# cisco/thor

Hardware: AMD Instinct MI355X
Metric: encoder Mpixels/s at fixed qp, bit-exact recon vs ref (higher is better)
Workload: dtype u8

## Files before the change

### include/thor_hip.h

```cpp
#ifndef THOR_HIP_H
#define THOR_HIP_H
#include <stddef.h>
#include <stdint.h>
#ifdef __cplusplus
extern "C" {
#endif

struct thor_encoder_info;
void encode_frame_lbd(struct thor_encoder_info* encoder_info);
void encode_frame_hbd(struct thor_encoder_info* encoder_info);

typedef struct thor_hip_params {
  int width, height, qp;
  int bitdepth, input_bitdepth;
  float frame_rate;
  float lambda_coeffI, lambda_coeffP;
  float early_skip_thr;
  int enable_tb_split, enable_pb_split, max_num_ref, HQperiod;
  int num_reorder_pics, interp_ref;
  int dqpP, dqpI;
  float mqpP;
  int intra_period, intra_rdo, encoder_speed;
  int deblocking, cdef, clpf, use_block_contexts, enable_bipred;
  int cfl_intra, cfl_inter;
  int dyadic_coding;
  float lambda_coeffB, lambda_coeffB0, lambda_coeffB1, lambda_coeffB2, lambda_coeffB3;
  int dqpB, dqpB0, dqpB1, dqpB2, dqpB3;
  float mqpB, mqpB0, mqpB1, mqpB2, mqpB3;
  int max_clpf_strength;
  int log2_sb_size;
} thor_hip_params;

typedef struct thor_hip_encoder thor_hip_encoder;

int thor_hip_params_from_config(thor_hip_params* p, const char* cfg_path);

int thor_hip_params_set(thor_hip_params* p, const char* name, const char* value);

int thor_hip_params_set_sb_size(thor_hip_params* p, int log2_sb_size);

int thor_hip_device_count(void);
thor_hip_encoder* thor_hip_open(const thor_hip_params* p, int num_streams, int device);
void thor_hip_close(thor_hip_encoder* e);

int thor_hip_begin_sequence(thor_hip_encoder* e, int stream, int skip, int num_frames, int file_frames);
int thor_hip_next_frame(thor_hip_encoder* e, int stream, int* display_index);

size_t thor_hip_frame_bytes(const thor_hip_encoder* e);
int thor_hip_stage_frame(thor_hip_encoder* e, int stream, int slot, const void* yuv);
int thor_hip_stage_frame_device(thor_hip_encoder* e, int stream, int slot, const void* dev_yuv);
int thor_hip_encode_staged(thor_hip_encoder* e, const int* slots);
typedef void (*thor_hip_frames_done_fn)(void* user, int first_stream, int num_streams);
int thor_hip_encode_staged_run(thor_hip_encoder* e, int nframes, thor_hip_frames_done_fn done, void* user);
int thor_hip_last_display_index(const thor_hip_encoder* e, int stream);
int thor_hip_encode_frame(thor_hip_encoder* e, const void* const* yuv_per_stream);

size_t thor_hip_stream_bytes(const thor_hip_encoder* e, int stream);
const uint8_t* thor_hip_stream_data(const thor_hip_encoder* e, int stream);
int thor_hip_get_recon(thor_hip_encoder* e, int stream, void* yuv_out);

void thor_hip_kernel_time(thor_hip_encoder* e, double* sb_ms, long* sb_launches, double* filter_ms);
void thor_hip_kernel_time_reset(thor_hip_encoder* e);
void thor_hip_read_stats(thor_hip_encoder* e, unsigned long long out[4], int reset);
void thor_hip_set_frame_distortion(thor_hip_encoder* e, int on);
typedef struct thor_hip_frame_stats {
  int display_index;
  int frame_type;
  int qp;
  int num_bits;
  int num_ref;
  int ref_array[4];
  int ref_frame_num[4];
  int has_sse;
  unsigned long long sse[3];
  double psnr[3];
} thor_hip_frame_stats;
int thor_hip_frame_stats_count(const thor_hip_encoder* e, int stream);
int thor_hip_get_frame_stats(const thor_hip_encoder* e, int stream, int i, thor_hip_frame_stats* out);
int thor_hip_report(const thor_hip_encoder* e, int stream, char* buf, size_t n);
int thor_hip_stat_line(const thor_hip_encoder* e, int stream, int num_frames, char* buf, size_t n);

void thor_hip_read_prof(thor_hip_encoder* e, long long out[32]);

int thor_hip_sad_batch(const uint8_t* org, int w, int h, const uint8_t* ref_plane, int plane_w, int plane_h,
                       int rstride, int bx, int by, const int* cand, int n, uint32_t* out);
int thor_hip_interp_luma(const uint8_t* ref_plane, int plane_w, int plane_h, int rstride, int pad, int bx, int by,
                         int w, int h, const int16_t* mv, int n, int bipred, uint8_t* out);
int thor_hip_code_tu_batch(const uint8_t* org, const uint8_t* pred, int size, int qp, int coeff_type, int fast, int n,
                           int16_t* coefq, uint8_t* rec, int* cbp);
typedef struct thor_hip_cell {
  int16_t mv0x, mv0y, mv1x, mv1y;
  uint8_t mode, size, tbpb, cbp;
  int8_t ref0, ref1, dir;
  uint8_t pad;
} thor_hip_cell;
int thor_hip_deblock_frame(uint8_t* yuv, int width, int height, int qp, const thor_hip_cell* cells);

int thor_hip_sad_batch_hbd(const uint16_t* org, int w, int h, const uint16_t* ref_plane, int plane_w, int plane_h,
                           int rstride, int bx, int by, const int* cand, int n, uint32_t* out);
int thor_hip_interp_luma_hbd(const uint16_t* ref_plane, int plane_w, int plane_h, int rstride, int pad, int bx, int by,
                             int w, int h, const int16_t* mv, int n, int bipred, int bitdepth, uint16_t* out);
int thor_hip_code_tu_batch_hbd(const uint16_t* org, const uint16_t* pred, int size, int qp, int coeff_type, int fast, int n,
                               int bitdepth, int16_t* coefq, uint16_t* rec, int* cbp);
int thor_hip_deblock_frame_hbd(uint16_t* yuv, int width, int height, int qp, int bitdepth, const thor_hip_cell* cells);

int thor_hip_kat_intra(const void* plane, int width, int height, int stride, int bitdepth, int size, int tb_split, int n, const int* par,
                       const void* rblocks, void* out);
int thor_hip_kat_inter_yuv(const void* yuv, int width, int height, int bitdepth, int size, int n, const int* par, const int16_t* mv, void* out);
int thor_hip_kat_average(const void* a, const void* b, int size, int bitdepth, int n, void* out);
int thor_hip_kat_cfl(const void* y, void* uv, const void* ry, int n_luma, int bitdepth, int n);
int thor_hip_kat_cdef_dir(const void* blocks, int bitdepth, int n, int* dir, int* var);
int thor_hip_kat_cdef_filter(const void* plane, int width, int height, int stride, int bitdepth, int bsize, int n, const int* par, void* out);
int thor_hip_kat_clpf(const void* rec_yuv, const void* org_yuv, int width, int height, int bitdepth, int qp, const thor_hip_cell* cells,
                      const int* strength, int fb_log2, const uint8_t* fb_on, uint32_t* stats, void* out_yuv);
int thor_hip_kat_interpolate(const void* yuv0, const void* yuv1, int width, int height, int bitdepth, void* out_yuv);

int thor_hip_kat_motion_estimate(const void* cur, const void* ref, int width, int height, int bitdepth, int n, const int* par, const double* lambda,
                                 const int16_t* cand, int ncand_total, int* out);
int thor_hip_kat_motion_estimate_bi(const void* cur, const void* ref0, const void* ref1, int width, int height, int bitdepth, int n, const int* par,
                                    const double* lambda, const int16_t* cand, int* out, int16_t* list_out);
int thor_hip_kat_early_skip(const int* chroma, const void* org, const void* pred, const int* size, const int* qp, const float* thr, int bitdepth, int n, int* out);
int thor_hip_kat_coeff_syntax(int n, const int* par, const int16_t* coef, int words, uint32_t* buf_single, uint32_t* buf_team, int* out);
int thor_hip_kat_block_syntax(int n, const int* par, const int16_t* pool, int npool, int words, uint32_t* buf_coop, uint32_t* buf_single, int* out);
int thor_hip_kat_gather_bits(int n, const uint32_t* src, int src_words, const int* src_off, const int* nbits, const long long* dst_bit, uint32_t* dst, int dst_words);

int thor_hip_frame_sse(const void* a, const void* b, int w, int h, int bitdepth, unsigned long long out[3]);
int thor_hip_kat_depth_up(const void* in, int w, int h, int bitdepth, int input_bitdepth, uint16_t* out);
int thor_hip_kat_depth_down(const uint16_t* in, int w, int h, int bitdepth, int input_bitdepth, void* out);
int thor_hip_frame_sse_depth(const void* a, const void* b, int w, int h, int bitdepth, int input_bitdepth, unsigned long long out[3]);

int thor_hip_superblock_kernel_info(int sample_bytes, int* num_regs, int* lds_bytes, int* private_bytes, int* workgroups_per_cu);
int thor_hip_superblock_kernel_in_use(void);

#ifdef __cplusplus
}
#endif
#endif
```

### thor_amd/binding.py

```python
import ctypes as C
import os
import subprocess
import numpy as np

REPO_ROOT = os.path.dirname(os.path.dirname(os.path.abspath(__file__)))
_LIB = None


def lib_path():
    return os.environ.get('THOR_HIP_LIB') or os.path.join(REPO_ROOT, 'thor_amd', 'libthor_hip.so')


HIPCC_FLAGS = ['--offload-arch=gfx950', '-O3', '-std=c++17', '-ffp-contract=off', '-fno-strict-aliasing', '-fPIC', '-pthread']
NATIVE_SOURCES = ['thor_hip.cpp', 'thor_hip_lat.cpp', 'thor_hip_wide.cpp', 'thor_hip_katbits.cpp']


def build_native(force=False):
    csrc = os.path.join(REPO_ROOT, 'thor_amd', 'csrc')
    out = os.path.join(REPO_ROOT, 'thor_amd', 'libthor_hip.so')
    hdrs = [os.path.join(csrc, f) for f in os.listdir(csrc)]
    hdrs += [os.path.join(REPO_ROOT, 'include', f) for f in os.listdir(os.path.join(REPO_ROOT, 'include'))]
    newest = max(os.path.getmtime(h) for h in hdrs)
    if force or not os.path.exists(out) or os.path.getmtime(out) < newest:
        hipcc = '/opt/rocm/bin/hipcc' if os.path.exists('/opt/rocm/bin/hipcc') else 'hipcc'
# ... 250 lines not shown
    return a.ctypes.data_as(C.c_void_p)


def _pix(bitdepth):
    return np.uint16 if bitdepth > 8 else np.uint8


def sad_batch(org, ref_plane, bx, by, cand, bitdepth=8):
    T = _pix(bitdepth)
    org = np.ascontiguousarray(org, dtype=T); ref_plane = np.ascontiguousarray(ref_plane, dtype=T)
    cand = np.ascontiguousarray(cand, dtype=np.int32)
    out = np.zeros(len(cand), dtype=np.uint32)
    fn = lib().thor_hip_sad_batch_hbd if bitdepth > 8 else lib().thor_hip_sad_batch
    rc = fn(_vp(org), org.shape[1], org.shape[0], _vp(ref_plane), ref_plane.shape[1], ref_plane.shape[0], ref_plane.shape[1], bx, by,
            _vp(cand), len(cand), _vp(out))
    if rc:
        raise RuntimeError(f'thor_hip_sad_batch rc={rc}')
    return out


def interp_luma(ref_padded, pad, pic_w, pic_h, bx, by, w, h, mvs, bipred, bitdepth=8):
    T = _pix(bitdepth)
    ref_padded = np.ascontiguousarray(ref_padded, dtype=T); mvs = np.ascontiguousarray(mvs, dtype=np.int16)
    out = np.zeros((len(mvs), h, w), dtype=T)
    if bitdepth > 8:
        rc = lib().thor_hip_interp_luma_hbd(_vp(ref_padded), pic_w, pic_h, ref_padded.shape[1], pad, bx, by, w, h, _vp(mvs), len(mvs),
                                            bipred, bitdepth, _vp(out))
    else:
        rc = lib().thor_hip_interp_luma(_vp(ref_padded), pic_w, pic_h, ref_padded.shape[1], pad, bx, by, w, h, _vp(mvs), len(mvs),
                                        bipred, _vp(out))
    if rc:
        raise RuntimeError(f'thor_hip_interp_luma rc={rc}')
    return out


def code_tu_batch(org, pred, qp, coeff_type, fast, bitdepth=8):
    T = _pix(bitdepth)
    org = np.ascontiguousarray(org, dtype=T); pred = np.ascontiguousarray(pred, dtype=T)
    n, size = org.shape[0], org.shape[1]
    q = min(size, 16)
    coefq = np.zeros((n, q, q), dtype=np.int16); rec = np.zeros_like(org); cbp = np.zeros(n, dtype=np.int32)
    if bitdepth > 8:
        rc = lib().thor_hip_code_tu_batch_hbd(_vp(org), _vp(pred), size, qp, coeff_type, fast, n, bitdepth, _vp(coefq), _vp(rec), _vp(cbp))
    else:
        rc = lib().thor_hip_code_tu_batch(_vp(org), _vp(pred), size, qp, coeff_type, fast, n, _vp(coefq), _vp(rec), _vp(cbp))
    if rc:
        raise RuntimeError(f'thor_hip_code_tu_batch rc={rc}')
    return coefq, rec, cbp


def deblock_frame(yuv, width, height, qp, cells, bitdepth=8):
    yuv = np.ascontiguousarray(yuv, dtype=_pix(bitdepth)).copy()
    cells = np.ascontiguousarray(cells, dtype=np.uint8)
    assert yuv.size == width * height * 3 // 2 and cells.size == (width // 4) * (height // 4) * 16
    if bitdepth > 8:
        rc = lib().thor_hip_deblock_frame_hbd(_vp(yuv), width, height, qp, bitdepth, _vp(cells))
    else:
        rc = lib().thor_hip_deblock_frame(_vp(yuv), width, height, qp, _vp(cells))
    if rc:
        raise RuntimeError(f'thor_hip_deblock_frame rc={rc}')
    return yuv


def _kat(name, *args):
    fn = getattr(lib(), name)
    fn.restype = C.c_int
    rc = fn(*args)
    if rc:
        raise RuntimeError(f'{name} rc={rc}')


def kat_intra(plane, size, par, bitdepth=8, rblocks=None):
    T = _pix(bitdepth)
    plane = np.ascontiguousarray(plane, dtype=T); par = np.ascontiguousarray(par, dtype=np.int32)
    n = len(par)
    out = np.zeros((n, size, size), dtype=T)
    rb = np.ascontiguousarray(rblocks, dtype=T) if rblocks is not None else None
    _kat('thor_hip_kat_intra', _vp(plane), plane.shape[1], plane.shape[0], plane.shape[1], bitdepth, size, 1 if rb is not None else 0, n, _vp(par),
         _vp(rb) if rb is not None else None, _vp(out))
    return out


def kat_inter_yuv(yuv, width, height, size, par, mvs, bitdepth=8):
    T = _pix(bitdepth)
    yuv = np.ascontiguousarray(yuv, dtype=T); par = np.ascontiguousarray(par, dtype=np.int32); mvs = np.ascontiguousarray(mvs, dtype=np.int16)
    n = len(par)
    out = np.zeros((n, size * size * 3 // 2), dtype=T)
    _kat('thor_hip_kat_inter_yuv', _vp(yuv), width, height, bitdepth, size, n, _vp(par), _vp(mvs), _vp(out))
    return out


def kat_average(a, b, size, bitdepth=8):
    T = _pix(bitdepth)
    a = np.ascontiguousarray(a, dtype=T); b = np.ascontiguousarray(b, dtype=T)
    out = np.zeros_like(a)
    _kat('thor_hip_kat_average', _vp(a), _vp(b), size, bitdepth, len(a), _vp(out))
    return out


def kat_cfl(y, uv, ry, n_luma, bitdepth=8):
    T = _pix(bitdepth)
    y = np.ascontiguousarray(y, dtype=T); ry = np.ascontiguousarray(ry, dtype=T); uv = np.array(uv, dtype=T, order='C')
    _kat('thor_hip_kat_cfl', _vp(y), _vp(uv), _vp(ry), n_luma, bitdepth, len(y))
    return uv


def kat_cdef_dir(blocks, bitdepth=8):
    T = _pix(bitdepth)
    blocks = np.ascontiguousarray(blocks, dtype=T)
    n = len(blocks)
    d = np.zeros(n, dtype=np.int32); v = np.zeros(n, dtype=np.int32)
    _kat('thor_hip_kat_cdef_dir', _vp(blocks), bitdepth, n, _vp(d), _vp(v))
    return d, v


def kat_cdef_filter(plane, bsize, par, bitdepth=8):
    T = _pix(bitdepth)
    plane = np.ascontiguousarray(plane, dtype=T); par = np.ascontiguousarray(par, dtype=np.int32)
    out = np.zeros((len(par), bsize, bsize), dtype=T)
    _kat('thor_hip_kat_cdef_filter', _vp(plane), plane.shape[1], plane.shape[0], plane.shape[1], bitdepth, bsize, len(par), _vp(par), _vp(out))
    return out


def kat_clpf(rec, org, width, height, qp, cells, strength, fb_log2, fb_on, bitdepth=8):
    T = _pix(bitdepth)
    rec = np.ascontiguousarray(rec, dtype=T); org = np.ascontiguousarray(org, dtype=T)
    cells = np.ascontiguousarray(cells, dtype=np.uint8); fb_on = np.ascontiguousarray(fb_on, dtype=np.uint8)
    st = np.ascontiguousarray(strength, dtype=np.int32)
    nblk = (width // 8) * (height // 8) + 2 * (width // 16) * (height // 16)
    stats = np.zeros((nblk, 4), dtype=np.uint32)
    out = np.zeros_like(rec)
    _kat('thor_hip_kat_clpf', _vp(rec), _vp(org), width, height, bitdepth, qp, _vp(cells), _vp(st), fb_log2, _vp(fb_on), _vp(stats), _vp(out))
    return stats, out


def kat_interpolate(yuv0, yuv1, width, height, bitdepth=8):
    T = _pix(bitdepth)
    a = np.ascontiguousarray(yuv0, dtype=T); b = np.ascontiguousarray(yuv1, dtype=T)
    out = np.zeros_like(a)
    _kat('thor_hip_kat_interpolate', _vp(a), _vp(b), width, height, bitdepth, _vp(out))
    return out


def kat_motion_estimate(cur, ref, par, lam, cand, bitdepth=8):
    T = _pix(bitdepth)
    cur = np.ascontiguousarray(cur, dtype=T); ref = np.ascontiguousarray(ref, dtype=T)
    par = np.ascontiguousarray(par, dtype=np.int32); lam = np.ascontiguousarray(lam, dtype=np.float64); cand = np.ascontiguousarray(cand, dtype=np.int16).reshape(-1, 2)
    assert cur.shape == ref.shape and par.shape[1] == 17 and len(lam) == len(par)
    out = np.full((len(par), 3), -1, dtype=np.int32)
    _kat('thor_hip_kat_motion_estimate', _vp(cur), _vp(ref), cur.shape[1], cur.shape[0], bitdepth, len(par), _vp(par), _vp(lam), _vp(cand), len(cand), _vp(out))
    return out


def kat_motion_estimate_bi(cur, ref0, ref1, par, lam, cand, bitdepth=8):
    T = _pix(bitdepth)
    cur, ref0, ref1 = (np.ascontiguousarray(a, dtype=T) for a in (cur, ref0, ref1))
    par = np.ascontiguousarray(par, dtype=np.int32); lam = np.ascontiguousarray(lam, dtype=np.float64); cand = np.ascontiguousarray(cand, dtype=np.int16)
    assert cur.shape == ref0.shape == ref1.shape and par.shape[1] == 17 and len(lam) == len(par) and cand.size == 12 * len(par)
    out = np.full((len(par), 3), -1, dtype=np.int32)
    lists = np.zeros((len(par), 6, 2), dtype=np.int16)
    _kat('thor_hip_kat_motion_estimate_bi', _vp(cur), _vp(ref0), _vp(ref1), cur.shape[1], cur.shape[0], bitdepth, len(par), _vp(par), _vp(lam), _vp(cand), _vp(out), _vp(lists))
    return out, lists


def kat_early_skip(chroma, org, pred, size, qp, thr, bitdepth=8):
    T = _pix(bitdepth)
    org = np.ascontiguousarray(org, dtype=T); pred = np.ascontiguousarray(pred, dtype=T)
    chroma, size, qp = (np.ascontiguousarray(a, dtype=np.int32) for a in (chroma, size, qp))
    thr = np.ascontiguousarray(thr, dtype=np.float32)
    n = len(org)
    assert org.shape == pred.shape == (n, 32, 32) and len(chroma) == len(size) == len(qp) == len(thr) == n
    out = np.full(n, -1, dtype=np.int32)
    _kat('thor_hip_kat_early_skip', _vp(chroma), _vp(org), _vp(pred), _vp(size), _vp(qp), _vp(thr), bitdepth, n, _vp(out))
    return out


def kat_coeff_syntax(par, coef, words, buf_single, buf_team):
    par = np.ascontiguousarray(par, dtype=np.int32); coef = np.ascontiguousarray(coef, dtype=np.int16)
    n = len(par)
    b1 = np.ascontiguousarray(buf_single, dtype=np.uint32).copy(); bt = np.ascontiguousarray(buf_team, dtype=np.uint32).copy()
    assert par.shape == (n, 4) and coef.shape == (n, 256) and b1.shape == (n, words) and bt.shape == (n, words)
    out = np.zeros((n, 6), dtype=np.int32)
    _kat('thor_hip_kat_coeff_syntax', n, _vp(par), _vp(coef), words, _vp(b1), _vp(bt), _vp(out))
    return out, b1, bt


def kat_block_syntax(par, pool, words, fill=0):
    par = np.ascontiguousarray(par, dtype=np.int32); pool = np.ascontiguousarray(pool, dtype=np.int16)
    n = len(par)
    assert par.shape == (n, 57) and pool.ndim == 2 and pool.shape[1] == 256
    bc = np.full((n, words), fill, dtype=np.uint32); b1 = np.full((n, words), fill, dtype=np.uint32)
    out = np.zeros((n, 10), dtype=np.int32)
    _kat('thor_hip_kat_block_syntax', n, _vp(par), _vp(pool), len(pool), words, _vp(bc), _vp(b1), _vp(out))
    return out, bc, b1


def kat_gather_bits(src, src_off, nbits, dst_bit, dst_words):
    src = np.ascontiguousarray(src, dtype=np.uint32); src_off = np.ascontiguousarray(src_off, dtype=np.int32)
    nbits = np.ascontiguousarray(nbits, dtype=np.int32); dst_bit = np.ascontiguousarray(dst_bit, dtype=np.int64)
    dst = np.zeros(dst_words, dtype=np.uint32)
    _kat('thor_hip_kat_gather_bits', len(nbits), _vp(src), len(src), _vp(src_off), _vp(nbits), _vp(dst_bit), _vp(dst), dst_words)
    return dst


def frame_sse(a, b, width, height, bitdepth=8):
    T = _pix(bitdepth)
    a = np.ascontiguousarray(a, dtype=T).reshape(-1); b = np.ascontiguousarray(b, dtype=T).reshape(-1)
    if a.size != width * height * 3 // 2 or b.size != a.size:
        raise ValueError('frame size does not match width x height 4:2:0')
    out = (C.c_ulonglong * 3)()
    rc = lib().thor_hip_frame_sse(_vp(a), _vp(b), width, height, bitdepth, out)
    if rc:
        raise RuntimeError(f'thor_hip_frame_sse returned {rc}')
    return [int(v) for v in out]


def _depth_frame(a, depth, width, height):
    a = np.ascontiguousarray(a, dtype=_pix(depth)).reshape(-1)
    if a.size != width * height * 3 // 2:
        raise ValueError('frame size does not match width x height 4:2:0')
    return a


def kat_depth_up(frame, width, height, bitdepth, input_bitdepth):
    a = _depth_frame(frame, input_bitdepth, width, height)
    out = np.zeros(a.size, dtype=np.uint16)
    _kat('thor_hip_kat_depth_up', _vp(a), width, height, bitdepth, input_bitdepth, _vp(out))
    return out


def kat_depth_down(frame, width, height, bitdepth, input_bitdepth):
    a = _depth_frame(frame, 16, width, height)
    out = np.zeros(a.size, dtype=_pix(input_bitdepth))
    _kat('thor_hip_kat_depth_down', _vp(a), width, height, bitdepth, input_bitdepth, _vp(out))
    return out


def frame_sse_depth(a, b, width, height, bitdepth, input_bitdepth):
    T = 16 if bitdepth > input_bitdepth else bitdepth
    a = _depth_frame(a, T, width, height); b = _depth_frame(b, T, width, height)
    out = (C.c_ulonglong * 3)()
    _kat('thor_hip_frame_sse_depth', _vp(a), _vp(b), width, height, bitdepth, input_bitdepth, out)
    return [int(v) for v in out]
```

### thor_amd/csrc/hip_kat.h

```cpp
#pragma once
#include "tk_kat_bits.h"
namespace tk {
template <typename PIX>
__global__ __launch_bounds__(64) void k_kat_sad(const PIX* org, int w, int h, const PIX* refp, int rstride, int bx, int by, const int* cand, int n,
                                               uint32_t* out) {
  const Team t = mk_team((int)threadIdx.x, 64);
  struct KC { const PIX* p; int dx, dy; };
  MeWin win;
  win.on = 0; win.w32 = nullptr; win.ox = win.oy = win.Ww = win.Wh = win.pitch = 0;
  auto cnd = [&](int c) -> KC {
    KC x;
    x.dx = cand[2 * c]; x.dy = cand[2 * c + 1];
    x.p = refp + (size_t)(by + x.dy) * rstride + bx + x.dx;
    return x;
  };
  seg_sads<SP_GLOBAL>(t, n, org, w, rstride, w, h, win, cnd, [&](int c, const KC&, int sad, int mine) { if (mine) out[c] = (uint32_t)sad; });
}
template <typename PIX>
__global__ __launch_bounds__(64) void k_kat_interp(const PIX* ref0, int rstride, int pic_w, int pic_h, int bx, int by, int w, int h,
                                                  const int16_t* mv, int bipred, int bitdepth, PIX* out) {
  const Team t = mk_team((int)threadIdx.x, 64);
  const int i = blockIdx.x;
  pred_luma<SP_GLOBAL>(t, out + (size_t)i * w * h, w, ref0 + (size_t)by * rstride + bx, rstride, w, h, mk_mv(mv[2 * i], mv[2 * i + 1]), 0,
            bipred, pic_w, pic_h, bx, by, bitdepth);
}
template <typename PIX>
__global__ __launch_bounds__(64) void k_kat_tu(const PIX* org, const PIX* pred, int size, int qp, int coeff_type, int fast, int bitdepth,
                                              int16_t* coefq, PIX* rec, int* cbp) {
  __shared__ XformWs xf;
  __shared__ XformTabs tabs;
  __shared__ int16_t cq[256];
  const Team t = mk_team((int)threadIdx.x, 64, tabs.izz);
  xf.prof = nullptr;
  xf.tabs = &tabs;
  xform_tables_fill(&tabs, (int)threadIdx.x, 64);
  t.sync();
  const int i = blockIdx.x, qs = size < 16 ? size : 16;
  const size_t o = (size_t)i * size * size;
  int c = code_tu(t, &xf, org + o, size, pred + o, size, rec + o, size, size, qp, coeff_type, fast, cq, bitdepth);
  for (int k = threadIdx.x; k < qs * qs; k += 64) coefq[(size_t)i * qs * qs + k] = cq[k];
  if (threadIdx.x == 0) cbp[i] = c;
}

template <typename PIX>
__global__ __launch_bounds__(64) void k_kat_intra(const PIX* plane, int stride, int bitdepth, int size, int tb_split, const int* par, const PIX* rblocks,
                                                 PIX* out) {
  __shared__ IntraEdge<PIX> edge;
  const Team t = mk_team((int)threadIdx.x, 64);
  const int it = blockIdx.x;
  const int* q = par + 7 * it;
  const int cbs = tb_split ? 2 * size : size;
  const PIX* rblock = tb_split ? rblocks + (size_t)it * cbs * cbs + q[5] * cbs + q[6] : nullptr;
  make_edges<SP_GLOBAL>(t, &edge, plane + (size_t)q[0] * stride + q[1], stride, rblock, cbs, q[5], q[6], q[0], q[1], size, q[2], q[3], tb_split, bitdepth);
  pred_intra<SP_GLOBAL>(t, &edge, q[0] + q[5], q[1] + q[6], size, out + (size_t)it * size * size, size, q[4], bitdepth);
}
template <typename PIX>
__global__ __launch_bounds__(kWgThreads, (sizeof(PIX) == 1 ? (int)kOcc : 2)) void k_kat_inter_yuv(Plane3<PIX> ref, int width, int height, int bitdepth, int size, const int* par, const int16_t* mv, PIX* out) {
  const Team t = mk_team((int)threadIdx.x, 64);
  const int it = blockIdx.x;
  const int* q = par + 5 * it;
  mv_t m[4];
  for (int k = 0; k < 4; k++) m[k] = mk_mv(mv[(it * 4 + k) * 2], mv[(it * 4 + k) * 2 + 1]);
  PIX* o = out + (size_t)it * (size * size * 3 / 2);
  pred_inter_yuv<SP_GLOBAL>(t, ref, o, o + size * size, o + size * size * 5 / 4, q[0], q[1], size, size, size, m, q[2], width, height, q[3], q[4], bitdepth);
}
template <typename PIX> __global__ __launch_bounds__(64) void k_kat_average(const PIX* a, const PIX* b, int size, PIX* out) {
  const Team t = mk_team((int)threadIdx.x, 64);
  const size_t o = (size_t)blockIdx.x * (size * size * 3 / 2);
  const int n = size * size, c = n / 4;
  average_yuv<SP_GLOBAL>(t, out + o, out + o + n, out + o + n + c, a + o, a + o + n, a + o + n + c, b + o, b + o + n, b + o + n + c, size, size, size);
}
template <typename PIX>
__global__ __launch_bounds__(kWgThreads, (sizeof(PIX) == 1 ? (int)kOcc : 2)) void k_kat_cfl(const PIX* y, PIX* uv, const PIX* ry, int n, int bitdepth) {
  const Team t = mk_team((int)threadIdx.x, 64);
  const int it = blockIdx.x, c = (n / 2) * (n / 2);
  improve_uv<PIX, SP_GLOBAL>(t, nullptr, y + (size_t)it * n * n, uv + (size_t)it * 2 * c, uv + (size_t)it * 2 * c + c, ry + (size_t)it * n * n, n, n, n, bitdepth);
}
template <typename PIX> __global__ void k_kat_cdef_dir(const PIX* blocks, int n, int cs, int* dir, int* var) {
  const int i = (int)(blockIdx.x * blockDim.x + threadIdx.x);
  if (i >= n) return;
  int v = 0;
  dir[i] = cdef_find_dir(blocks + (size_t)i * 64, 8, &v, cs);
  var[i] = v;
}
template <typename PIX>
__global__ __launch_bounds__(64) void k_kat_cdef_filter(const PIX* plane, int w, int h, int stride, int bsize, int cs, const int* par, PIX* out) {
  const int it = blockIdx.x, k = threadIdx.x;
  if (k >= bsize * bsize) return;
  const int* q = par + 7 * it;
  const int x = q[0] + k % bsize, y = q[1] + k / bsize;
  out[(size_t)it * bsize * bsize + k] = (PIX)cdef_filter_px(plane, stride, x, y, w, h, q[2], q[3], q[4], q[5], q[6], cs);
}
enum { kKatMePar = 17 };
template <typename PIX>
__global__ __launch_bounds__(kWgThreads, (sizeof(PIX) == 1 ? (int)kOcc : 2)) void k_kat_me(int bi, Plane3<PIX> cur, Plane3<PIX> ref0, Plane3<PIX> ref1, int fw, int fh, int bitdepth,
                                                                                           const int* par, const double* lam, const int16_t* cand, unsigned char* big, int* out,
                                                                                           int16_t* list_out) {
  __shared__ WgShared sh;
  __shared__ SmallWs<PIX> sws;
  const int lane = (int)threadIdx.x, it = (int)blockIdx.x;
  TeamWs<PIX> ws = make_ws(&sws, &sh, (BigWs<PIX>*)big);
  const Team t = mk_team(lane, 64, sh.tabs.izz);
  xform_tables_fill(&sh.tabs, lane, 64);
  const int* q = par + kKatMePar * it;
  const int cbx = q[0], cby = q[1], cb = q[2], pux = cbx + q[3], puy = cby + q[4];
  MeLists* lists = &sh.lists;
  const int nl = bi ? 6 : q[14];
  for (int c = lane; c < nl; c += 64) { lists->mvcand[0][c].x = cand[2 * (q[15] + c)]; lists->mvcand[0][c].y = cand[2 * (q[15] + c) + 1]; }
  if (lane == 0) { lists->mvcand_num[0] = q[14]; lists->mvcand_mask[0] = 0; lists->best_ref = 0; }
  const int lds_blk = __builtin_amdgcn_readfirstlane(cb <= kLdsBlk);
  PIX* orgc = (PIX*)sh.org_raw;
  if (lds_blk)
    for (int k = lane; k < cb * cb; k += 64) orgc[k] = cur.y[(size_t)(cby + k / cb) * cur.sy + cbx + k % cb];
  __syncthreads();
  MeArgs a;
  a.cb_size = cb; a.ostride = lds_blk ? cb : cur.sy; a.width = q[5]; a.height = q[6]; a.rstride = ref0.sy; a.sign = q[11]; a.fwidth = fw; a.fheight = fh;
  a.xpos = cbx; a.ypos = cby; a.pu_x = pux; a.pu_y = puy; a.enable_bipred = q[12]; a.bitdepth = bitdepth; a.speed = q[13]; a.lam = lam[it];
  const mv_t mvc = mk_mv(q[7], q[8]), mvp = mk_mv(q[9], q[10]);
  const PIX* org = lds_blk ? orgc + q[4] * cb + q[3] : cur.y + (size_t)puy * cur.sy + pux;
  mv_t mv = mk_mv(0, 0);
  unsigned cost;
  if (bi) {
    const PIX* r0 = ref0.y + (size_t)cby * ref0.sy + cbx;
    const PIX* r1 = ref1.y + (size_t)cby * ref1.sy + cbx;
    cost = lds_blk ? motion_estimate_bi<PIX, SP_LDS>(t, ws.mep, org, r0, r1, a, mvc, mvp, 0, &mv) : motion_estimate_bi<PIX, SP_GLOBAL>(t, ws.mep, org, r0, r1, a, mvc, mvp, 0, &mv);
  } else {
    if (q[16]) me_stage_cb_window<PIX>(t, ws.mep, ref0.y + (size_t)cby * ref0.sy + cbx, ref0.sy, cbx, cby, cb, mvc, a.sign, fw, fh, 0);
    const PIX* rp = ref0.y + (size_t)puy * ref0.sy + pux;
    cost = lds_blk ? motion_estimate<PIX, SP_LDS>(t, ws.mep, org, rp, a, mvc, mvp, 0, &mv) : motion_estimate<PIX, SP_GLOBAL>(t, ws.mep, org, rp, a, mvc, mvp, 0, &mv);
  }
  __syncthreads();
  if (lane == 0) { out[3 * it] = mv.x; out[3 * it + 1] = mv.y; out[3 * it + 2] = (int)cost; }
  if (bi && lane < 6) { list_out[12 * it + 2 * lane] = lists->mvcand[0][lane].x; list_out[12 * it + 2 * lane + 1] = lists->mvcand[0][lane].y; }
}
template <typename PIX>
__global__ __launch_bounds__(kWgThreads, (sizeof(PIX) == 1 ? (int)kOcc : 2)) void k_kat_early_skip(const int* chroma, const PIX* org, const PIX* pred, const int* size, const int* qp,
                                                                                                   const float* thr, int bitdepth, unsigned char* big, int* out) {
  __shared__ FrameJob<PIX> sJ;
  __shared__ WgShared sh;
  __shared__ SmallWs<PIX> sws;
  __shared__ TeamWs<PIX> s_view;
  const int lane = (int)threadIdx.x, it = (int)blockIdx.x;
  lds_st(&s_view, make_ws(&sws, &sh, (BigWs<PIX>*)big));
  WsP<PIX> ws = ldsc(&s_view);
  JobR<PIX> J = *ldsc(&sJ);
  const Team t = mk_team(lane, 64, sh.tabs.izz);
  xform_tables_fill(&sh.tabs, lane, 64);
  if (lane == 0) sJ.cfg.bitdepth = bitdepth;
  const int ch = __builtin_amdgcn_readfirstlane(chroma[it]), n = __builtin_amdgcn_readfirstlane(size[it]), qpi = __builtin_amdgcn_readfirstlane(qp[it]);
  const float th = thr[it];
  const PIX* o = org + (size_t)it * 1024;
  const PIX* p = pred + (size_t)it * 1024;
  const int lds_blk = n <= (ch ? kLdsBlk / 2 : kLdsBlk);
  PIX* lo = sws.lbuf;
  PIX* lp = sws.lbuf + kLdsBlk * kLdsBlk;
  if (lds_blk)
    for (int k = lane; k < n * n; k += 64) { lo[k] = o[(k / n) * 32 + k % n]; lp[k] = p[(k / n) * 32 + k % n]; }
  __syncthreads();
  int r;
  if (ch) r = lds_blk ? early_skip_subC<PIX, SP_LDS>(t, J, ws, lo, n, lp, n, n, qpi, th) : early_skip_subC<PIX, SP_GLOBAL>(t, J, ws, o, 32, p, 32, n, qpi, th);
  else r = lds_blk ? early_skip_sub<PIX, SP_LDS>(t, J, ws, lo, n, lp, n, n, qpi, th) : early_skip_sub<PIX, SP_GLOBAL>(t, J, ws, o, 32, p, 32, n, qpi, th);
  if (lane == 0) out[it] = r;
}
}

template <typename PIX>
static int kat_sad_batch(const PIX* org, int w, int h, const PIX* ref_plane, int plane_w, int plane_h, int rstride, int bx, int by, const int* cand,
                         int n, uint32_t* out) {
  if (!org || !ref_plane || !cand || !out || n <= 0 || w < 4 || h < 4 || (w & (w - 1)) || (h & (h - 1))) return 1;
  for (int i = 0; i < n; i++) {
    int x = bx + cand[2 * i], y = by + cand[2 * i + 1];
    if (x < 0 || y < 0 || x + w > plane_w || y + h > plane_h) return 2;
  }
  if (!ensure_init_any()) return 3;
  DevBuf<PIX> d_org((size_t)w * h, org);
  DevBuf<PIX> d_ref((size_t)rstride * plane_h + 16);
  backend::h2d(d_ref, ref_plane, (size_t)rstride * plane_h * sizeof(PIX));
  DevBuf<int> d_c((size_t)2 * n, cand);
  DevBuf<uint32_t> d_o(n);
  hipLaunchKernelGGL(k_kat_sad<PIX>, dim3(1), dim3(64), 0, g_stream, d_org, w, h, d_ref, rstride, bx, by, d_c, n, d_o);
  HIPCHECK(hipGetLastError());
  backend::d2h(out, d_o, (size_t)n * 4);
  return 0;
}
extern "C" int thor_hip_sad_batch(const uint8_t* org, int w, int h, const uint8_t* ref_plane, int plane_w, int plane_h, int rstride,
                                  int bx, int by, const int* cand, int n, uint32_t* out) {
  return kat_sad_batch<uint8_t>(org, w, h, ref_plane, plane_w, plane_h, rstride, bx, by, cand, n, out);
}
extern "C" int thor_hip_sad_batch_hbd(const uint16_t* org, int w, int h, const uint16_t* ref_plane, int plane_w, int plane_h, int rstride,
                                      int bx, int by, const int* cand, int n, uint32_t* out) {
  return kat_sad_batch<uint16_t>(org, w, h, ref_plane, plane_w, plane_h, rstride, bx, by, cand, n, out);
}

template <typename PIX>
static int kat_interp_luma(const PIX* ref_plane, int plane_w, int plane_h, int rstride, int pad, int bx, int by, int w, int h, const int16_t* mv,
                           int n, int bipred, int bitdepth, PIX* out) {
  if (!ref_plane || !mv || !out || n <= 0) return 1;
  if (!ensure_init_any()) return 3;
  DevBuf<PIX> d_ref((size_t)rstride * (plane_h + 2 * pad), ref_plane);
  DevBuf<int16_t> d_mv((size_t)2 * n, mv);
  DevBuf<PIX> d_o((size_t)n * w * h);
  hipLaunchKernelGGL(k_kat_interp<PIX>, dim3(n), dim3(64), 0, g_stream, d_ref.get() + (size_t)pad * rstride + pad, rstride, plane_w, plane_h, bx,
                     by, w, h, d_mv, bipred, bitdepth, d_o);
  HIPCHECK(hipGetLastError());
  backend::d2h(out, d_o, (size_t)n * w * h * sizeof(PIX));
  return 0;
}
extern "C" int thor_hip_interp_luma(const uint8_t* ref_plane, int plane_w, int plane_h, int rstride, int pad, int bx, int by, int w,
                                    int h, const int16_t* mv, int n, int bipred, uint8_t* out) {
  return kat_interp_luma<uint8_t>(ref_plane, plane_w, plane_h, rstride, pad, bx, by, w, h, mv, n, bipred, 8, out);
}
extern "C" int thor_hip_interp_luma_hbd(const uint16_t* ref_plane, int plane_w, int plane_h, int rstride, int pad, int bx, int by, int w,
                                        int h, const int16_t* mv, int n, int bipred, int bitdepth, uint16_t* out) {
  if (bitdepth < 9 || bitdepth > 12) return 1;
  return kat_interp_luma<uint16_t>(ref_plane, plane_w, plane_h, rstride, pad, bx, by, w, h, mv, n, bipred, bitdepth, out);
}

template <typename PIX>
static int kat_code_tu_batch(const PIX* org, const PIX* pred, int size, int qp, int coeff_type, int fast, int n, int bitdepth, int16_t* coefq,
                             PIX* rec, int* cbp) {
  if (!org || !pred || !coefq || !rec || !cbp || n <= 0) return 1;
  if (size != 4 && size != 8 && size != 16 && size != 32 && size != 64 && size != 128) return 2;
  if (!ensure_init_any()) return 3;
  const size_t px = (size_t)n * size * size;
  const int qs = size < 16 ? size : 16;
  DevBuf<PIX> d_org(px, org), d_pred(px, pred), d_rec(px);
  DevBuf<int16_t> d_cq((size_t)n * qs * qs);
  DevBuf<int> d_cbp(n);
  hipLaunchKernelGGL(k_kat_tu<PIX>, dim3(n), dim3(64), 0, g_stream, d_org, d_pred, size, qp, coeff_type, fast, bitdepth, d_cq, d_rec,
                     d_cbp);
  HIPCHECK(hipGetLastError());
  backend::d2h(coefq, d_cq, (size_t)n * qs * qs * 2);
  backend::d2h(rec, d_rec, px * sizeof(PIX));
  backend::d2h(cbp, d_cbp, (size_t)n * 4);
  return 0;
}
extern "C" int thor_hip_code_tu_batch(const uint8_t* org, const uint8_t* pred, int size, int qp, int coeff_type, int fast, int n,
                                      int16_t* coefq, uint8_t* rec, int* cbp) {
  return kat_code_tu_batch<uint8_t>(org, pred, size, qp, coeff_type, fast, n, 8, coefq, rec, cbp);
}
extern "C" int thor_hip_code_tu_batch_hbd(const uint16_t* org, const uint16_t* pred, int size, int qp, int coeff_type, int fast, int n,
                                          int bitdepth, int16_t* coefq, uint16_t* rec, int* cbp) {
  if (bitdepth < 9 || bitdepth > 12) return 1;
  return kat_code_tu_batch<uint16_t>(org, pred, size, qp, coeff_type, fast, n, bitdepth, coefq, rec, cbp);
}

template <typename PIX> static int kat_deblock_frame(PIX* yuv, int width, int height, int qp, int bitdepth, const thor_hip_cell* cells) {
  static_assert(sizeof(thor_hip_cell) == sizeof(DbCell), "thor_hip_cell must mirror tk::DbCell");
  if (!yuv || !cells || width % 8 || height % 8 || width < 16 || height < 16 || qp < 0 || qp > 51) return 1;
  if (!ensure_init_any()) return 3;
  DevFrame<PIX> f;
  f.alloc(width, height, 0);
  DevBuf<DbCell> d_cells((size_t)(width / 4) * (height / 4), (const DbCell*)cells);
  upload_yuv(f, yuv, width, height);
  FrameJob<PIX> J;
  memset(&J, 0, sizeof(J));
  J.cfg.width = width; J.cfg.height = height; J.cfg.bitdepth = bitdepth;
  J.qp = qp; J.rec = f.p; J.cells = d_cells; J.cell_stride = width / 4;
  DevBuf<FrameJob<PIX>> d_job(1, &J);
  backend::run_deblock<PIX>(d_job, &J, 1);
  backend::dev_sync();
  download_yuv(f, yuv, width, height);
  f.release();
  return 0;
}
extern "C" int thor_hip_deblock_frame(uint8_t* yuv, int width, int height, int qp, const thor_hip_cell* cells) {
  return kat_deblock_frame<uint8_t>(yuv, width, height, qp, 8, cells);
}
extern "C" int thor_hip_deblock_frame_hbd(uint16_t* yuv, int width, int height, int qp, int bitdepth, const thor_hip_cell* cells) {
  if (bitdepth < 9 || bitdepth > 12) return 1;
  return kat_deblock_frame<uint16_t>(yuv, width, height, qp, bitdepth, cells);
}

namespace {
template <typename PIX>
int kat_intra(const PIX* plane, int width, int height, int stride, int bitdepth, int size, int tb_split, int n, const int* par, const PIX* rblocks, PIX* out) {
  if (!plane || !par || !out || n <= 0 || size < 4 || size > 64 || (size & (size - 1)) || (tb_split && !rblocks) || stride < width) return 1;
  const int cbs = tb_split ? 2 * size : size;
  for (int i = 0; i < n; i++) {
    const int* q = par + 7 * i;
    if (q[0] < 0 || q[1] < 0 || q[0] + cbs > height || q[1] + cbs > width || q[4] < 0 || q[5] < 0 || q[6] < 0 || q[5] + size > cbs || q[6] + size > cbs) return 2;
    if ((q[2] && q[1] + 2 * cbs > width) || (q[3] && q[0] + 2 * cbs > height)) return 2;
  }
  if (!ensure_init_any()) return 3;
  DevBuf<PIX> d_p((size_t)stride * height, plane);
  DevBuf<int> d_par((size_t)7 * n, par);
  DevBuf<PIX> d_rb(tb_split ? (size_t)n * cbs * cbs : 0, tb_split ? rblocks : nullptr);
  DevBuf<PIX> d_o((size_t)n * size * size);
// ... 29 lines not shown
  const size_t per = (size_t)size * size * 3 / 2;
  DevBuf<PIX> d_o(per * n);
  hipLaunchKernelGGL(k_kat_inter_yuv<PIX>, dim3(n), dim3(64), 0, g_stream, ref.p, width, height, bitdepth, size, d_par, d_mv, d_o);
  HIPCHECK(hipGetLastError());
  backend::d2h(out, d_o, per * n * sizeof(PIX));
  ref.release();
  return 0;
}
template <typename PIX> int kat_average(const PIX* a, const PIX* b, int size, int n, PIX* out) {
  if (!a || !b || !out || n <= 0 || size < 8 || size > 128 || (size & (size - 1))) return 1;
  if (!ensure_init_any()) return 3;
  const size_t tot = (size_t)n * size * size * 3 / 2;
  DevBuf<PIX> d_a(tot, a), d_b(tot, b), d_o(tot);
  hipLaunchKernelGGL(k_kat_average<PIX>, dim3(n), dim3(64), 0, g_stream, d_a, d_b, size, d_o);
  HIPCHECK(hipGetLastError());
  backend::d2h(out, d_o, tot * sizeof(PIX));
  return 0;
}
template <typename PIX> int kat_cfl(const PIX* y, PIX* uv, const PIX* ry, int nl, int bitdepth, int n) {
  if (!y || !uv || !ry || n <= 0 || nl < 8 || nl > 128 || (nl & (nl - 1))) return 1;
  if (!ensure_init_any()) return 3;
  const size_t ny = (size_t)n * nl * nl, nc = (size_t)n * 2 * (nl / 2) * (nl / 2);
  DevBuf<PIX> d_y(ny, y), d_r(ny, ry), d_uv(nc, uv);
  hipLaunchKernelGGL(k_kat_cfl<PIX>, dim3(n), dim3(64), 0, g_stream, d_y, d_uv, d_r, nl, bitdepth);
  HIPCHECK(hipGetLastError());
  backend::d2h(uv, d_uv, nc * sizeof(PIX));
  return 0;
}
template <typename PIX> int kat_cdef_dir(const PIX* blocks, int bitdepth, int n, int* dir, int* var) {
  if (!blocks || !dir || !var || n <= 0) return 1;
  if (!ensure_init_any()) return 3;
  DevBuf<PIX> d_b((size_t)n * 64, blocks);
  DevBuf<int> d_d(n), d_v(n);
  hipLaunchKernelGGL(k_kat_cdef_dir<PIX>, dim3((n + 63) / 64), dim3(64), 0, g_stream, d_b, n, bitdepth - 8, d_d, d_v);
  HIPCHECK(hipGetLastError());
  backend::d2h(dir, d_d, (size_t)n * 4); backend::d2h(var, d_v, (size_t)n * 4);
  return 0;
}
template <typename PIX> int kat_cdef_filter(const PIX* plane, int w, int h, int stride, int bitdepth, int bsize, int n, const int* par, PIX* out) {
  if (!plane || !par || !out || n <= 0 || (bsize != 4 && bsize != 8) || stride < w) return 1;
  for (int i = 0; i < n; i++) {
    const int* q = par + 7 * i;
    if (q[0] < 0 || q[1] < 0 || q[0] + bsize > w || q[1] + bsize > h || q[4] < 0 || q[4] > 7) return 2;
  }
  if (!ensure_init_any()) return 3;
  DevBuf<PIX> d_p((size_t)stride * h, plane);
  DevBuf<int> d_par((size_t)7 * n, par);
  DevBuf<PIX> d_o((size_t)n * bsize * bsize);
  hipLaunchKernelGGL(k_kat_cdef_filter<PIX>, dim3(n), dim3(64), 0, g_stream, d_p, w, h, stride, bsize, bitdepth - 8, d_par, d_o);
  HIPCHECK(hipGetLastError());
  backend::d2h(out, d_o, (size_t)n * bsize * bsize * sizeof(PIX));
  return 0;
}
template <typename PIX>
int kat_clpf(const PIX* rec_yuv, const PIX* org_yuv, int width, int height, int bitdepth, int qp, const thor_hip_cell* cells, const int* strength, int fb_log2,
             const uint8_t* fb_on, uint32_t* stats, PIX* out_yuv) {
  if (!rec_yuv || !org_yuv || !cells || !strength || !fb_on || !stats || !out_yuv || width % 16 || height % 16 || fb_log2 < 5 || fb_log2 > 7) return 1;
  if (!ensure_init_any()) return 3;
  DevFrame<PIX> rec, src, org;
  rec.alloc(width, height, 0); src.alloc(width, height, 0); org.alloc(width, height, 0);
  upload_yuv(rec, rec_yuv, width, height); upload_yuv(src, rec_yuv, width, height); upload_yuv(org, org_yuv, width, height);
  DevBuf<DbCell> d_cells((size_t)(width / 4) * (height / 4), (const DbCell*)cells);
  const int nblk = (width / 8) * (height / 8) + 2 * (width / 16) * (height / 16);
  const int nfb = ((width + (1 << fb_log2) - 1) >> fb_log2) * ((height + (1 << fb_log2) - 1) >> fb_log2);
  DevBuf<uint32_t> d_stats((size_t)4 * nblk);
  DevBuf<uint8_t> d_on((size_t)nfb, fb_on);
  ClpfJob<PIX> J;
  memset(&J, 0, sizeof(J));
  J.rec = rec.p; J.src = src.p; J.org = org.p; J.width = width; J.height = height; J.bitdepth = bitdepth; J.qp = qp;
  J.cells = d_cells; J.cs = width / 4; J.stats = d_stats;
  for (int k = 0; k < 3; k++) J.strength[k] = strength[k];
  J.fb_log2 = fb_log2; J.fb_on = d_on;
  DevBuf<ClpfJob<PIX>> d_job(1, &J);
  backend::run_clpf_stats<PIX>(d_job, &J, 1);
  backend::run_clpf_apply<PIX>(d_job, &J, 1);
  backend::dev_sync();
  backend::d2h(stats, d_stats, (size_t)4 * nblk * 4);
  download_yuv(rec, out_yuv, width, height);
  rec.release(); src.release(); org.release();
  return 0;
}
template <typename PIX> int kat_interpolate(const PIX* yuv0, const PIX* yuv1, int width, int height, int bitdepth, PIX* out_yuv) {
  if (!yuv0 || !yuv1 || !out_yuv || width % 8 || height % 8 || width < 64 || height < 64) return 1;
  if (!ensure_init_any()) return 3;
  SeqParams sp;
  sp.width = width; sp.height = height; sp.bitdepth = bitdepth; sp.input_bitdepth = bitdepth;
  sp.num_reorder_pics = 7; sp.interp_ref = 1; sp.max_num_ref = 2; sp.HQperiod = 8; sp.cdef = 0; sp.clpf = 0;
  Engine<PIX>* eng = new Engine<PIX>();
  eng->open(sp, 1);
  Stream<PIX>& q = eng->st[0];
  for (int k = 0; k < 2; k++) {
    upload_yuv(q.rec, k ? yuv1 : yuv0, width, height);
    FrameJob<PIX> J;
    memset(&J, 0, sizeof(J));
    J.cfg.width = width; J.cfg.height = height; J.rec = q.rec.p;
    backend::run_make_ref<PIX>(&J, &q.ring[k].p, 1);
    backend::dev_sync();
  }
  std::vector<FrameParams> fp(1);
  fp[0].interp_ref = 1; fp[0].interp_src[0] = 0; fp[0].interp_src[1] = 1; fp[0].frame_num = 1;
  eng->make_interp_frames(fp, 0, 1);
  backend::dev_sync();
  download_yuv(q.interp, out_yuv, width, height);
  eng->close();
  delete eng;
  return 0;
}
template <typename PIX> DevFrame<PIX> kat_luma_frame(const PIX* luma, int width, int height, int pad_ref) {
  std::vector<PIX> yuv((size_t)width * height * 3 / 2, (PIX)0);
  memcpy(yuv.data(), luma, (size_t)width * height * sizeof(PIX));
  if (pad_ref) return kat_padded_ref(yuv.data(), width, height);
  DevFrame<PIX> f;
  f.alloc(width, height, 0);
  upload_yuv(f, yuv.data(), width, height);
  return f;
}
template <typename PIX>
int kat_me(int bi, const PIX* cur, const PIX* ref0, const PIX* ref1, int width, int height, int bitdepth, int n, const int* par, const double* lam, const int16_t* cand,
           int ncand_total, int* out, int16_t* list_out) {
  if (!cur || !ref0 || (bi && (!ref1 || !list_out)) || !par || !lam || !out || n <= 0 || ncand_total < 0 || (ncand_total && !cand) || width % 8 || height % 8 || width < 16 ||
      height < 16 || width > 8192 || height > 8192)
    return 1;
  auto pow2 = [](int v, int lo, int hi) { return v >= lo && v <= hi && !(v & (v - 1)); };
  for (int i = 0; i < n; i++) {
    const int* q = par + kKatMePar * i;
    if (!pow2(q[2], 8, kMaxSb) || !pow2(q[5], 4, q[2]) || !pow2(q[6], 4, q[2]) || (q[11] & ~1) || (q[12] & ~1) || q[13] < 0 || q[13] > 2 || !(lam[i] >= 0.0 && lam[i] <= 1e6)) return 1;
    if (q[0] < 0 || q[1] < 0 || q[0] + q[2] > width || q[1] + q[2] > height || q[3] < 0 || q[4] < 0 || q[3] + q[5] > q[2] || q[4] + q[6] > q[2] || q[3] % 4 || q[4] % 4) return 2;
    for (int k = 7; k <= 10; k++) if (q[k] < -8192 || q[k] > 8192) return 1;
    const int slots = bi ? 6 : q[14];
    if (q[14] < 0 || q[14] > (bi ? 6 : 64) || q[15] < 0 || q[15] + slots > ncand_total) return 2;
    if (bi && (q[3] || q[4] || q[5] != q[2] || q[6] != q[2])) return 1;
    for (int c = 0; c < slots; c++) if (cand[2 * (q[15] + c)] < -2047 || cand[2 * (q[15] + c)] > 2047 || cand[2 * (q[15] + c) + 1] < -2047 || cand[2 * (q[15] + c) + 1] > 2047) return 1;
  }
  if (!ensure_init_any()) return 3;
  DevFrame<PIX> fc = kat_luma_frame(cur, width, height, 0), f0 = kat_luma_frame(ref0, width, height, 1), f1 = bi ? kat_luma_frame(ref1, width, height, 1) : DevFrame<PIX>();
  {
    DevBuf<int> d_par((size_t)kKatMePar * n, par);
    DevBuf<double> d_lam(n, lam);
    DevBuf<int16_t> d_cand((size_t)2 * (ncand_total ? ncand_total : 1));
    if (ncand_total) backend::h2d(d_cand, cand, (size_t)4 * ncand_total);
    DevBuf<unsigned char> d_big(sizeof(BigWs<PIX>));
    DevBuf<int> d_o((size_t)3 * n);
    DevBuf<int16_t> d_l((size_t)12 * n);
    hipLaunchKernelGGL(k_kat_me<PIX>, dim3(n), dim3(64), 0, g_stream, bi, fc.p, f0.p, bi ? f1.p : f0.p, width, height, bitdepth, d_par, d_lam, d_cand, d_big, d_o, d_l);
    HIPCHECK(hipGetLastError());
    backend::d2h(out, d_o, (size_t)3 * n * 4);
    if (bi) backend::d2h(list_out, d_l, (size_t)12 * n * 2);
  }
  fc.release(); f0.release();
  if (bi) f1.release();
  return 0;
}
template <typename PIX>
int kat_early_skip(const int* chroma, const PIX* org, const PIX* pred, const int* size, const int* qp, const float* thr, int bitdepth, int n, int* out) {
  if (!chroma || !org || !pred || !size || !qp || !thr || !out || n <= 0) return 1;
  for (int i = 0; i < n; i++) {
    const int s = size[i];
    if ((chroma[i] & ~1) || qp[i] < 0 || qp[i] > 51 || !(thr[i] >= 0.0f && thr[i] <= 1e3f)) return 1;
    if (chroma[i] ? (s != 4 && s != 8 && s != 16) : (s != 8 && s != 16 && s != 32)) return 2;
  }
  if (!ensure_init_any()) return 3;
  DevBuf<PIX> d_org((size_t)n * 1024, org), d_pred((size_t)n * 1024, pred);
  DevBuf<int> d_ch(n, chroma), d_size(n, size), d_qp(n, qp), d_o(n);
  DevBuf<float> d_thr(n, thr);
  DevBuf<unsigned char> d_big(sizeof(BigWs<PIX>));
  hipLaunchKernelGGL(k_kat_early_skip<PIX>, dim3(n), dim3(64), 0, g_stream, d_ch, d_org, d_pred, d_size, d_qp, d_thr, bitdepth, d_big, d_o);
  HIPCHECK(hipGetLastError());
  backend::d2h(out, d_o, (size_t)n * 4);
  return 0;
}
}
#define KAT_BD(call8, call16) do { if (bitdepth == 8) return call8; if (bitdepth >= 9 && bitdepth <= 12) return call16; return 1; } while (0)
extern "C" int thor_hip_kat_intra(const void* plane, int width, int height, int stride, int bitdepth, int size, int tb_split, int n, const int* par,
                                  const void* rblocks, void* out) {
  KAT_BD(kat_intra<uint8_t>((const uint8_t*)plane, width, height, stride, 8, size, tb_split, n, par, (const uint8_t*)rblocks, (uint8_t*)out),
         kat_intra<uint16_t>((const uint16_t*)plane, width, height, stride, bitdepth, size, tb_split, n, par, (const uint16_t*)rblocks, (uint16_t*)out));
}
extern "C" int thor_hip_kat_inter_yuv(const void* yuv, int width, int height, int bitdepth, int size, int n, const int* par, const int16_t* mv, void* out) {
  KAT_BD(kat_inter_yuv<uint8_t>((const uint8_t*)yuv, width, height, 8, size, n, par, mv, (uint8_t*)out),
         kat_inter_yuv<uint16_t>((const uint16_t*)yuv, width, height, bitdepth, size, n, par, mv, (uint16_t*)out));
}
extern "C" int thor_hip_kat_average(const void* a, const void* b, int size, int bitdepth, int n, void* out) {
  KAT_BD(kat_average<uint8_t>((const uint8_t*)a, (const uint8_t*)b, size, n, (uint8_t*)out),
         kat_average<uint16_t>((const uint16_t*)a, (const uint16_t*)b, size, n, (uint16_t*)out));
}
extern "C" int thor_hip_kat_cfl(const void* y, void* uv, const void* ry, int n_luma, int bitdepth, int n) {
  KAT_BD(kat_cfl<uint8_t>((const uint8_t*)y, (uint8_t*)uv, (const uint8_t*)ry, n_luma, 8, n),
         kat_cfl<uint16_t>((const uint16_t*)y, (uint16_t*)uv, (const uint16_t*)ry, n_luma, bitdepth, n));
}
extern "C" int thor_hip_kat_cdef_dir(const void* blocks, int bitdepth, int n, int* dir, int* var) {
  KAT_BD(kat_cdef_dir<uint8_t>((const uint8_t*)blocks, 8, n, dir, var), kat_cdef_dir<uint16_t>((const uint16_t*)blocks, bitdepth, n, dir, var));
}
extern "C" int thor_hip_kat_cdef_filter(const void* plane, int width, int height, int stride, int bitdepth, int bsize, int n, const int* par, void* out) {
  KAT_BD(kat_cdef_filter<uint8_t>((const uint8_t*)plane, width, height, stride, 8, bsize, n, par, (uint8_t*)out),
         kat_cdef_filter<uint16_t>((const uint16_t*)plane, width, height, stride, bitdepth, bsize, n, par, (uint16_t*)out));
}
extern "C" int thor_hip_kat_clpf(const void* rec_yuv, const void* org_yuv, int width, int height, int bitdepth, int qp, const thor_hip_cell* cells,
                                 const int* strength, int fb_log2, const uint8_t* fb_on, uint32_t* stats, void* out_yuv) {
  KAT_BD(kat_clpf<uint8_t>((const uint8_t*)rec_yuv, (const uint8_t*)org_yuv, width, height, 8, qp, cells, strength, fb_log2, fb_on, stats, (uint8_t*)out_yuv),
         kat_clpf<uint16_t>((const uint16_t*)rec_yuv, (const uint16_t*)org_yuv, width, height, bitdepth, qp, cells, strength, fb_log2, fb_on, stats, (uint16_t*)out_yuv));
}
extern "C" int thor_hip_kat_motion_estimate(const void* cur, const void* ref, int width, int height, int bitdepth, int n, const int* par, const double* lambda,
                                            const int16_t* cand, int ncand_total, int* out) {
  KAT_BD(kat_me<uint8_t>(0, (const uint8_t*)cur, (const uint8_t*)ref, nullptr, width, height, 8, n, par, lambda, cand, ncand_total, out, nullptr),
         kat_me<uint16_t>(0, (const uint16_t*)cur, (const uint16_t*)ref, nullptr, width, height, bitdepth, n, par, lambda, cand, ncand_total, out, nullptr));
}
extern "C" int thor_hip_kat_motion_estimate_bi(const void* cur, const void* ref0, const void* ref1, int width, int height, int bitdepth, int n, const int* par,
                                               const double* lambda, const int16_t* cand, int* out, int16_t* list_out) {
  KAT_BD(kat_me<uint8_t>(1, (const uint8_t*)cur, (const uint8_t*)ref0, (const uint8_t*)ref1, width, height, 8, n, par, lambda, cand, 6 * n, out, list_out),
         kat_me<uint16_t>(1, (const uint16_t*)cur, (const uint16_t*)ref0, (const uint16_t*)ref1, width, height, bitdepth, n, par, lambda, cand, 6 * n, out, list_out));
}
extern "C" int thor_hip_kat_early_skip(const int* chroma, const void* org, const void* pred, const int* size, const int* qp, const float* thr, int bitdepth, int n, int* out) {
  KAT_BD(kat_early_skip<uint8_t>(chroma, (const uint8_t*)org, (const uint8_t*)pred, size, qp, thr, 8, n, out),
         kat_early_skip<uint16_t>(chroma, (const uint16_t*)org, (const uint16_t*)pred, size, qp, thr, bitdepth, n, out));
}
extern "C" int thor_hip_kat_coeff_syntax(int n, const int* par, const int16_t* coef, int words, uint32_t* buf_single, uint32_t* buf_team, int* out) {
  if (n <= 0 || !par || !coef || words <= 0 || words > (1 << 16) || !buf_single || !buf_team || !out) return 1;
  for (int i = 0; i < n; i++) if (kat_coeff_check(par + kKatCoPar * i, words)) return 1;
  if (!ensure_init_any()) return 3;
  DevBuf<int> d_par((size_t)kKatCoPar * n, par), d_o((size_t)kKatCoOut * n);
  DevBuf<int16_t> d_c((size_t)256 * n, coef);
  DevBuf<uint32_t> d_1((size_t)words * n, buf_single), d_t((size_t)words * n, buf_team);
  if (thor_katbits_launch_coeff(g_stream, n, d_par, d_c, words, d_1, d_t, d_o)) return 3;
  backend::d2h(buf_single, d_1, (size_t)words * n * 4); backend::d2h(buf_team, d_t, (size_t)words * n * 4);
  backend::d2h(out, d_o, (size_t)kKatCoOut * n * 4);
  return 0;
}
extern "C" int thor_hip_kat_block_syntax(int n, const int* par, const int16_t* pool, int npool, int words, uint32_t* buf_coop, uint32_t* buf_single, int* out) {
  if (n <= 0 || !par || npool < 0 || (npool && !pool) || words <= 0 || words > (1 << 16) || !buf_coop || !buf_single || !out) return 1;
  std::vector<int16_t> coef((size_t)n * 3072);
  for (int i = 0; i < n; i++) if (kat_block_resolve(par + kKatBlPar * i, pool, npool, coef.data() + (size_t)i * 3072)) return 1;
  if (!ensure_init_any()) return 3;
  DevBuf<int> d_par((size_t)kKatBlPar * n, par), d_o((size_t)kKatBlOut * n);
  DevBuf<int16_t> d_c(coef.size(), coef.data());
  DevBuf<uint32_t> d_w((size_t)words * n, buf_coop), d_1((size_t)words * n, buf_single);
  if (thor_katbits_launch_block(g_stream, n, d_par, d_c, words, d_w, d_1, d_o)) return 3;
  backend::d2h(buf_coop, d_w, (size_t)words * n * 4); backend::d2h(buf_single, d_1, (size_t)words * n * 4);
  backend::d2h(out, d_o, (size_t)kKatBlOut * n * 4);
  return 0;
}
extern "C" int thor_hip_kat_gather_bits(int n, const uint32_t* src, int src_words, const int* src_off, const int* nbits, const long long* dst_bit, uint32_t* dst, int dst_words) {
  if (n <= 0 || !src || src_words <= 0 || !src_off || !nbits || !dst_bit || !dst || dst_words <= 0) return 1;
  for (int i = 0; i < n; i++) {
    if (nbits[i] < 0 || src_off[i] < 0 || dst_bit[i] < 0) return 1;
    if ((long long)src_off[i] + (nbits[i] + 31) / 32 > src_words || dst_bit[i] + nbits[i] > (long long)dst_words * 32) return 2;
  }
  if (!ensure_init_any()) return 3;
  std::vector<backend::GatherItem> items(n);
  DevBuf<uint32_t> d_src((size_t)src_words, src), d_dst((size_t)dst_words);
  for (int i = 0; i < n; i++) {
    items[i].src = d_src.get() + src_off[i]; items[i].nbits = nbits[i]; items[i].dst_bit = dst_bit[i];
  }
  DevBuf<backend::GatherItem> d_items((size_t)n, items.data());
  backend::run_gather(d_items, n, d_dst);
  backend::d2h(dst, d_dst, (size_t)dst_words * 4);
  return 0;
}
template <typename PIX> int frame_sse_host(const PIX* a, const PIX* b, int width, int height, unsigned long long out[3]) {
  if (!a || !b || !out || width % 8 || height % 8 || width < 8 || height < 8) return 1;
  if (!ensure_init_any()) return 3;
  DevFrame<PIX> fa, fb;
  fa.alloc(width, height, 0); fb.alloc(width, height, 0);
  upload_yuv(fa, a, width, height); upload_yuv(fb, b, width, height);
  FrameJob<PIX> J;
  memset(&J, 0, sizeof(J));
  J.cfg.width = width; J.cfg.height = height; J.orig = fa.p; J.rec = fb.p;
  DevBuf<FrameJob<PIX>> dj(1, &J);
  DevBuf<unsigned long long> dout(4);
  launch_frame_sse<PIX>(dj, &J, 1, dout);
  backend::dev_sync();
  backend::d2h(out, dout, 3 * sizeof(unsigned long long));
  fa.release(); fb.release();
  return 0;
}
extern "C" int thor_hip_frame_sse(const void* a, const void* b, int w, int h, int bitdepth, unsigned long long out[3]) {
  KAT_BD(frame_sse_host<uint8_t>((const uint8_t*)a, (const uint8_t*)b, w, h, out),
         frame_sse_host<uint16_t>((const uint16_t*)a, (const uint16_t*)b, w, h, out));
}
static int kat_depth_args(const void* a, const void* b, int w, int h, int bitdepth, int input_bitdepth) {
  auto ok = [](int d) { return d == 8 || d == 10 || d == 12; };
  return !a || !b || w % 8 || h % 8 || w < 8 || h < 8 || !ok(bitdepth) || !ok(input_bitdepth) || input_bitdepth >= bitdepth;
}
extern "C" int thor_hip_kat_depth_up(const void* in, int w, int h, int bitdepth, int input_bitdepth, uint16_t* out) {
  if (kat_depth_args(in, out, w, h, bitdepth, input_bitdepth)) return 1;
  if (!ensure_init_any()) return 3;
  const size_t bytes = (size_t)w * h * 3 / 2 * (input_bitdepth > 8 ? 2 : 1);
  DevBuf<uint8_t> packed(bytes, (const uint8_t*)in);
  DevFrame<uint16_t> f;
  f.alloc(w, h, 0);
  launch_depth_up(packed, f.p, w, h, bitdepth, input_bitdepth);
  backend::dev_sync();
  download_yuv(f, out, w, h);
  f.release();
  return 0;
}
extern "C" int thor_hip_kat_depth_down(const uint16_t* in, int w, int h, int bitdepth, int input_bitdepth, void* out) {
  if (kat_depth_args(in, out, w, h, bitdepth, input_bitdepth)) return 1;
  if (!ensure_init_any()) return 3;
  const size_t bytes = (size_t)w * h * 3 / 2 * (input_bitdepth > 8 ? 2 : 1);
  DevBuf<uint8_t> packed(bytes);
  DevFrame<uint16_t> f;
  f.alloc(w, h, 0);
  upload_yuv(f, in, w, h);
  launch_depth_down(f.p, packed, w, h, bitdepth, input_bitdepth);
  backend::d2h(out, packed, bytes);
  f.release();
  return 0;
}
extern "C" int thor_hip_frame_sse_depth(const void* a, const void* b, int w, int h, int bitdepth, int input_bitdepth, unsigned long long out[3]) {
  if (bitdepth == input_bitdepth) return thor_hip_frame_sse(a, b, w, h, bitdepth, out);
  if (!out || kat_depth_args(a, b, w, h, bitdepth, input_bitdepth)) return 1;
  if (!ensure_init_any()) return 3;
  DevFrame<uint16_t> fa, fb;
  fa.alloc(w, h, 0); fb.alloc(w, h, 0);
  upload_yuv(fa, (const uint16_t*)a, w, h); upload_yuv(fb, (const uint16_t*)b, w, h);
  FrameJob<uint16_t> J;
  memset(&J, 0, sizeof(J));
  J.cfg.width = w; J.cfg.height = h; J.orig = fa.p; J.rec = fb.p;
  DevBuf<FrameJob<uint16_t>> dj(1, &J);
  DevBuf<unsigned long long> dout(4);
  launch_frame_sse_depth(dj, &J, 1, bitdepth, input_bitdepth, dout);
  backend::dev_sync();
  backend::d2h(out, dout, 3 * sizeof(unsigned long long));
  fa.release(); fb.release();
  return 0;
}
extern "C" int thor_hip_kat_interpolate(const void* yuv0, const void* yuv1, int width, int height, int bitdepth, void* out_yuv) {
  KAT_BD(kat_interpolate<uint8_t>((const uint8_t*)yuv0, (const uint8_t*)yuv1, width, height, 8, (uint8_t*)out_yuv),
         kat_interpolate<uint16_t>((const uint16_t*)yuv0, (const uint16_t*)yuv1, width, height, bitdepth, (uint16_t*)out_yuv));
}

extern "C" int thor_hip_superblock_kernel_info(int sample_bytes, int* num_regs, int* lds_bytes, int* private_bytes, int* workgroups_per_cu) {
  if (!ensure_init_any()) return 3;
  hipFuncAttributes a;
  int per_cu = 0;
  if (sample_bytes == 1) {
    HIPCHECK(hipFuncGetAttributes(&a, reinterpret_cast<const void*>(&k_superblocks<uint8_t>)));
    HIPCHECK(hipOccupancyMaxActiveBlocksPerMultiprocessor(&per_cu, k_superblocks<uint8_t>, kWgThreads, 0));
  } else if (sample_bytes == 2) {
    HIPCHECK(hipFuncGetAttributes(&a, reinterpret_cast<const void*>(&k_superblocks<uint16_t>)));
    HIPCHECK(hipOccupancyMaxActiveBlocksPerMultiprocessor(&per_cu, k_superblocks<uint16_t>, kWgThreads, 0));
  } else if (sample_bytes == 0) {
    if (thor_lat_kernel_info(num_regs, lds_bytes, private_bytes)) return 2;
    if (workgroups_per_cu) *workgroups_per_cu = thor_lat_workgroups_per_cu();
    return 0;
  } else if (sample_bytes == 3) {
    if (thor_wide_kernel_info(num_regs, lds_bytes, private_bytes)) return 2;
    if (workgroups_per_cu) *workgroups_per_cu = thor_wide_workgroups_per_cu();
    return 0;
  } else return 1;
  if (num_regs) *num_regs = a.numRegs;
  if (lds_bytes) *lds_bytes = (int)a.sharedSizeBytes;
  if (private_bytes) *private_bytes = (int)a.localSizeBytes;
  if (workgroups_per_cu) *workgroups_per_cu = per_cu;
  return 0;
}
extern "C" int thor_hip_superblock_kernel_in_use(void) { return tk::backend::g_last_kern; }
```

### thor_amd/csrc/tk_block_md.h

```cpp
#pragma once
#include "tk_block_search.h"

namespace tk {
template <typename PIX, int SP>
TK_DEVNI unsigned mode_decision(const Team t, JobR<PIX> J, WsP<PIX> ws, Node& nd) {
  const auto& c = J.cfg;
  const int size = nd.size;
  const double lambda = J.lambda;
  const int rect = nd.bw != size || nd.bh != size;
  const int max_tb = c.enable_tb_split == 1 ? 2 : 1;
  const int max_pb = c.enable_pb_split ? 4 : 1;
  unsigned min_cost = kCostInit;
  int do_inter = 1, do_intra = 1;
  BlkParam p;
  p.mode = M_SKIP; p.intra_mode = 0; p.skip_idx = 0; p.pb_part = P_NONE; p.ref0 = p.ref1 = 0; p.dir = 0;
  p.tb_param = 0; p.tb_split = 0; p.cbp_y = p.cbp_u = p.cbp_v = 0;
  for (int i = 0; i < 4; i++) { p.mv0[i] = mk_mv(0, 0); p.mv1[i] = mk_mv(0, 0); }

  if (J.frame_type != F_I) {
    p.tb_param = 0;
    p.pb_part = P_NONE;
    for (int k = 0; k < nd.syn.num_skip; k++) {
      set_cand(p, nd.skip[k], k, M_SKIP);
      unsigned cost = rdo_trial<PIX, SP>(t, J, ws, nd, p, lambda);
      if (cost < min_cost) { min_cost = cost; if (t.rank == 0) keep_best(nd, p); }
    }
  }
  if ((size < 128 || c.encoder_speed == 0) && !rect) {
    if (J.frame_type != F_I) {
      for (int k = 0; k < nd.syn.num_merge; k++) {
        set_cand(p, nd.merge[k], k, M_MERGE);
        for (int tb = 0; tb <= max_tb - 1; tb++) {
          p.tb_param = (int8_t)tb;
          unsigned cost = rdo_trial<PIX, SP>(t, J, ws, nd, p, lambda, tb > 0, min_cost);
          if (cost < min_cost) { min_cost = cost; if (t.rank == 0) keep_best(nd, p); }
        }
      }
      const int intra_inter_sad = c.encoder_speed > 0;
      unsigned sad_intra = 0xffffffffu;
      if (intra_inter_sad) {
        int im;
        sad_intra = intra_sad_search<PIX, SP>(t, J, ws, nd, J.num_intra_modes, &im);
        sad_intra += (unsigned)(int)mul_add_nofma(J.sqrt_lambda, 2.0, 0.5);
      }
      mv_t mv_center[kMaxRefs];
      mv_t mv_all[4][4];
      mv_t mvp = mk_mv(0, 0);
      const PIX* oy = ws->org_y;
      int min_idx = 0, max_idx = J.num_ref - 1;
      {
        const int br = ws->mep->lists->best_ref;
        if (!(br < 0 || c.encoder_speed < 2 || c.enable_bipred)) min_idx = max_idx = br;
      }
      if (J.frame_type == F_B && J.interp_ref > 2) min_idx = 1;
      unsigned worst_cost = 0, best_cost = 0xffffffffu;
      for (int r = min_idx; r <= max_idx; r++) {
        mvp = get_mv_pred(J.cells, J.cell_stride, nd.ypos, nd.xpos, c.width, c.height, size, sb_size_of(c));
        if (t.rank == 0) add_mvcand(ws->mep, r, mvp);
        t.sync();
        nd.syn.mvp = mvp;
        mv_center[r] = mvp;
        unsigned sad_inter = 0xffffffffu;
        for (int part = 0; part < max_pb; part++) {
          unsigned sad = search_inter<PIX, SP>(t, J, ws, nd.ypos, nd.xpos, size, oy, ws->org_sy, r, mv_center[r], mvp, mv_all[part], part, J.sign[r]);
          add_cands4(t, ws, r, mv_all[part]);
          mv_center[r] = mv_all[0][0];
          sad_inter = sad < sad_inter ? sad : sad_inter;
        }
        if (intra_inter_sad) {
          do_inter = sad_inter < sad_intra;
          if (sad_inter < sad_intra) do_intra = 0;
        }
        if (!do_inter) continue;
        p.mode = M_INTER;
        p.ref0 = p.ref1 = (int8_t)r;
        for (int part = 0; part < max_pb; part++) {
          p.pb_part = (int8_t)part;
          for (int i = 0; i < 4; i++) { p.mv0[i] = mv_all[part][i]; p.mv1[i] = mv_all[part][i]; }
          const int min_tb = c.encoder_speed < 1 ? -1 : 0;
          for (int tb = min_tb; tb <= max_tb - 1; tb++) {
            p.tb_param = (int8_t)tb;
            unsigned cost = rdo_trial<PIX, SP>(t, J, ws, nd, p, lambda, tb > min_tb, (c.encoder_speed < 2 || c.enable_bipred) ? min_cost : 0xffffffffu);
            worst_cost = cost > worst_cost ? cost : worst_cost;
            best_cost = cost < best_cost ? cost : best_cost;
            if (cost < min_cost) { min_cost = cost; if (t.rank == 0) keep_best(nd, p); }
          }
        }
      }
      if (worst_cost && worst_cost * 3u > best_cost * 4u) {
        t.sync();
        if (t.rank == 0) ws->mep->lists->best_ref = 0;
        t.sync();
      }
      if (J.num_ref > 1 && c.enable_bipred && do_inter) {
        int r0, r1;
        mv_t a0[4], a1[4];
        search_bipred<PIX, SP>(t, J, ws, nd, 0, mv_center, mvp, &r0, &r1, a0, a1);
        p.mode = M_BIPRED;
        p.pb_part = P_NONE;
        p.ref0 = (int8_t)r0; p.ref1 = (int8_t)r1;
        for (int i = 0; i < 4; i++) { p.mv0[i] = a0[i]; p.mv1[i] = a1[i]; }
        for (int tb = 0; tb <= max_tb - 1; tb++) {
          p.tb_param = (int8_t)tb;
          unsigned cost = rdo_trial<PIX, SP>(t, J, ws, nd, p, lambda, tb > 0, min_cost);
          if (cost < min_cost) { min_cost = cost; if (t.rank == 0) keep_best(nd, p); }
        }
        if (J.frame_type == F_B && c.encoder_speed == 0) {
          const int ri0 = J.interp_ref ? 1 : 0, ri1 = J.interp_ref ? 2 : 1;
          const Plane3<PIX> f0 = lds_ld(&J.ref[ri0]);
          const Plane3<PIX> f1 = lds_ld(&J.ref[ri1]);
          MeArgs a;
          a.cb_size = size; a.ostride = ws->org_sy; a.width = size; a.height = size; a.rstride = f0.sy; a.sign = 0;
          a.fwidth = c.width; a.fheight = c.height; a.xpos = nd.xpos; a.ypos = nd.ypos; a.enable_bipred = 1;
          a.bitdepth = c.bitdepth; a.lam = J.sqrt_lambda; a.speed = c.encoder_speed; a.pu_x = nd.xpos; a.pu_y = nd.ypos;
          mv_t mvb;
          motion_estimate_bi<PIX, SP>(t, ws->mep, oy, f0.y + nd.ypos * f0.sy + nd.xpos, f1.y + nd.ypos * f1.sy + nd.xpos, a, mv_center[ri0],
                             mvp, ri0, &mvb);
          p.mode = M_BIPRED;
          p.pb_part = P_NONE;
          p.ref0 = (int8_t)ri0; p.ref1 = (int8_t)ri1;
          for (int i = 0; i < 4; i++) { p.mv0[i] = mvb; p.mv1[i] = mvb; }
          p.tb_param = 0;
          unsigned cost = rdo_trial<PIX, SP>(t, J, ws, nd, p, lambda);
          if (cost < min_cost) { min_cost = cost; if (t.rank == 0) keep_best(nd, p); }
        }
      }
    }
    p.mode = M_INTRA;
    int intra_mode = 0;
    unsigned best_tb_cost[2] = {kCostInit, kCostInit};
    if (!do_intra) {
    } else if (c.intra_rdo) {
      unsigned min_intra = kCostInit;
      for (int m = 0; m < J.num_intra_modes; m++) {
        p.intra_mode = (int8_t)m;
        unsigned tbc[2] = {kCostInit, kCostInit};
        int improved = 0;
        for (int tb = 0; tb <= max_tb - 1; tb++) {
          p.tb_param = (int8_t)tb;
          unsigned cost = rdo_trial<PIX, SP>(t, J, ws, nd, p, lambda, 0, min_intra < min_cost ? min_intra : min_cost);
          tbc[tb] = cost;
          if (cost < min_intra) { min_intra = cost; intra_mode = m; improved = 1; }
        }
        if (improved) { best_tb_cost[0] = tbc[0]; best_tb_cost[1] = tbc[1]; }
      }
      p.intra_mode = (int8_t)intra_mode;
      for (int tb = 0; tb <= max_tb - 1; tb++) {
        p.tb_param = (int8_t)tb;
        unsigned cost = best_tb_cost[tb];
        if (cost < min_cost) { min_cost = cost; p.cbp_y = p.cbp_u = p.cbp_v = 0; if (t.rank == 0) keep_best(nd, p); }
      }
    } else {
      intra_sad_search<PIX, SP>(t, J, ws, nd, J.num_intra_modes, &intra_mode);
      p.intra_mode = (int8_t)intra_mode;
      for (int tb = 0; tb <= max_tb - 1; tb++) {
        p.tb_param = (int8_t)tb;
        unsigned cost = rdo_trial<PIX, SP>(t, J, ws, nd, p, lambda);
        if (cost < min_cost) { min_cost = cost; if (t.rank == 0) keep_best(nd, p); }
      }
    }
  }
  return min_cost;
}
}
```

### thor_amd/csrc/tk_block_queue.h

```cpp
#pragma once
#include "tk_block_md.h"

namespace tk {
TK_DEV BlkParam blank_param() {
  BlkParam p;
  p.mode = M_SKIP; p.intra_mode = 0; p.skip_idx = 0; p.pb_part = P_NONE; p.ref0 = p.ref1 = 0; p.dir = 0;
  p.tb_param = 0; p.tb_split = 0; p.cbp_y = p.cbp_u = p.cbp_v = 0;
  for (int i = 0; i < 4; i++) { p.mv0[i] = mk_mv(0, 0); p.mv1[i] = mk_mv(0, 0); }
  return p;
}

template <typename PIX, int SP>
TK_DEV void snapshot_trial(const Team t, WsP<PIX> ws, int size, const BlkParam& p) {
  BigWs<PIX>* g = ws->big;
  const int sc = size >> 1;
  copy_block<SP_GLOBAL, SP>(t, g->best_y, size, ws->rec_y, size, size, size);
  copy_block<SP_GLOBAL, SP>(t, g->best_u, sc, ws->rec_u, sc, sc, sc);
  copy_block<SP_GLOBAL, SP>(t, g->best_v, sc, ws->rec_v, sc, sc, sc);
  if (TKU(p.cbp_y) | TKU(p.cbp_u) | TKU(p.cbp_v)) {
    const int tbs = TKU(p.tb_split);
    const int qy = tbs ? tmin(size >> 1, (int)kMaxQuant) : tmin(size, (int)kMaxQuant);
    const int ny = (tbs ? 4 : 1) * qy * qy;
    const int csplit = tbs && sc > 4;
    const int qc = csplit ? tmin(sc >> 1, (int)kMaxQuant) : tmin(sc, (int)kMaxQuant);
    const int nc = (csplit ? 4 : 1) * qc * qc;
    const int16_t *cy = ws->coef_y, *cu = ws->coef_u, *cv = ws->coef_v;
    TK_GLOBAL int16_t* dy = gptr(g->best_cy);
    TK_GLOBAL int16_t* du = gptr(g->best_cu);
    TK_GLOBAL int16_t* dv = gptr(g->best_cv);
    for (int k = t.rank; k < ny; k += t.size) dy[k] = cy[k];
    for (int k = t.rank; k < nc; k += t.size) { du[k] = cu[k]; dv[k] = cv[k]; }
  }
}

template <typename PIX> struct MdCtx {
  Wg wg;
  WgShared* sh;
  Node* nd;
  unsigned long long mykey;
};

template <typename PIX, int SP>
TK_DEV int par_trial(const Team t, JobR<PIX> J, WsP<PIX> ws, MdCtx<PIX>& M, BlkParam& p, unsigned order, int reuse_pred) {
  int untouched = 0;
  const unsigned cost = rdo_trial<PIX, SP>(t, J, ws, *M.nd, p, J.lambda, reuse_pred, 0xffffffffu, &M.sh->bestkey, order, nullptr, &untouched);
  if (cost == (unsigned)kCostInit) return !untouched;
  const unsigned long long key = ((unsigned long long)cost << 32) | order;
  if (key < M.mykey) {
    M.mykey = key;
    if (t.rank == 0) {
      lds_st(&M.sh->wbest[M.wg.wave], normalize_best(*M.nd, p));
      *ldsc(&M.sh->wkey[M.wg.wave]) = key;
      wg_min64(&M.sh->bestkey, key);
    }
    snapshot_trial<PIX, SP>(t, ws, tk_uniform(ldsc(M.nd)->size), p);
    t.sync();
  }
  return 1;
}

TK_DEV void wg_wait_at_least(const Team t, int* p, int at_least) {
  const unsigned long long w0 = wg_clock();
  for (unsigned spins = 1;; spins++) {
    const int d = wg_load_acquire(p);
    if (team_bcast0(t, d) >= at_least) break;
    if ((spins & 1023u) == 0 && tk_uniform64(wg_clock() - w0) > (unsigned long long)kWgWaitLimit) wg_wait_failed();
    wg_pause();
  }
}
template <typename PIX, int SP>
TK_DEVNI int md_bijoint_telescope(const Team t, JobR<PIX> J, WsP<PIX> ws, MdCtx<PIX>& M) {
  const auto& c = J.cfg;
  WgShared* const sh_ = tk_uniform_ptr(M.sh);
  int mine = 0;
  if (t.rank == 0) mine = wg_cas(&sh_->bj_state, 0, 1);
  if (!team_bcast0(t, mine)) return 0;
  const NodePos nd = node_pos(M.nd);
  const int ri0 = J.interp_ref ? 1 : 0, ri1 = J.interp_ref ? 2 : 1;
  const Plane3<PIX> f0 = lds_ld(&J.ref[ri0]);
  const Plane3<PIX> f1 = lds_ld(&J.ref[ri1]);
  MeArgs a;
  a.cb_size = nd.size; a.ostride = ws->org_sy; a.width = nd.size; a.height = nd.size; a.rstride = f0.sy; a.sign = 0;
  a.fwidth = c.width; a.fheight = c.height; a.xpos = nd.xpos; a.ypos = nd.ypos; a.enable_bipred = 1;
  a.bitdepth = c.bitdepth; a.lam = J.sqrt_lambda; a.speed = c.encoder_speed; a.pu_x = nd.xpos; a.pu_y = nd.ypos;
  mv_t mvb = mk_mv(0, 0);
  const mv_t ctr = lds_ld(&sh_->ref_mv[ri0][0][0]);
  const unsigned sad = motion_estimate_bi<PIX, SP>(t, ws->mep, ws->org_y, f0.y + nd.ypos * f0.sy + nd.xpos, f1.y + nd.ypos * f1.sy + nd.xpos, a, ctr,
                                                   lds_ld(&sh_->mvp), ri0, &mvb, 1);
  t.sync();
  if (t.rank == 0) {
    *ldsc(&sh_->bj_sad) = sad;
    lds_st(&sh_->bj_mv, mvb);
    wg_store_release(&sh_->bj_state, 2);
  }
  t.sync();
  return 1;
}

template <typename PIX, int SP>
TK_DEVNI void md_item_bipred(const Team t, JobR<PIX> J, WsP<PIX> ws, MdCtx<PIX>& M) {
  const auto& c = J.cfg;
  Node& nd_ = *M.nd;
  const NodePos nd = node_pos(&nd_);
  const int size = nd.size;
  const int max_tb = c.enable_tb_split == 1 ? 2 : 1;
  const mv_t mvp = lds_ld(&M.sh->mvp);
  mv_t mv_center[kMaxRefs];
  for (int r = 0; r < kMaxRefs; r++) mv_center[r] = lds_ld(&M.sh->mv_center[r]);
  int r0, r1;
  mv_t a0[4], a1[4];
  search_bipred<PIX, SP>(t, J, ws, nd_, 0, mv_center, mvp, &r0, &r1, a0, a1);
  BlkParam p = blank_param();
  p.mode = M_BIPRED; p.pb_part = P_NONE;
  p.ref0 = (int8_t)r0; p.ref1 = (int8_t)r1;
  for (int i = 0; i < 4; i++) { p.mv0[i] = a0[i]; p.mv1[i] = a1[i]; }
  for (int tb = 0, have_pred = 0; tb <= max_tb - 1; tb++) {
    p.tb_param = (int8_t)tb;
    have_pred |= par_trial<PIX, SP>(t, J, ws, M, p, 54u + (unsigned)tb, have_pred);
  }
  if (J.frame_type == F_B) {
    const int ri0 = J.interp_ref ? 1 : 0, ri1 = J.interp_ref ? 2 : 1;
    const Plane3<PIX> f0 = lds_ld(&J.ref[ri0]);
    const Plane3<PIX> f1 = lds_ld(&J.ref[ri1]);
    const PIX* oy = ws->org_y;
    MeArgs a;
    a.cb_size = size; a.ostride = ws->org_sy; a.width = size; a.height = size; a.rstride = f0.sy; a.sign = 0;
    a.fwidth = c.width; a.fheight = c.height; a.xpos = nd.xpos; a.ypos = nd.ypos; a.enable_bipred = 1;
    a.bitdepth = c.bitdepth; a.lam = J.sqrt_lambda; a.speed = c.encoder_speed; a.pu_x = nd.xpos; a.pu_y = nd.ypos;
    WgShared* const sh_ = tk_uniform_ptr(M.sh);
    if (!md_bijoint_telescope<PIX, SP>(t, J, ws, M)) wg_wait_at_least(t, &sh_->bj_state, 2);
    mv_t mvb = lds_ld(&sh_->bj_mv);
    const unsigned sad0 = (unsigned)tk_uniform((int)*ldsc(&sh_->bj_sad));
    motion_estimate_bi<PIX, SP>(t, ws->mep, oy, f0.y + nd.ypos * f0.sy + nd.xpos, f1.y + nd.ypos * f1.sy + nd.xpos, a, mv_center[ri0], mvp, ri0, &mvb, 2, sad0);
    p.mode = M_BIPRED; p.pb_part = P_NONE;
    p.ref0 = (int8_t)ri0; p.ref1 = (int8_t)ri1;
    for (int i = 0; i < 4; i++) { p.mv0[i] = mvb; p.mv1[i] = mvb; }
    p.tb_param = 0;
    par_trial<PIX, SP>(t, J, ws, M, p, 56u, 0);
  }
}

template <typename PIX, int SP>
TK_DEVNI void md_item_ref(const Team t, JobR<PIX> J, WsP<PIX> ws, MdCtx<PIX>& M, int r) {
  const auto& c = J.cfg;
  const NodePos nd = node_pos(M.nd);
  const int size = nd.size;
  const int max_pb = c.enable_pb_split ? 4 : 1;
  const mv_t mvp = lds_ld(&M.sh->mvp);
  const PIX* oy = ws->org_y;
  if (t.rank == 0) add_mvcand(ws->mep, r, mvp);
  t.sync();
  mv_t mv_center = mvp;
  if (t.rank == 0) ldsc(ws->mep)->cwin_valid = 0;
  t.sync();
  for (int part = 0; part < max_pb; part++) {
    mv_t mv_all[4];
    search_inter<PIX, SP>(t, J, ws, nd.ypos, nd.xpos, size, oy, ws->org_sy, r, mv_center, mvp, mv_all, part, J.sign[r]);
    add_cands4(t, ws, r, mv_all);
    if (part == 0) {
      mv_center = mv_all[0];
      if (max_pb > 1) {
        const Plane3<PIX> rp = lds_ld(&J.ref[r]);
        me_stage_cb_window<PIX>(t, ws->mep, rp.y + nd.ypos * rp.sy + nd.xpos, rp.sy, nd.xpos, nd.ypos, size, mv_center, J.sign[r], c.width, c.height, r);
      }
    }
    if (t.rank == 0) {
      for (int i = 0; i < 4; i++) lds_st(&M.sh->ref_mv[r][part][i], mv_all[i]);
      if (part == max_pb - 1) lds_st(&M.sh->mv_center[r], mv_center);
      wg_fetch_add(&M.sh->parts_done[r], 1);
    }
    t.sync();
  }
  if (t.rank == 0) ldsc(ws->mep)->cwin_valid = 0;
  t.sync();
}

template <typename PIX, int SP>
TK_DEVNI void md_item_trial(const Team t, JobR<PIX> J, WsP<PIX> ws, MdCtx<PIX>& M, int r, int part) {
  const auto& c = J.cfg;
  const int max_tb = c.enable_tb_split == 1 ? 2 : 1;
  r = tk_uniform(r); part = tk_uniform(part);
  WgShared* const sh_ = tk_uniform_ptr(M.sh);
  TK_PROFMD_MARK(pwt_);
  wg_wait_at_least(t, &sh_->parts_done[r], part + 1);
  if (TK_PROFMD_ON(2)) TK_PROFMD_ACC(ws, 20, pwt_);
  mv_t mv_all[4][4];
  for (int q = 0; q <= part; q++)
    for (int i = 0; i < 4; i++) mv_all[q][i] = lds_ld(&sh_->ref_mv[r][q][i]);
  int dup = 0;
  for (int q = 0; q < part && c.enable_pb_split; q++) {
    int eq = 1;
    for (int i = 0; i < 4; i++) eq = eq && mv_all[q][i].x == mv_all[part][i].x && mv_all[q][i].y == mv_all[part][i].y;
    dup = dup || eq;
  }
  if (tk_uniform(dup)) return;
  BlkParam p = blank_param();
  p.mode = M_INTER;
  p.ref0 = p.ref1 = (int8_t)r;
  p.pb_part = (int8_t)part;
  for (int i = 0; i < 4; i++) { p.mv0[i] = mv_all[part][i]; p.mv1[i] = mv_all[part][i]; }
  for (int tb = -1, have_pred = 0; tb <= max_tb - 1; tb++) {
    p.tb_param = (int8_t)tb;
    have_pred |= par_trial<PIX, SP>(t, J, ws, M, p, 6u + 12u * (unsigned)r + 3u * (unsigned)part + (unsigned)(tb + 1), have_pred);
  }
}

template <typename PIX, int SP>
TK_DEVNI void bipred_par(const Wg wg, const Team t, JobR<PIX> J, WsP<PIX> ws, MdCtx<PIX>& M) {
  const auto& c = J.cfg;
  WgShared* sh_ = M.sh;
  const auto sh = ldsc(sh_);
  const NodePos nd = node_pos(M.nd);
  const auto lists = ldsc(lds_ld(&ws->mep->lists));
  const int size = nd.size;
  const int num_iter = c.encoder_speed == 0 ? 2 : 1;
  const int max_tb = c.enable_tb_split == 1 ? 2 : 1;
  const mv_t mvp = lds_ld(&sh_->mvp);
  int prev_ref[2] = {-1, -1}, prev_cnt[2][kMaxRefs];
  mv_t prev_mv[2][4];
  mv_t min0[4], min1[4];
  for (int i = 0; i < 4; i++) { min0[i] = mvp; min1[i] = mvp; }
  int ref0 = 0, ref1 = 0;
  unsigned min_sad = 1u << 30;
  if (wg.wave == 0 && t.rank == 0) sh->bp_org8 = ws->org8;
  t.sync();
  wg.barrier();
  PIX* const org8 = (PIX*)sh->bp_org8;
  const int whole = nd.bw == size && nd.bh == size;
  for (int n = 0; n < num_iter; n++)
    for (int list = 1; list >= 0; list--) {
      const int buf = (2 * n + (1 - list)) & 1;
      const mv_t* mo = list ? min0 : min1;
      const int ref_o = list ? ref0 : ref1;
      int same = n > 0 && prev_ref[list] == ref_o;
      for (int i = 0; i < 4; i++) same = same && prev_mv[list][i].x == mo[i].x && prev_mv[list][i].y == mo[i].y;
      for (int r = 0; r < J.num_ref; r++) {
        const int cnt = lists->mvcand_num[r];
        same = same && prev_cnt[list][r] == cnt;
        prev_cnt[list][r] = cnt;
      }
      prev_ref[list] = ref_o;
      for (int i = 0; i < 4; i++) prev_mv[list][i] = mo[i];
      if (tk_uniform(same)) continue;
      if (whole) {
        const Plane3<PIX> rp = lds_ld(&J.ref[ref_o]);
        const int sgn = J.sign[ref_o];
        const mv_t mvc_ = clip_mv(mo[0], nd.ypos, nd.xpos, c.width, c.height, size, size, sgn);
        const SubPel sp = luma_setup(mvc_, sgn, size, size, c.width, c.height, nd.xpos, nd.ypos, c.enable_bipred);
        const PIX* ry = rp.y + nd.ypos * rp.sy + nd.xpos;
        const int rows = (size + wg.nwaves - 1) / wg.nwaves, r0 = tmin(size, wg.wave * rows), r1 = tmin(size, r0 + rows);
        const auto o8 = spc<SP>(org8);
        const auto oys = spc<SP>(ws->org_y);
        const int osy = ws->org_sy;
        const Pow2 pw = mk_pow2(size);
        for (int k = r0 * size + t.rank; k < r1 * size; k += t.size) {
          int i, j;
          split2(pw, k, i, j);
          o8[k] = (PIX)sat_pix(2 * (int)oys[i * osy + j] - luma_sample(ry, rp.sy, i, j, sp, c.enable_bipred, c.bitdepth), c.bitdepth);
        }
      } else if (wg.wave == 0) {
        pred_inter_yuv<SP>(t, lds_ld(&J.ref[ref_o]), ws->pred_y, ws->pred_u, ws->pred_v, nd.ypos, nd.xpos, size, nd.bw, nd.bh, mo, J.sign[ref_o], c.width,
                           c.height, c.enable_bipred, 0, c.bitdepth, 1);
        t.sync();
        build_org8<PIX, SP>(t, org8, ws->org_y, ws->org_sy, ws->pred_y, size, c.bitdepth);
      }
      t.sync();
      wg.barrier();
      for (int r = wg.wave; r < J.num_ref; r += wg.nwaves) {
        mv_t mv_all[4];
        const unsigned sad = search_inter<PIX, SP>(t, J, ws, nd.ypos, nd.xpos, size, org8, size, r, lds_ld(&sh_->mv_center[r]), mvp, mv_all, 0, J.sign[r]);
        add_cands4(t, ws, r, mv_all);
        if (t.rank == 0) { sh->bp_sad2[buf][r] = sad; for (int i = 0; i < 4; i++) lds_st(&sh_->bp_mv2[buf][r][i], mv_all[i]); }
      }
      t.sync();
      wg.barrier();
      for (int r = 0; r < J.num_ref; r++) {
        const unsigned sd = (unsigned)tk_uniform((int)sh->bp_sad2[buf][r]);
        if (sd < min_sad) {
          min_sad = sd;
          if (list) { ref1 = r; for (int i = 0; i < 4; i++) min1[i] = lds_ld(&sh_->bp_mv2[buf][r][i]); }
          else { ref0 = r; for (int i = 0; i < 4; i++) min0[i] = lds_ld(&sh_->bp_mv2[buf][r][i]); }
        }
      }
    }
  for (int tb = 0; tb <= max_tb - 1; tb++)
    if (wg.wave == tb % wg.nwaves) {
      BlkParam p = blank_param();
      p.mode = M_BIPRED; p.pb_part = P_NONE;
      p.ref0 = (int8_t)ref0; p.ref1 = (int8_t)ref1;
      for (int i = 0; i < 4; i++) { p.mv0[i] = min0[i]; p.mv1[i] = min1[i]; }
      p.tb_param = (int8_t)tb;
      par_trial<PIX, SP>(t, J, ws, M, p, 54u + (unsigned)tb, 0);
    }
}

template <typename PIX, int SP>
TK_MDW void md_worker_sp(const Wg wg, const Team t, JobR<PIX> J, WsP<PIX> ws) {
  WgShared* sh_ = ws->sh;
  const auto sh = ldsc(sh_);
  MdCtx<PIX> M;
  M.wg = wg; M.sh = sh_; M.nd = &sh_->stack[sh->node]; M.mykey = ~0ull;
  if (t.rank == 0) sh->wsnap[wg.wave] = (void*)ws->big;
  const auto ndl = ldsc(M.nd);
  ws_select(ws, tk_uniform(ndl->size));
  org_select(t, J, ws, tk_uniform(ndl->size), ndl->ypos, ndl->xpos, ndl->bw, ndl->bh, 0);
  const auto& c = J.cfg;
  const int max_tb = c.enable_tb_split == 1 ? 2 : 1;
  const int n_items = sh->n_items;
#if TK_PROF_MD
  long long pmd_acc_[4] = {0, 0, 0, 0};
#endif
  for (;;) {
    int i = 0;
    if (t.rank == 0) i = wg_fetch_add(&sh_->next_item, 1);
    i = team_bcast0(t, i);
    if (i >= n_items) break;
    const int kind = team_bcast0(t, sh->items[i].kind), ia = team_bcast0(t, sh->items[i].a), ib = team_bcast0(t, sh->items[i].b);
    TK_PROFMD_MARK(pk_);
    if (kind == MD_SKIP) {
      BlkParam p = blank_param();
      set_cand(p, lds_ld(&M.nd->skip[ia]), ia, M_SKIP);
      par_trial<PIX, SP>(t, J, ws, M, p, (unsigned)ia, 0);
    } else if (kind == MD_MERGE) {
      BlkParam p = blank_param();
      set_cand(p, lds_ld(&M.nd->merge[ia]), ia, M_MERGE);
      for (int tb = 0, have_pred = 0; tb <= max_tb - 1; tb++) {
        p.tb_param = (int8_t)tb;
        have_pred |= par_trial<PIX, SP>(t, J, ws, M, p, 2u + 2u * (unsigned)ia + (unsigned)tb, have_pred);
      }
    } else if (kind == MD_INTRA) {
      BlkParam p = blank_param();
      p.mode = M_INTRA; p.intra_mode = (int8_t)ia; p.tb_param = (int8_t)ib;
      par_trial<PIX, SP>(t, J, ws, M, p, 57u + 2u * (unsigned)ia + (unsigned)ib, 0);
    } else if (kind == MD_REF) {
      md_item_ref<PIX, SP>(t, J, ws, M, ia);
      t.sync();
      int done = 0;
      if (t.rank == 0) done = wg_fetch_add(&sh_->refs_done, 1) + 1;
      done = team_bcast0(t, done);
      if (done == sh->n_ref_items && sh->do_bipred == 1) {
        md_item_bipred<PIX, SP>(t, J, ws, M);
      }
    } else if (kind == MD_TRIAL) {
      md_item_trial<PIX, SP>(t, J, ws, M, ia, ib);
    } else if (kind == MD_BIJOINT) {
      wg_wait_at_least(t, &sh_->parts_done[J.interp_ref ? 1 : 0], 1);
      md_bijoint_telescope<PIX, SP>(t, J, ws, M);
    }
#if TK_PROF_MD
    if (TK_PROFMD_ON(1)) {
      const int slot_ = (kind == MD_SKIP || kind == MD_MERGE) ? 0 : kind == MD_INTRA ? 1 : (kind == MD_REF || kind == MD_BIJOINT) ? 2 : 3;
      if (TK_PROFMD_ON(8)) { const long long d_ = TK_CYC() - pk_; pmd_acc_[0] += slot_ == 0 ? d_ : 0; pmd_acc_[1] += slot_ == 1 ? d_ : 0; pmd_acc_[2] += slot_ == 2 ? d_ : 0; pmd_acc_[3] += slot_ == 3 ? d_ : 0; }
      else TK_PROF_ACC(ws, 16 + slot_, pk_);
    }
#endif
  }
#if TK_PROF_MD
  if (TK_PROFMD_ON(8) && t.rank == 0) for (int q_ = 0; q_ < 4; q_++) ws->prof[16 + q_] += pmd_acc_[q_];
#endif
  if (tk_uniform(sh->do_bipred) == 2) {
    t.sync();
    TK_PROF_MARK(pb_);
    wg.barrier();
    bipred_par<PIX, SP>(wg, t, J, ws, M);
    TK_PROF_ACC(ws, 27, pb_);
  }
}
template <typename PIX>
TK_DEV void md_worker(const Wg wg, const Team t, JobR<PIX> J, WsP<PIX> ws) {
  const auto sh = ldsc(ws->sh);
  const int size = tk_uniform(ldsc(&ws->sh->stack[sh->node])->size);
  if (size <= kLdsBlk) md_worker_sp<PIX, SP_LDS>(wg, t, J, ws);
  else md_worker_sp<PIX, SP_GLOBAL>(wg, t, J, ws);
}

template <typename PIX>
TK_DEV void wg_helper_loop(const Wg wg, const Team t, JobR<PIX> J, WsP<PIX> ws) {
  for (;;) {
    TK_PROF_MARK(ph_);
    wg.barrier();
    TK_PROF_ACC(ws, 28, ph_);
    const int cmd = team_bcast0(t, ws->sh->cmd);
    if (cmd == WG_CMD_EXIT) { wg.barrier(); break; }
#ifdef THOR_PROF
    { TK_PROF_MARK(pw_); md_worker(wg, t, J, ws); TK_PROF_ACC(ws, 5, pw_); }
#else
    md_worker(wg, t, J, ws);
#endif
    t.sync();
    wg.barrier();
  }
}

template <typename PIX>
TK_MDW unsigned mode_decision_par(const Wg wg, const Team t, JobR<PIX> J, WsP<PIX> ws, int node, int* win_wave) {
  const auto& c = J.cfg;
  WgShared* sh_ = ws->sh;
  const auto sh = ldsc(sh_);
  const auto nd = ldsc(&sh_->stack[node]);
  const int max_tb = c.enable_tb_split == 1 ? 2 : 1;
  const int inter = J.frame_type != F_I;
  TK_PROFMD_MARK(pqs_);
  mv_t mvp = mk_mv(0, 0);
  if (inter) mvp = get_mv_pred(J.cells, J.cell_stride, nd->ypos, nd->xpos, c.width, c.height, nd->size, sb_size_of(c));
  t.sync();
  if (t.rank == 0) {
    int n = 0;
    auto push = [&](int kind, int a, int b) { sh->items[n].kind = (int8_t)kind; sh->items[n].a = (int8_t)a; sh->items[n].b = (int8_t)b; sh->items[n].pad = 0; n++; };
    static_assert(2 + 2 + kMaxRefs + 1 + 2 * kNumIntraModes + 4 * kMaxRefs <= kMdMaxItems, "work queue too small");
    static_assert(6 + 12 * kMaxRefs <= 54, "evaluation-order layout: the reference trials must end before the bi-prediction trials");
    if (inter) {
      for (int k = 0; k < nd->syn.num_skip; k++) push(MD_SKIP, k, 0);
      for (int k = 0; k < nd->syn.num_merge; k++) push(MD_MERGE, k, 0);
      for (int r = 0; r < J.num_ref; r++) push(MD_REF, r, 0);
      if (J.num_ref > 1 && c.enable_bipred && J.frame_type == F_B) push(MD_BIJOINT, 0, 0);
      nd->syn.mvp.x = mvp.x; nd->syn.mvp.y = mvp.y;
    }
    for (int m = 0; m < J.num_intra_modes; m++)
      for (int tb = 0; tb <= max_tb - 1; tb++) push(MD_INTRA, m, tb);
    if (inter)
      for (int part = 0; part < (c.enable_pb_split ? 4 : 1); part++)
        for (int r = 0; r < J.num_ref; r++) { push(MD_TRIAL, r, part); sh->parts_done[r] = 0; }
    sh->n_items = n; sh->next_item = 0;
    sh->refs_done = 0; sh->n_ref_items = inter ? J.num_ref : 0;
    sh->do_bipred = (inter && J.num_ref > 1 && c.enable_bipred) ? (J.frame_type == F_P ? 2 : 1) : 0;
    sh->bj_state = 0;
    sh->node = node; lds_st(&sh_->mvp, mvp);
    sh->bestkey = ~0ull;
    for (int w = 0; w < kWaves; w++) sh->wkey[w] = ~0ull;
    sh->cmd = WG_CMD_MD;
  }
  t.sync();
  if (TK_PROFMD_ON(4)) TK_PROFMD_ACC(ws, 21, pqs_);
  wg.barrier();
#ifdef THOR_PROF
  { TK_PROF_MARK(pw_); md_worker(wg, t, J, ws); TK_PROF_ACC(ws, 5, pw_); t.sync(); wg.barrier(); TK_PROF_ACC(ws, 29, pw_); }
#else
// ... 18 lines not shown
```

### thor_amd/csrc/tk_block_search.h

```cpp
#pragma once
#include "tk_block_rd.h"

namespace tk {
template <typename PIX, int SP>
TK_DEV unsigned search_inter(const Team t, JobR<PIX> J, WsP<PIX> ws, int ypos, int xpos, int size,
                             const PIX* org, int ostride, int ref_idx, mv_t mvc, mv_t mvp, mv_t* mv_arr, int part,
                             int sign) {
  const Plane3<PIX> ref = lds_ld(&J.ref[ref_idx]);
  const PIX* ref_y = ref.y + ypos * ref.sy + xpos;
  MeArgs a;
  a.cb_size = size; a.rstride = ref.sy; a.sign = sign; a.fwidth = J.cfg.width; a.fheight = J.cfg.height;
  a.xpos = xpos; a.ypos = ypos; a.enable_bipred = J.cfg.enable_bipred; a.bitdepth = J.cfg.bitdepth;
  a.lam = J.sqrt_lambda; a.ostride = ostride; a.speed = J.cfg.encoder_speed;
  unsigned sad = 0;
  mv_t mv, mvp2 = mvp;
  if (part == P_NONE) {
    a.width = size; a.height = size; a.pu_x = xpos; a.pu_y = ypos;
    sad += motion_estimate<PIX, SP>(t, ws->mep, org, ref_y, a, mvc, mvp2, ref_idx, &mv);
    mv_arr[0] = mv_arr[1] = mv_arr[2] = mv_arr[3] = mv;
  } else if (part == P_HOR) {
    a.width = size; a.height = size / 2;
    for (int index = 0; index < 4; index += 2) {
      int py = index >> 1;
      a.pu_x = xpos; a.pu_y = ypos + py * (size / 2);
      sad += motion_estimate<PIX, SP>(t, ws->mep, org + py * (size / 2) * ostride, ref_y + py * (size / 2) * ref.sy, a, mvc, mvp2, ref_idx, &mv);
      mv_arr[index] = mv; mv_arr[index + 1] = mv;
      mvp2 = mv_arr[0];
    }
  } else if (part == P_VER) {
    a.width = size / 2; a.height = size;
    for (int index = 0; index < 2; index++) {
      a.pu_x = xpos + index * (size / 2); a.pu_y = ypos;
      sad += motion_estimate<PIX, SP>(t, ws->mep, org + index * (size / 2), ref_y + index * (size / 2), a, mvc, mvp2, ref_idx, &mv);
      mv_arr[index] = mv; mv_arr[index + 2] = mv;
      mvp2 = mv_arr[0];
    }
  } else {
    a.width = size / 2; a.height = size / 2;
    for (int index = 0; index < 4; index++) {
      int px = index & 1, py = index >> 1;
      a.pu_x = xpos + px * (size / 2); a.pu_y = ypos + py * (size / 2);
      sad += motion_estimate<PIX, SP>(t, ws->mep, org + py * (size / 2) * ostride + px * (size / 2),
                             ref_y + py * (size / 2) * ref.sy + px * (size / 2), a, mvc, mvp2, ref_idx, &mv);
      mv_arr[index] = mv;
      mvp2 = mv_arr[0];
    }
  }
  return sad;
}

template <typename PIX> TK_DEV void add_cands4(const Team t, WsP<PIX> ws, int ref_idx, const mv_t* mv4) {
  if (t.rank == 0)
    for (int i = 0; i < 4; i++) add_mvcand(ws->mep, ref_idx, mv4[i]);
  t.sync();
}

template <typename PIX, int SP>
TK_DEV void build_org8(const Team t, PIX* o8_, const PIX* oy_, int osy, const PIX* py_, int size, int bitdepth) {
#ifndef TK_NOVEC
  const int S = (int)sizeof(PIX);
  const unsigned al = (unsigned)(uintptr_t)o8_ | (unsigned)(uintptr_t)oy_ | (unsigned)(uintptr_t)py_ | (unsigned)(osy * S);
  if (tk_uniform(!(al & (unsigned)(4 * S - 1)))) {
    const int ppr = size >> 2, lg = ilog2((unsigned)ppr);
    for (int k = t.rank; k < ppr * size; k += t.size) {
      const int i = k >> lg, j = (k & (ppr - 1)) << 2;
      int o[4], p[4];
      load_samples<SP, PIX, 4>(oy_ + i * osy + j, o);
      load_samples<SP, PIX, 4>(py_ + i * size + j, p);
      for (int q = 0; q < 4; q++) o[q] = sat_pix(2 * o[q] - p[q], bitdepth);
      store_samples<SP, PIX, 4>(o8_ + i * size + j, o);
    }
    return;
  }
#endif
  const auto o8 = spc<SP>(o8_);
  const auto oys = spc<SP>(oy_);
  const auto pys = spc<SP>(py_);
  for (int k = t.rank; k < size * size; k += t.size) {
    int i, j;
    split2(mk_pow2(size), k, i, j);
    o8[k] = (PIX)sat_pix(2 * (int)oys[i * osy + j] - (int)pys[k], bitdepth);
  }
}

template <typename PIX, int SP>
TK_DEVNI void search_bipred(const Team t, JobR<PIX> J, WsP<PIX> ws, const Node& nd_, int part,
                          const mv_t* mv_center, mv_t mvp, int* ref_idx0, int* ref_idx1, mv_t* mv_arr0, mv_t* mv_arr1) {
  const auto& c = J.cfg;
  const NodePos nd = node_pos(&nd_);
  const auto lists = ldsc(lds_ld(&ws->mep->lists));
  const int size = nd.size;
  const int num_iter = c.encoder_speed == 0 ? 2 : 1;
  int min_ref0 = (J.frame_type == F_B && J.interp_ref > 0) ? 1 : 0, min_ref1 = 0;
  mv_t min0[4], min1[4];
  for (int i = 0; i < 4; i++) { min0[i] = mvp; min1[i] = mvp; }
  unsigned min_sad = 1u << 30;
  const PIX* oy = ws->org_y;
  const int osy = ws->org_sy;
  int prev_ref[2] = {-1, -1}, prev_cnt[2][kMaxRefs];
  mv_t prev_mv[2][4];
  for (int n = 0; n < num_iter; n++) {
    const int stop = part == 0 ? 0 : 1;
    for (int list = 1; list >= stop; list--) {
      mv_t mvo = list ? min0[0] : min1[0];
      int ref_o = list ? min_ref0 : min_ref1;
      {
        const mv_t* mo = list ? min0 : min1;
        int same = n > 0 && prev_ref[list] == ref_o;
        for (int i = 0; i < 4; i++) same = same && prev_mv[list][i].x == mo[i].x && prev_mv[list][i].y == mo[i].y;
        for (int r = 0; r < J.num_ref; r++) {
          const int cnt = lists->mvcand_num[r];
          same = same && prev_cnt[list][r] == cnt;
          prev_cnt[list][r] = cnt;
        }
        prev_ref[list] = ref_o;
        for (int i = 0; i < 4; i++) prev_mv[list][i] = mo[i];
        if (tk_uniform(same)) continue;
      }
      pred_inter_yuv<SP>(t, lds_ld(&J.ref[ref_o]), ws->pred_y, ws->pred_u, ws->pred_v, nd.ypos, nd.xpos, size, nd.bw, nd.bh,
                     list ? min0 : min1, J.sign[ref_o], c.width, c.height, c.enable_bipred, part > 0, c.bitdepth, 1);
      t.sync();
      build_org8<PIX, SP>(t, ws->org8, oy, osy, ws->pred_y, size, c.bitdepth);
      t.sync();
      int ref_start, ref_end;
      if (J.frame_type == F_P) { ref_start = 0; ref_end = J.num_ref - 1; }
      else {
        ref_start = ref_end = list ? 1 : 0;
        if (J.interp_ref) { ref_start++; ref_end++; }
      }
      for (int r = ref_start; r <= ref_end; r++) {
        mv_t mvp2 = (J.frame_type == F_B && list == 1) ? mvo : mvp;
        mv_t mv_all[4];
        unsigned sad = search_inter<PIX, SP>(t, J, ws, nd.ypos, nd.xpos, size, ws->org8, size, r, mv_center[r], mvp2, mv_all, part, J.sign[r]);
        add_cands4(t, ws, r, mv_all);
        if (sad < min_sad) {
          min_sad = sad;
          if (list) { min_ref1 = r; for (int i = 0; i < 4; i++) min1[i] = mv_all[i]; }
          else { min_ref0 = r; for (int i = 0; i < 4; i++) min0[i] = mv_all[i]; }
        }
      }
    }
  }
  *ref_idx0 = min_ref0;
  *ref_idx1 = min_ref1;
  for (int i = 0; i < 4; i++) { mv_arr0[i] = min0[i]; mv_arr1[i] = min1[i]; }
}

template <typename PIX, int SP>
TK_DEVNI unsigned intra_sad_search(const Team t, JobR<PIX> J, WsP<PIX> ws, const Node& nd, int num_modes, int* mode_out) {
  const auto& c = J.cfg;
  const int size = nd.size, bd = c.bitdepth;
  const int ur = upright_avail(nd.ypos, nd.xpos, size, size, c.width, sb_size_of(c));
  const int dl = downleft_avail(nd.ypos, nd.xpos, size, size, c.height, sb_size_of(c));
  const PIX* fy = J.rec.y + nd.ypos * J.rec.sy + nd.xpos;
  const PIX* oy = ws->org_y;
  const int osy = ws->org_sy;
  make_edges<SP>(t, ws->edgep, fy, J.rec.sy, (const PIX*)nullptr, 0, 0, 0, nd.ypos, nd.xpos, size, ur, dl, 0, bd);
  t.sync();
  unsigned min_sad = 1u << 30;
  int best = 0;
  const int n = num_modes == 4 ? 4 : 10;
  for (int e = 0; e < n; e++) {
    const int m = e == 0 ? 0 : e == 1 ? 2 : e == 2 ? 3 : e == 3 ? 1 : e;
    pred_intra<SP>(t, ws->edgep, 1, 1, size, ws->pred_y, size, m, bd);
    t.sync();
    int local = 0;
    for (int k = t.rank; k < size * size; k += t.size) {
      int i, j;
      split2(mk_pow2(size), k, i, j);
      local += iabs((int)spc<SP>(oy)[i * osy + j] - (int)spc<SP>(ws->pred_y)[k]);
    }
    const unsigned sad = (unsigned)team_sum(t, local) >> (bd - 8);
    t.sync();
    if (sad < min_sad) { min_sad = sad; best = m; }
  }
  *mode_out = best;
  return min_sad;
}
}
```

### thor_amd/csrc/tk_common.h

```cpp
#pragma once
#include <stdint.h>
#include <stddef.h>
#if defined(THOR_HOSTSIM)
#include <string.h>
#include <stdlib.h>
#include <stdio.h>
#include <sched.h>
#define TK_DEV static inline
#define TK_HD static inline
#define TK_CONST static const
#define TK_HOST 1
#else
#include <hip/hip_runtime.h>
#define TK_DEV __device__ __forceinline__
#define TK_HD __host__ __device__ __forceinline__
#define TK_DEVNI __device__ __noinline__
#define TK_CONST __device__ const
#define TK_HOST 0
#endif
#if TK_HOST
#define TK_DEVNI static
#endif
#if TK_HOST
#define TK_UNROLL
#else
#define TK_UNROLL _Pragma("unroll")
#endif
#if defined(THOR_PROF) && !TK_HOST
#define TK_PROF_DEV 1
#else
#define TK_PROF_DEV 0
#endif
#if TK_PROF_DEV && !defined(THOR_PROF_NOMACROS)
#define TK_PROF_MACROS 1
#else
#define TK_PROF_MACROS 0
#endif
#if TK_PROF_DEV && defined(THOR_PROF_ME)
#define TK_PROF_ME 1
#else
#define TK_PROF_ME 0
#endif
#if TK_PROF_DEV && defined(THOR_PROF_MD)
#define TK_PROF_MD 1
#else
#define TK_PROF_MD 0
#endif
#if TK_PROF_DEV && defined(THOR_PROF_SUBPEL)
#define TK_PROF_SUBPEL 1
#else
#define TK_PROF_SUBPEL 0
#endif
#if defined(TK_MDW_INLINE)
#define TK_MDW TK_DEV
#else
#define TK_MDW TK_DEVNI
#endif

namespace tk {

#if TK_HOST && defined(THOR_HOSTSIM_LANES)
namespace hostlanes {
void barrier();
const unsigned long long* exchange_begin(unsigned long long v);
void exchange_end();
int lanes();
int rank();
}
#define TK_LANES 1
#else
#define TK_LANES 0
#endif

struct Team {
  int rank;
#if TK_HOST
  int size;
#else
  static constexpr int size = 64;
#endif
  const int16_t* izz = nullptr;
#if TK_LANES
  inline void sync() const { hostlanes::barrier(); }
  inline void block_sync() const { hostlanes::barrier(); }
#elif TK_HOST
  inline void sync() const {}
  inline void block_sync() const {}
#else
  __device__ __forceinline__ void sync() const {
    __builtin_amdgcn_fence(__ATOMIC_RELEASE, "workgroup");
    __builtin_amdgcn_wave_barrier();
    __builtin_amdgcn_fence(__ATOMIC_ACQUIRE, "workgroup");
  }
  __device__ __forceinline__ void block_sync() const { __syncthreads(); }
#endif
};

TK_DEV Team mk_team(int rank, int size, const int16_t* izz = nullptr) {
  Team t;
  t.rank = rank;
#if TK_HOST
  t.size = size;
#else
  (void)size;
#endif
  t.izz = izz;
  return t;
}
#if !TK_HOST
struct BlockTeam {
  int rank;
  int size;
  __device__ __forceinline__ void block_sync() const { __syncthreads(); }
};
#endif

#if !TK_HOST
#ifndef TK_WAVES
#define TK_WAVES 4
#endif
enum { kWaves = TK_WAVES };
#elif defined(THOR_HOSTSIM_WAVES)
enum { kWaves = THOR_HOSTSIM_WAVES };
#else
enum { kWaves = 1 };
#endif
#if TK_HOST && defined(THOR_HOSTSIM_WAVES)
namespace hostwaves { void barrier(); }
#endif
struct Wg {
  int wave, nwaves;
#if TK_PROF_DEV
  long long* prof;
  __device__ __forceinline__ void barrier() const {
    const long long t0 = (long long)__builtin_readcyclecounter();
    __syncthreads();
    if ((threadIdx.x & 63) == 0) prof[26] += (long long)__builtin_readcyclecounter() - t0;
  }
#elif !TK_HOST
  __device__ __forceinline__ void barrier() const { __syncthreads(); }
#elif defined(THOR_HOSTSIM_WAVES)
  inline void barrier() const { hostwaves::barrier(); }
#else
  inline void barrier() const {}
#endif
};
TK_DEV int wg_fetch_add(int* p, int v) {
#if TK_HOST
  return __atomic_fetch_add(p, v, __ATOMIC_ACQ_REL);
#else
  return __hip_atomic_fetch_add((__attribute__((address_space(3))) int*)p, v, __ATOMIC_ACQ_REL, __HIP_MEMORY_SCOPE_WORKGROUP);
#endif
}
TK_DEV void wg_min64(unsigned long long* p, unsigned long long v) {
#if TK_HOST
  unsigned long long cur = __atomic_load_n(p, __ATOMIC_RELAXED);
  while (v < cur && !__atomic_compare_exchange_n(p, &cur, v, true, __ATOMIC_ACQ_REL, __ATOMIC_RELAXED)) {}
#else
  __hip_atomic_fetch_min((__attribute__((address_space(3))) unsigned long long*)p, v, __ATOMIC_RELAXED, __HIP_MEMORY_SCOPE_WORKGROUP);
#endif
}
TK_DEV int wg_load_acquire(const int* p) {
#if TK_HOST
  return __atomic_load_n(p, __ATOMIC_ACQUIRE);
#else
  return __hip_atomic_load((const __attribute__((address_space(3))) int*)p, __ATOMIC_ACQUIRE, __HIP_MEMORY_SCOPE_WORKGROUP);
#endif
}
TK_DEV void wg_store_release(int* p, int v) {
#if TK_HOST
  __atomic_store_n(p, v, __ATOMIC_RELEASE);
#else
  __hip_atomic_store((__attribute__((address_space(3))) int*)p, v, __ATOMIC_RELEASE, __HIP_MEMORY_SCOPE_WORKGROUP);
#endif
}
TK_DEV int wg_cas(int* p, int expected, int desired) {
#if TK_HOST
  return __atomic_compare_exchange_n(p, &expected, desired, false, __ATOMIC_ACQ_REL, __ATOMIC_ACQUIRE) ? 1 : 0;
#else
  return __hip_atomic_compare_exchange_strong((__attribute__((address_space(3))) int*)p, &expected, desired, __ATOMIC_ACQ_REL, __ATOMIC_ACQUIRE,
                                              __HIP_MEMORY_SCOPE_WORKGROUP) ? 1 : 0;
#endif
}
TK_DEV void wg_pause() {
#if TK_HOST
  sched_yield();
#else
  __builtin_amdgcn_s_sleep(8);
#endif
}
#if TK_HOST
}
#include <time.h>
namespace tk {
#endif
#if TK_HOST
static inline unsigned long long wg_wait_limit() {
  static const unsigned long long lim = [] { const char* e = getenv("THOR_HOSTSIM_WAIT_S"); return (unsigned long long)((e && atof(e) > 0 ? atof(e) : 120.0) * 1e8); }();
  return lim;
}
#define kWgWaitLimit wg_wait_limit()
#else
enum { kWgWaitLimit = 800000000 };
#endif
// ... 523 lines not shown
```

### thor_amd/csrc/tk_me.h

```cpp
#pragma once
#include "tk_me_seg.h"
#include "tk_me_lanes.h"
#include "tk_me_fastsub.h"

namespace tk {

template <typename PIX>
TK_DEV void me_stage_cb_window(const Team t, MeWs* w_, const PIX* ref_cb, int rstride, int cb_x, int cb_y, int cb, mv_t mvc, int sign, int fwidth,
                               int fheight, int ref_idx) {
  const auto w = ldsc(w_);
  const int S = (int)sizeof(PIX), s = sign ? -1 : 1;
  const int cap = TKU(w->win_cap);
  int R = kMeWinR;
  while (R >= kMeWinRmin && me_win_bytes(cb, cb, R, S) > cap) R -= 4;
  const mv_t mv_ref = mk_mv(((mvc.x + 2) >> 2) << 2, ((mvc.y + 2) >> 2) << 2);
  const int Ww = cb + 2 * R, Wh = cb + 2 * R, pitch = Ww * S + 4;
  const int ox = s * (mv_ref.x >> 2) - R, oy = s * (mv_ref.y >> 2) - R;
  const int ok = TKU(w->win != nullptr && R >= kMeWinRmin && cb_x + ox >= -kPadY && cb_x + ox + Ww <= fwidth + kPadY && cb_y + oy >= -kPadY &&
                     cb_y + oy + Wh <= fheight + kPadY);
  t.sync();
  if (ok) {
    const uint32_t* w32 = lds_ld(&w_->win);
    const int rowb = Ww * S, spr = (rowb + 15) >> 4, total = spr * Wh;
    for (int k0 = 0; k0 < total; k0 += t.size) {
      const int k = k0 + t.rank;
      if (k < total) {
        const int row = k / spr, sg = k - row * spr;
        const Seg16 v = seg_load<SP_GLOBAL, 16>((const char*)(ref_cb + (oy + row) * rstride + ox) + 16 * sg);
        const int d = (row * pitch + 16 * sg) >> 2;
        const int nd = tmin(4, (rowb - 16 * sg) >> 2);
#if TK_HOST
        for (int q = 0; q < nd; q++) ((uint32_t*)w32)[d + q] = v.d[q];
#else
        TK_LDS uint32_t* l = (TK_LDS uint32_t*)(uint32_t)(uintptr_t)w32 + d;
        l[0] = v.d[0];
        if (nd > 1) l[1] = v.d[1];
        if (nd > 2) l[2] = v.d[2];
        if (nd > 3) l[3] = v.d[3];
#endif
      }
    }
  }
  if (t.rank == 0) {
    w->cwin_valid = ok; w->cwin_ref = ref_idx; w->cwin_ax = cb_x + ox; w->cwin_ay = cb_y + oy; w->cwin_Ww = Ww; w->cwin_Wh = Wh; w->cwin_pitch = pitch;
  }
  t.sync();
}

template <typename PIX, int SP>
TK_DEVNI unsigned motion_estimate(const Team t, MeWs* w_, const PIX* org, const PIX* ref, const MeArgs& a_in, mv_t mvc,
                                mv_t mvp, int ref_idx, mv_t* mv_out) {
  TK_PROF_T0();
#if TK_PROF_ME
  const long long pme0_ = (long long)__builtin_readcyclecounter();
#endif
  const auto w = ldsc(w_);
  const auto lists = ldsc(lds_ld(&w_->lists));
  const auto orgs = spc<SP>(org);
  auto cmv_get = [&](int c) -> mv_t { return mk_mv(w->cmv[c].x, w->cmv[c].y); };
  auto cmv_set = [&](int c, mv_t m) { w->cmv[c].x = m.x; w->cmv[c].y = m.y; };
  const MeArgs a = uniform(a_in);
  mvc = uniform(mvc);
  mvp = uniform(mvp);
  ref_idx = tk_uniform(ref_idx);
  const int s = a.sign ? -1 : 1;
  const int sh = a.bitdepth - 8;
  unsigned min_sad = kCostInit;
  mv_t mv_opt = mk_mv(0, 0);
  mv_t mv_ref = mk_mv(((mvc.x + 2) >> 2) << 2, ((mvc.y + 2) >> 2) << 2);
  struct FP { mv_t mv; const PIX* p; int dx, dy; unsigned rate; };
  auto rate_of = [&](mv_t m) -> unsigned { return mv_cost(a.lam, m.y - mvp.y, m.x - mvp.x); };
  auto fp_cost = [&](const FP& x, int sad) -> unsigned { return ((unsigned)sad >> sh) + x.rate; };
  auto clip_free = [&](mv_t ctr, int R) -> int {
    const int ext = kPadY - 16, cy = s * ctr.y, cx = s * ctr.x;
    return a.ypos + ((cy - R) >> 2) >= -ext && a.ypos + ((cy + R + 3) >> 2) + a.cb_size <= a.fheight + ext &&
           a.xpos + ((cx - R) >> 2) >= -ext && a.xpos + ((cx + R + 3) >> 2) + a.cb_size <= a.fwidth + ext;
  };
  auto mk_fp = [&](mv_t mv, int noclip) -> FP {
    FP x;
    x.mv = noclip ? mv : clip_mv(mv, a.ypos, a.xpos, a.fwidth, a.fheight, a.cb_size, a.cb_size, a.sign);
    x.dx = s * (x.mv.x >> 2);
    x.dy = s * (x.mv.y >> 2);
    x.p = ref + mul24(x.dy, a.rstride) + x.dx;
    x.rate = rate_of(x.mv);
    return x;
  };
#if TK_PROF_MACROS
  long long pq_ = (long long)__builtin_readcyclecounter();
  if (t.rank == 0) w->prof[11] += 1;
#endif
  MeWin win;
  win.on = 0; win.w32 = nullptr; win.ox = win.oy = win.Ww = win.Wh = win.pitch = 0;
  const int use_cb_win = TKU(w->cwin_valid && w->cwin_ref == ref_idx && a.speed == 0);
  if (use_cb_win) {
    win.Ww = TKU(w->cwin_Ww); win.Wh = TKU(w->cwin_Wh); win.pitch = TKU(w->cwin_pitch);
    win.ox = TKU(w->cwin_ax) - a.pu_x; win.oy = TKU(w->cwin_ay) - a.pu_y;
    win.w32 = lds_ld(&w_->win);
    win.on = 1;
  } else {
    const int S = (int)sizeof(PIX);
    const int cap = TKU(w->win_cap);
    int R = kMeWinR;
    while (R >= kMeWinRmin && me_win_bytes(a.width, a.height, R, S) > cap) R -= 4;
    if (w->win && R >= kMeWinRmin && a.speed == 0) {
      win.Ww = a.width + 2 * R; win.Wh = a.height + 2 * R; win.pitch = win.Ww * S + 4;
      win.ox = s * (mv_ref.x >> 2) - R; win.oy = s * (mv_ref.y >> 2) - R;
      win.w32 = lds_ld(&w_->win);
      win.on = TKU(a.pu_x + win.ox >= -kPadY && a.pu_x + win.ox + win.Ww <= a.fwidth + kPadY && a.pu_y + win.oy >= -kPadY &&
                   a.pu_y + win.oy + win.Wh <= a.fheight + kPadY);
    }
    if (win.on) {
      const int rowb = win.Ww * S;
      const int spr = (rowb + 15) >> 4, total = spr * win.Wh;
      t.sync();
      for (int k0 = 0; k0 < total; k0 += t.size) {
        const int k = k0 + t.rank;
        if (k < total) {
          const int row = k / spr, sg = k - row * spr;
          const Seg16 v = seg_load<SP_GLOBAL, 16>((const char*)(ref + (win.oy + row) * a.rstride + win.ox) + 16 * sg);
          const int d = (row * win.pitch + 16 * sg) >> 2;
          const int nd = tmin(4, (rowb - 16 * sg) >> 2);
#if TK_HOST
          for (int q = 0; q < nd; q++) ((uint32_t*)win.w32)[d + q] = v.d[q];
#else
          TK_LDS uint32_t* l = (TK_LDS uint32_t*)(uint32_t)(uintptr_t)win.w32 + d;
          l[0] = v.d[0];
          if (nd > 1) l[1] = v.d[1];
          if (nd > 2) l[2] = v.d[2];
          if (nd > 3) l[3] = v.d[3];
#endif
        }
      }
      t.sync();
    }
  }
  auto eval_wide = [&](int n) -> unsigned long long {
    unsigned long long bestk = ~0ull;
    for (int base = 0; base < n; base += kMeWideChunk) {
      const int m = n - base < kMeWideChunk ? n - base : kMeWideChunk;
      auto widepel = [&](int c5) -> FP {
        int c = mul24(c5, 13) >> 6, o = c5 - c - (c << 2);
        int off = o == 0 ? -3 : o == 1 ? -1 : o == 2 ? 0 : o == 3 ? 1 : 3;
        FP x;
        x.mv = cmv_get(base + c);
        x.dx = s * (x.mv.x >> 2) + off;
        x.dy = s * (x.mv.y >> 2);
        x.p = ref + mul24(x.dy, a.rstride) + x.dx;
        x.rate = 0;
        return x;
      };
      {
        const auto sadl = ldsc(w_->sad);
        seg_sads<SP>(t, m * 5, org, a.ostride, a.rstride, a.width, a.height, win, widepel, [&](int c5, const FP&, int sad, int mine) { if (mine) sadl[c5] = sad; });
      }
      t.sync();
      unsigned long long k = ~0ull;
      for (int lc = t.rank; lc < m; lc += t.size) {
        const int c = base + lc;
        mv_t mm = cmv_get(c);
        int x = 0;
        unsigned best = 1u << 31;
        for (int o = 0; o < 5; o++) {
          unsigned v = (unsigned)w->sad[lc * 5 + o];
          if (v < best) { best = v; x = o == 0 ? -3 : o == 1 ? -1 : o == 2 ? 0 : o == 3 ? 1 : 3; }
        }
        mm.x = (int16_t)(mm.x + ((s * x) << 2));
        cmv_set(c, mm);
        unsigned long long kk = ((unsigned long long)((best >> sh) + mv_cost(a.lam, mm.y - mvp.y, mm.x - mvp.x)) << 32) | (unsigned)c;
        k = kk < k ? kk : k;
      }
      t.sync();
      k = TKU64(team_min64(t, k));
      bestk = k < bestk ? k : bestk;
    }
    return bestk;
  };
  mv_t g_ctr = mk_mv(0, 0);
  int g_step = 0;
  mv_t gc32 = mk_mv(0, 0), gc16 = mk_mv(0, 0), gc8 = mk_mv(0, 0);
  auto on_grid_of = [&](mv_t m, mv_t ctr, int gs) -> int {
    const int dx = m.x - ctr.x, dy = m.y - ctr.y;
    return !((dx | dy) & (gs - 1)) && iabs(dx) <= 2 * gs && iabs(dy) <= 2 * gs;
  };
  auto on_any_grid = [&](mv_t m) -> int {
    return g_step == 4 && (on_grid_of(m, gc32, 32) | on_grid_of(m, gc16, 16) | on_grid_of(m, gc8, 8) | on_grid_of(m, g_ctr, 4));
  };
  auto on_grid = [&](mv_t m) -> int {
    const int dx = m.x - g_ctr.x, dy = m.y - g_ctr.y;
    return g_step && !((dx | dy) & (g_step - 1)) && iabs(dx) <= 2 * g_step && iabs(dy) <= 2 * g_step;
  };
  const int lw_ = (a.width < 16 / (int)sizeof(PIX)) ? a.width : 16 / (int)sizeof(PIX);
  const int dedup = a.speed == 0 && a.height * (a.width / lw_) >= 16;
  int small_done = 0;
  {
    if (TKU(a.speed == 0 && t.size == 64 && a.width <= 32 && a.height <= 32)) {
#ifndef TK_ME_NO_SMALL
      unsigned long long fr;
#define TK_ME_FP_ARGS t, w_, org, ref, a.cb_size, a.ostride, a.width, a.height, a.rstride, a.sign, a.fwidth, a.fheight, a.xpos, a.ypos, a.lam, win.w32, win.ox, win.oy, win.Ww, win.Wh, win.pitch, win.on, mvc, mvp, ref_idx, sh
      const int rowb = a.width * (int)sizeof(PIX);
      if (rowb == 4) { if constexpr (sizeof(PIX) == 1) fr = me_cand_fullpel<PIX, 4, SP>(TK_ME_FP_ARGS); else fr = 0; }
      else if (rowb == 8) fr = me_cand_fullpel<PIX, 8, SP>(TK_ME_FP_ARGS);
      else fr = me_cand_fullpel<PIX, 16, SP>(TK_ME_FP_ARGS);
#undef TK_ME_FP_ARGS
      min_sad = (unsigned)(fr >> 32);
      mv_opt = mk_mv((int16_t)(uint16_t)(fr >> 16), (int16_t)(uint16_t)fr);
      mv_ref = mv_opt;
      small_done = 1;
#endif
    }
  }
#ifdef TK_ME_CROSSCHECK
  const int xs_have = small_done;
  const unsigned xs_min = min_sad;
  const mv_t xs_mv = mv_opt;
  if (small_done) { small_done = 0; min_sad = kCostInit; mv_opt = mk_mv(0, 0); mv_ref = mk_mv(((mvc.x + 2) >> 2) << 2, ((mvc.y + 2) >> 2) << 2); }
#endif
  if (!small_done) {
  if ((a.cb_size == 16 && a.enable_bipred) || a.speed == 0)
  for (int step = 32; step >= 4; step >>= 1) {
    const int n = step < 32 ? 24 : 25;
    const mv_t centre = mv_ref;
    const int noclip = TKU(clip_free(centre, 2 * step));
    auto tele_mv = [&](int c) -> mv_t {
      int idx = (step < 32 && c >= 12) ? c + 1 : c;
      int q = mul24(idx, 13) >> 6;
      return mk_mv(centre.x + mul24(idx - q - (q << 2) - 2, step), centre.y + mul24(q - 2, step));
    };
    auto tele = [&](int c) -> FP { return mk_fp(tele_mv(c), noclip); };
    if (dedup && g_step) {
      t.sync();
      int cnt = 0;
      for (int c0 = 0; c0 < n; c0 += t.size) {
        const int c = c0 + t.rank;
        const mv_t m = tele_mv(c < n ? c : 0);
        const int keep = c < n && !on_grid(m);
        const unsigned long long mask = team_ballot(t, keep);
        if (keep) cmv_set(cnt + __builtin_popcountll(mask & ((1ull << t.rank) - 1ull)), mk_fp(m, noclip).mv);
        cnt += __builtin_popcountll(mask);
      }
      t.sync();
      cnt = TKU(cnt);
      auto cl = [&](int c) -> FP { return mk_fp(cmv_get(c), 1); };
      unsigned long long k = eval_fullpel<SP>(t, cnt, org, a.ostride, a.rstride, a.width, a.height, win, cl, fp_cost);
      if ((unsigned)(k >> 32) < min_sad) { min_sad = (unsigned)(k >> 32); mv_opt = cmv_get((int)(unsigned)k); }
      t.sync();
    } else
    if (step == 32 && a.cb_size == 16 && a.speed == 1) {
      t.sync();
      for (int c = t.rank; c < n; c += t.size) cmv_set(c, tele(c).mv);
      t.sync();
      unsigned long long k = eval_wide(n);
      if ((unsigned)(k >> 32) < min_sad) { min_sad = (unsigned)(k >> 32); mv_opt = cmv_get((int)(unsigned)k); }
      t.sync();
    } else {
      unsigned long long k = eval_fullpel<SP>(t, n, org, a.ostride, a.rstride, a.width, a.height, win, tele, fp_cost);
      if ((unsigned)(k >> 32) < min_sad) { min_sad = (unsigned)(k >> 32); mv_opt = tele((int)(unsigned)k).mv; }
    }
    g_ctr = centre; g_step = a.speed == 0 ? step : 0;
    if (step == 32) gc32 = centre; else if (step == 16) gc16 = centre; else if (step == 8) gc8 = centre;
    mv_ref = mv_opt;
  }

#if TK_PROF_MACROS
  if (t.rank == 0) w->prof[13] += (long long)__builtin_readcyclecounter() - pq_;
  pq_ = (long long)__builtin_readcyclecounter();
#endif
  {
    const int n = TKU(lists->mvcand_num[ref_idx]);
    if (n > 0) {
      const int wide = a.cb_size == 16;
      for (int c = t.rank; c < n; c += t.size) {
        const mv_t m = mk_mv(lists->mvcand[ref_idx][c].x, lists->mvcand[ref_idx][c].y);
        cmv_set(c, clip_mv(mk_mv(m.x << 2, m.y << 2), a.ypos, a.xpos, a.fwidth, a.fheight, a.cb_size, a.cb_size, a.sign));
      }
      t.sync();
      if (wide) {
        unsigned long long bestk = eval_wide(n);
        if ((unsigned)(bestk >> 32) < min_sad) { min_sad = (unsigned)(bestk >> 32); mv_opt = cmv_get((int)(unsigned)bestk); }
        t.sync();
      } else {
        int cnt = n;
        if (a.speed == 0) {
          cnt = 0;
          for (int c0 = 0; c0 < n; c0 += t.size) {
            const int c = c0 + t.rank;
            const mv_t m = cmv_get(c < n ? c : 0);
// ... 408 lines not shown
```

### thor_amd/csrc/tk_me_lanes.h

```cpp
#pragma once
#include "tk_me_seg.h"

namespace tk {
template <typename PIX, int NB, int SP>
TK_DEVNI unsigned long long me_cand_fullpel(const Team t, MeWs* w_, const PIX* org_, const PIX* ref, int a_cb, int a_ostride, int a_width, int a_height,
                                            int a_rstride, int a_sign, int a_fw, int a_fh, int a_xpos, int a_ypos, double a_lam, const uint32_t* win_w32, int win_ox,
                                            int win_oy, int win_Ww, int win_Wh, int win_pitch, int win_on, mv_t mvc, mv_t mvp, int ref_idx, int a_sh) {
  constexpr int S = (int)sizeof(PIX), SPS = 16 / S;
  const int sh = tk_uniform(a_sh);
  MeWin win_in;
  win_in.w32 = win_w32; win_in.ox = win_ox; win_in.oy = win_oy; win_in.Ww = win_Ww; win_in.Wh = win_Wh; win_in.pitch = win_pitch; win_in.on = win_on;
  const auto lists = ldsc(lds_ld(&w_->lists));
  const int cb = tk_uniform(a_cb), ostride = tk_uniform(a_ostride), width = tk_uniform(a_width), height = tk_uniform(a_height);
  const int rstride = tk_uniform(a_rstride), sign = tk_uniform(a_sign), fw = tk_uniform(a_fw), fh = tk_uniform(a_fh);
  const int xpos = tk_uniform(a_xpos), ypos = tk_uniform(a_ypos);
  const double lam = tk_uniform_f64(a_lam);
  const MeWin win = uniform(win_in);
  mvc = uniform(mvc);
  mvp = uniform(mvp);
  ref_idx = tk_uniform(ref_idx);
  org_ = tk_uniform_ptr(org_);
  ref = tk_uniform_ptr(ref);
  const int s = sign ? -1 : 1;
  const int spr = NB == 16 ? ((width * S) >> 4) : 1;
// ... 68 lines not shown
    const int c = t.rank - lo;
    unsigned k = (cost << 8) | (unsigned)(c & 0xff);
    if (c < 0 || c >= n || cost == ~0u) k = ~0u;
    return team_min32(t, k);
  };
  struct NoWide { enum { value = 0 }; };
  struct Wide { enum { value = 1 }; };
  auto grid_mv = [&](mv_t centre, int step, int c) -> mv_t {
    const int idx = (step < 32 && c >= 12) ? c + 1 : c;
    const int q = mul24(idx, 13) >> 6;
    return mk_mv(centre.x + mul24(idx - q - (q << 2) - 2, step), centre.y + mul24(q - 2, step));
  };
  auto take = [&](mv_t m) {
    m = clip_mv(m, ypos, xpos, fw, fh, cb, cb, sign);
    mv_opt = mk_mv(tk_uniform(m.x), tk_uniform(m.y));
  };
  for (int step = 32; step >= 4;) {
#ifdef TK_ME_NOSPEC
    const int n1 = step < 32 ? 24 : 25, n2 = 0;
#else
    const int n1 = step < 32 ? 24 : 25, n2 = step > 4 ? 24 : 0;
#endif
    const mv_t centre = mv_ref;
    const int c1 = t.rank, c2 = t.rank - n1;
    const int v1 = c1 < n1, v2 = c2 >= 0 && c2 < n2;
    const mv_t m = v2 ? grid_mv(centre, step >> 1, c2) : grid_mv(centre, step, v1 ? c1 : 0);
    const unsigned cost = lane_cost(m, v1 || v2, NoWide(), nullptr);
    const unsigned k1 = range_min(cost, 0, n1);
    if (k1 != ~0u && (k1 >> 8) < min_sad) { min_sad = k1 >> 8; take(grid_mv(centre, step, (int)(k1 & 0xffu))); }
    mv_ref = mv_opt;
    step >>= 1;
    if (n2 && mv_ref.x == centre.x && mv_ref.y == centre.y) {
      const unsigned k2 = range_min(cost, n1, n2);
      if (k2 != ~0u && (k2 >> 8) < min_sad) { min_sad = k2 >> 8; take(grid_mv(centre, step, (int)(k2 & 0xffu))); }
      mv_ref = mv_opt;
      step >>= 1;
    }
  }
  {
    const int n = TKU(lists->mvcand_num[ref_idx]);
    if (n > 0) {
      auto list_mv = [&](int c) -> mv_t { return mk_mv((int16_t)(lists->mvcand[ref_idx][c].x << 2), (int16_t)(lists->mvcand[ref_idx][c].y << 2)); };
      const int valid = t.rank < n;
      const mv_t m = list_mv(valid ? t.rank : 0);
      if (cb == 16) {
        unsigned osel = 0;
        const unsigned cost = lane_cost(m, valid, Wide(), &osel);
        const unsigned k = range_min(cost, 0, n);
        if (k != ~0u && (k >> 8) < min_sad) {
          min_sad = k >> 8;
          const int c = (int)(k & 0xffu);
          const int q = team_read_lane(t, (int)osel, c);
          mv_t mm = clip_mv(list_mv(c), ypos, xpos, fw, fh, cb, cb, sign);
          const int bx = q == 0 ? -3 : q == 1 ? -1 : q == 2 ? 0 : q == 3 ? 1 : 3;
          mm.x = (int16_t)(mm.x + ((s * bx) << 2));
          mv_opt = mk_mv(tk_uniform(mm.x), tk_uniform(mm.y));
        }
      } else {
        const unsigned cost = lane_cost(m, valid, NoWide(), nullptr);
        const unsigned k = range_min(cost, 0, n);
        if (k != ~0u && (k >> 8) < min_sad) { min_sad = k >> 8; take(list_mv((int)(k & 0xffu))); }
      }
    }
    mv_ref = mv_opt;
  }
  {
    auto hex_off = [&](int dir, int* ox, int* oy) {
      *ox = dir == 0 ? 1 : dir == 1 ? 2 : dir == 2 ? 1 : dir == 3 ? -1 : dir == 4 ? -2 : -1;
      *oy = dir == 0 ? -1 : dir == 1 ? 0 : dir == 2 ? 1 : dir == 3 ? 1 : dir == 4 ? 0 : -1;
    };
    int start = 0, end = 5;
    for (int round = 1; round < 6;) {
      const int n = (end - start + 6) % 6 + 1;
      const mv_t centre = mv_ref;
      const int L = t.rank;
      int ox, oy, valid = L < n * 4;
      mv_t m;
      {
        const int j = L < n ? L : mul24(L - n, 11) >> 5;
        const int dir1 = (start + (j < n ? j : 0)) % 6;
        hex_off(dir1, &ox, &oy);
        m = mk_mv(centre.x + ox * 4, centre.y + oy * 4);
        if (L >= n) {
          const int st2 = dir1 ? dir1 - 1 : 5;
          const int dir2 = (st2 + (L - n - mul24(j, 3))) % 6;
          hex_off(dir2, &ox, &oy);
          m = mk_mv(m.x + ox * 4, m.y + oy * 4);
        }
      }
#ifdef TK_ME_NOSPEC
      const int speculate = 0;
#else
      const int speculate = round < 5;
#endif
      if (!speculate) valid = L < n;
      const unsigned cost = lane_cost(m, valid, NoWide(), nullptr);
      int which = -1;
      const unsigned k = range_min(cost, 0, n);
      auto hex_mv = [&](mv_t ctr, int st, int c) -> mv_t { int x, y; hex_off((st + c) % 6, &x, &y); return mk_mv(ctr.x + x * 4, ctr.y + y * 4); };
      if (k != ~0u && (k >> 8) < min_sad) { min_sad = k >> 8; which = (int)(k & 0xffu); take(hex_mv(centre, start, which)); }
      int best_dir = which < 0 ? -1 : (start + which) % 6;
      const mv_t raw = which < 0 ? centre : hex_mv(centre, start, which);
      mv_ref = mv_opt;
      const int start0 = start;
      start = best_dir ? best_dir - 1 : 5;
      end = start + 2;
      end -= (end >= 6) * 6;
      round++;
      if (best_dir < 0) break;
      if (speculate && round < 6 && raw.x == mv_ref.x && raw.y == mv_ref.y) {
        (void)start0;
        const mv_t centre2 = mv_ref;
        const unsigned k2 = range_min(cost, n + 3 * which, 3);
        int which2 = -1;
        if (k2 != ~0u && (k2 >> 8) < min_sad) { min_sad = k2 >> 8; which2 = (int)(k2 & 0xffu); take(hex_mv(centre2, start, which2)); }
        best_dir = which2 < 0 ? -1 : (start + which2) % 6;
        mv_ref = mv_opt;
        start = best_dir ? best_dir - 1 : 5;
        end = start + 2;
        end -= (end >= 6) * 6;
        round++;
        if (best_dir < 0) break;
      }
    }
  }
  return ((unsigned long long)min_sad << 32) | ((unsigned long long)(uint16_t)mv_opt.x << 16) | (unsigned long long)(uint16_t)mv_opt.y;
}


template <int SP>
TK_DEVNI unsigned me_cand8_subpel(const Team t, const uint8_t* org_, int a_ostride, int a_width, int a_height, int a_sign, int a_fw, int a_fh, int a_xpos, int a_ypos,
                                  int a_bipred, double a_lam, const uint32_t* win_w32, int win_ox, int win_oy, int win_Ww, int win_Wh, int win_pitch, int win_on, mv_t base,
                                  int d, mv_t mvp) {
  enum : unsigned { kNone = 0xffffffffu };
  struct { int ostride, width, height, sign, fwidth, fheight, xpos, ypos, enable_bipred; double lam; } a_in = {a_ostride, a_width, a_height, a_sign, a_fw, a_fh, a_xpos, a_ypos, a_bipred, a_lam};
  MeWin win_in;
  win_in.w32 = win_w32; win_in.ox = win_ox; win_in.oy = win_oy; win_in.Ww = win_Ww; win_in.Wh = win_Wh; win_in.pitch = win_pitch; win_in.on = win_on;
  const int ostride = tk_uniform(a_in.ostride), width = tk_uniform(a_in.width), height = tk_uniform(a_in.height), sign = tk_uniform(a_in.sign);
  const int fw = tk_uniform(a_in.fwidth), fh = tk_uniform(a_in.fheight), xpos = tk_uniform(a_in.xpos), ypos = tk_uniform(a_in.ypos);
  const int bip = tk_uniform(a_in.enable_bipred);
  const double lam = tk_uniform_f64(a_in.lam);
  const MeWin win = uniform(win_in);
  base = uniform(base);
  mvp = uniform(mvp);
  d = tk_uniform(d);
  org_ = tk_uniform_ptr(org_);
  if (!win.on) return kNone;
  const int c = t.rank >> 3, part = t.rank & 7;
  const int oy = c == 0 ? 0 : c == 1 ? -d : c == 2 ? d : c == 3 ? 0 : c == 4 ? -d : c == 5 ? -d : d;
  const int ox = c == 0 ? -d : c == 1 ? 0 : c == 2 ? 0 : c == 3 ? d : c == 4 ? -d : c == 5 ? d : c == 6 ? -d : d;
  const mv_t mv = mk_mv(base.x + ox, base.y + oy);
  const SubPel sp = luma_setup(mv, sign, width, height, fw, fh, xpos, ypos, bip);
  const int centre = sp.ver_frac == 2 && sp.hor_frac == 2 && bip < 2;
  const int outside = !(sp.hor_int - 2 >= win.ox && sp.hor_int + width + 6 <= win.ox + win.Ww && sp.ver_int - 2 >= win.oy && sp.ver_int + height + 3 <= win.oy + win.Wh);
  if (team_ballot(t, outside) != 0ull) return kNone;
  const int dual = team_ballot(t, centre) != 0ull;
  const unsigned long long thA = centre ? 0x0000000001010000ull : sp.ph, thB = centre ? 0x0000000102020100ull : sp.ph;
  const int biasA = centre ? 128 * 2 : 128 * 64, biasB = centre ? 128 * 6 : 128 * 64;
  int tv[6];
  for (int m = 0; m < 6; m++) tv[m] = centre ? (m >= 1 && m <= 4 ? 1 : 0) : sp.tv[m];
  const int rnd = centre ? 8 : 2048, rsh = centre ? 4 : 12;
  const int lgw = ilog2((unsigned)width);
  const int SH = height == 4 ? 4 : 8;
  const int units = width * (height == 4 ? 1 : (height >> 3));
  unsigned sad = 0;
  auto strip = [&](auto sh_tag, auto dual_tag, int i0, int j) {
    constexpr int SHC = decltype(sh_tag)::value, DUAL = decltype(dual_tag)::value, NR = SHC + 5;
    const int woff = mul24(i0 + sp.ver_int - 2 - win.oy, win.pitch) + (j + sp.hor_int - 2 - win.ox);
    int hA[NR], hB[NR];
    TK_UNROLL
    for (int r = 0; r < NR; r++) {
      const Seg16 sg = win_seg<8>(win.w32, woff + mul24(r, win.pitch));
      const unsigned lo = sg.d[0] ^ 0x80808080u, hi = sg.d[1] ^ 0x80808080u;
      hA[r] = dot4_i8((int)(unsigned)thA, (int)lo, dot4_i8((int)(unsigned)(thA >> 32), (int)hi, biasA));
      if constexpr (DUAL) hB[r] = dot4_i8((int)(unsigned)thB, (int)lo, dot4_i8((int)(unsigned)(thB >> 32), (int)hi, biasB));
      else hB[r] = hA[r];
    }
    TK_UNROLL
    for (int q = 0; q < SHC; q++) {
      int sum = mul24(tv[0], hA[q]) + mul24(tv[1], hA[q + 1]) + mul24(tv[2], hB[q + 2]) + mul24(tv[3], hB[q + 3]) + mul24(tv[4], hA[q + 4]) + mul24(tv[5], hA[q + 5]);
      const int pr = sat_pix((sum + rnd) >> rsh, 8);
      const int o = (int)spc<SP>(org_)[mul24(i0 + q, ostride) + j];
      sad += (unsigned)(o > pr ? o - pr : pr - o);
    }
  };
  struct S4 { enum { value = 4 }; };
  struct S8 { enum { value = 8 }; };
  struct D0 { enum { value = 0 }; };
  struct D1 { enum { value = 1 }; };
  for (int u = part; u < units; u += 8) {
    const int j = u & (width - 1), i0 = (u >> lgw) << 3;
    if (SH == 4) { if (dual) strip(S4(), D1(), 0, j); else strip(S4(), D0(), 0, j); }
    else { if (dual) strip(S8(), D1(), i0, j); else strip(S8(), D0(), i0, j); }
  }
  const unsigned tot = (unsigned)team_group_sum(t, (int)sad, 8);
  const unsigned cost = tot + mv_cost(lam, mv.y - mvp.y, mv.x - mvp.x);
  unsigned k = (cost << 8) | (unsigned)c;
  if (part != 0) k = ~0u;
  return team_min32(t, k);
}


template <int SP>
TK_DEVNI unsigned me_cand16_subpel(const Team t, const uint16_t* org_, int a_ostride, int a_width, int a_height, int a_sign, int a_fw, int a_fh, int a_xpos, int a_ypos,
                                   int a_bipred, double a_lam, const uint32_t* win_w32, int win_ox, int win_oy, int win_Ww, int win_Wh, int win_pitch, int win_on, mv_t base,
                                   int d, mv_t mvp, int a_bitdepth) {
  enum : unsigned { kNone = 0xffffffffu };
  struct { int ostride, width, height, sign, fwidth, fheight, xpos, ypos, enable_bipred, bitdepth; double lam; } a_in = {a_ostride, a_width, a_height, a_sign, a_fw, a_fh, a_xpos, a_ypos, a_bipred, a_bitdepth, a_lam};
  MeWin win_in;
  win_in.w32 = win_w32; win_in.ox = win_ox; win_in.oy = win_oy; win_in.Ww = win_Ww; win_in.Wh = win_Wh; win_in.pitch = win_pitch; win_in.on = win_on;
  const int ostride = tk_uniform(a_in.ostride), width = tk_uniform(a_in.width), height = tk_uniform(a_in.height), sign = tk_uniform(a_in.sign);
  const int fw = tk_uniform(a_in.fwidth), fh = tk_uniform(a_in.fheight), xpos = tk_uniform(a_in.xpos), ypos = tk_uniform(a_in.ypos);
  const int bip = tk_uniform(a_in.enable_bipred), bitdepth = tk_uniform(a_in.bitdepth);
  const double lam = tk_uniform_f64(a_in.lam);
  const MeWin win = uniform(win_in);
  base = uniform(base);
  mvp = uniform(mvp);
  d = tk_uniform(d);
  org_ = tk_uniform_ptr(org_);
  if (!win.on) return kNone;
  const int c = t.rank >> 3, part = t.rank & 7;
  const int oy = c == 0 ? 0 : c == 1 ? -d : c == 2 ? d : c == 3 ? 0 : c == 4 ? -d : c == 5 ? -d : d;
  const int ox = c == 0 ? -d : c == 1 ? 0 : c == 2 ? 0 : c == 3 ? d : c == 4 ? -d : c == 5 ? d : c == 6 ? -d : d;
  const mv_t mv = mk_mv(base.x + ox, base.y + oy);
  const SubPel sp = luma_setup(mv, sign, width, height, fw, fh, xpos, ypos, bip);
  const int centre = sp.ver_frac == 2 && sp.hor_frac == 2 && bip < 2;
  const int outside = !(sp.hor_int - 2 >= win.ox && sp.hor_int + width + 6 <= win.ox + win.Ww && sp.ver_int - 2 >= win.oy && sp.ver_int + height + 3 <= win.oy + win.Wh);
  if (team_ballot(t, outside) != 0ull) return kNone;
  const int dual = team_ballot(t, centre) != 0ull;
  auto pair = [](int a, int b) -> uint32_t { return (uint32_t)(uint16_t)(int16_t)a | ((uint32_t)(uint16_t)(int16_t)b << 16); };
  uint32_t tA[3], tB[3];
  for (int q = 0; q < 3; q++) {
    tA[q] = centre ? (q == 1 ? pair(1, 1) : 0u) : pair(sp.th[2 * q], sp.th[2 * q + 1]);
    tB[q] = centre ? (q == 0 ? pair(0, 1) : q == 1 ? pair(2, 2) : pair(1, 0)) : pair(sp.th[2 * q], sp.th[2 * q + 1]);
  }
  int tv[6];
  for (int m = 0; m < 6; m++) tv[m] = centre ? (m >= 1 && m <= 4 ? 1 : 0) : sp.tv[m];
  const int rnd = centre ? 8 : 2048, rsh = centre ? 4 : 12;
  const int lgw = ilog2((unsigned)width);
  const int SH = height == 4 ? 4 : 8;
  const int units = width * (height == 4 ? 1 : (height >> 3));
  unsigned sad = 0;
  auto strip = [&](auto sh_tag, auto dual_tag, int i0, int j) {
    constexpr int SHC = decltype(sh_tag)::value, DUAL = decltype(dual_tag)::value, NR = SHC + 5;
    const int woff = mul24(i0 + sp.ver_int - 2 - win.oy, win.pitch) + ((j + sp.hor_int - 2 - win.ox) << 1);
    int hA[NR], hB[NR];
    TK_UNROLL
    for (int r = 0; r < NR; r++) {
      const Seg16 sg = win_seg<12>(win.w32, woff + mul24(r, win.pitch));
      hA[r] = dot2_i16(tA[0], sg.d[0], dot2_i16(tA[1], sg.d[1], dot2_i16(tA[2], sg.d[2], 0)));
      if constexpr (DUAL) hB[r] = dot2_i16(tB[0], sg.d[0], dot2_i16(tB[1], sg.d[1], dot2_i16(tB[2], sg.d[2], 0)));
      else hB[r] = hA[r];
    }
    TK_UNROLL
    for (int q = 0; q < SHC; q++) {
      int sum = mul24(tv[0], hA[q]) + mul24(tv[1], hA[q + 1]) + mul24(tv[2], hB[q + 2]) + mul24(tv[3], hB[q + 3]) + mul24(tv[4], hA[q + 4]) + mul24(tv[5], hA[q + 5]);
      const int pr = sat_pix((sum + rnd) >> rsh, bitdepth);
      const int o = (int)spc<SP>(org_)[mul24(i0 + q, ostride) + j];
      sad += (unsigned)(o > pr ? o - pr : pr - o);
    }
  };
  struct S4 { enum { value = 4 }; };
  struct S8 { enum { value = 8 }; };
  struct D0 { enum { value = 0 }; };
  struct D1 { enum { value = 1 }; };
  for (int u = part; u < units; u += 8) {
    const int j = u & (width - 1), i0 = (u >> lgw) << 3;
    if (SH == 4) { if (dual) strip(S4(), D1(), 0, j); else strip(S4(), D0(), 0, j); }
    else { if (dual) strip(S8(), D1(), i0, j); else strip(S8(), D0(), i0, j); }
  }
  const unsigned tot = (unsigned)team_group_sum(t, (int)sad, 8);
  const unsigned cost = (tot >> (bitdepth - 8)) + mv_cost(lam, mv.y - mvp.y, mv.x - mvp.x);
  unsigned k = (cost << 8) | (unsigned)c;
  if (part != 0) k = ~0u;
  return team_min32(t, k);
}
}
```

### thor_amd/csrc/tk_xform.h

```cpp
#pragma once
#include "tk_common.h"

#ifndef TK_PROF_T0
#if TK_PROF_MACROS
#ifdef THOR_PROF_WALL
#define TK_CYC() ((long long)wall_clock64())
#else
#define TK_CYC() ((long long)__builtin_readcyclecounter())
#endif
#define TK_PROF_T0() long long pt0_ = TK_CYC()
#define TK_PROF_ADD(ws, id) do { if (t.rank == 0) (ws)->prof[id] += TK_CYC() - pt0_; } while (0)
#define TK_PROF_MARK(v) long long v = TK_CYC()
#define TK_PROF_ACC(ws, id, v) do { if (t.rank == 0) (ws)->prof[id] += TK_CYC() - (v); } while (0)
#define TK_PROF_CNT(ws, id) do { if (t.rank == 0) (ws)->prof[id] += 1; } while (0)
#else
#define TK_PROF_T0() do {} while (0)
#define TK_PROF_ADD(ws, id) do {} while (0)
#define TK_PROF_MARK(v) do {} while (0)
#define TK_PROF_ACC(ws, id, v) do {} while (0)
#define TK_PROF_CNT(ws, id) do {} while (0)
#endif
#endif

namespace tk {
// ... 274 lines not shown
    if (jj >= 0) carry = (int)((mV >> jj) & 1ull);
  }
  t.sync();
  return cbp;
}

template <int SC>
TK_DEV void dequantize(const Team t, XformWs* ws, const int16_t* coefq_, int qp, int size) {
  const auto coefq = spc<SC>(coefq_);
  const int qsize = size < kMaxQuant ? size : kMaxQuant;
  const int lshift = qp / 6, rshift = ilog2(size) - 1;
  const int64_t scale = dequant_scale(qp % 6);
  lds_i16* const rcoef = TK_LDS_PTR(ws->coef);
  const int lgq = ilog2((unsigned)qsize);
  for (int k = t.rank; k < qsize * qsize; k += t.size) {
    int64_t c = coefq[k];
    int16_t r;
    if (lshift >= rshift) r = (int16_t)((c * scale) << (lshift - rshift));
    else r = (int16_t)((c * scale + ((int64_t)1 << (rshift - lshift - 1))) >> (rshift - lshift));
    rcoef[((k & (qsize - 1)) << lgq) + (k >> lgq)] = r;
  }
  t.sync();
}

template <typename PIX, int SP>
TK_DEV void inv_transform_recon(const Team t, XformWs* ws, const PIX* pred_, int pstride, PIX* rec_, int rstride,
                                int size, int bitdepth) {
  const auto pred = spc<SP>(pred_);
  const auto rec = spc<SP>(rec_);
  const int n = size < 32 ? size : 32;
  const int scale = size / n;
  const int qsize = n < kMaxQuant ? n : kMaxQuant;
  const int rs = 5 - ilog2((unsigned)n);
  lds_i16* const itmp = TK_LDS_PTR(ws->in);
  const lds_i16* const mt = TK_DCTT(t, ws) + dctT_off(n);
  const lds_i16* const rcoef = TK_LDS_PTR(ws->coef);
  const int shift_2 = 20 - bitdepth, add_2 = 1 << (shift_2 - 1);
  const Pow2 dn = mk_pow2(n);
  (void)rs;
  for (int k = t.rank; k < qsize * n; k += t.size) {
    int i, j;
    split2(dn, k, i, j);
    const int sum = dot_i16(mt + j * n, rcoef + i * qsize, qsize, j);
    itmp[j * qsize + i] = (int16_t)clampi((sum + 64) >> 7, -32768, 32767);
  }
  t.sync();
#ifndef TK_NOVEC
  {
    const int S = (int)sizeof(PIX);
    const unsigned al = (unsigned)(uintptr_t)pred_ | (unsigned)(uintptr_t)rec_ | (unsigned)(pstride * S) | (unsigned)(rstride * S);
    const int step = scale == 1 ? 4 : scale;
    if (tk_uniform(!(al & (unsigned)(step * S - 1)))) {
      if (scale == 1) {
        const int ppr = n >> 2, lg = ilog2((unsigned)ppr);
        for (int k = t.rank; k < ppr * n; k += t.size) {
          const int i = k >> lg, j = (k & (ppr - 1)) << 2;
          int p[4];
          load_samples<SP, PIX, 4>(pred_ + i * pstride + j, p);
          TK_UNROLL
          for (int q = 0; q < 4; q++) {
            const int sum = dot_i16(mt + (j + q) * n, itmp + i * qsize, qsize, j + q);
            p[q] = sat_pix(clampi((sum + add_2) >> shift_2, -32768, 32767) + p[q], bitdepth);
          }
          store_samples<SP, PIX, 4>(rec_ + i * rstride + j, p);
        }
      } else {
        for (int k = t.rank; k < n * n; k += t.size) {
          int i, j;
          split2(dn, k, i, j);
          const int sum = dot_i16(mt + j * n, itmp + i * qsize, qsize, j);
          const int r = clampi((sum + add_2) >> shift_2, -32768, 32767);
          const PIX* p = pred_ + scale * i * pstride + scale * j;
          PIX* o = rec_ + scale * i * rstride + scale * j;
          if (scale == 2) box_recon<SP, PIX, 2>(r, p, pstride, o, rstride, bitdepth);
          else if (scale == 4) box_recon<SP, PIX, 4>(r, p, pstride, o, rstride, bitdepth);
          else box_recon<SP, PIX, 8>(r, p, pstride, o, rstride, bitdepth);
        }
      }
      t.sync();
      return;
    }
  }
#endif
  for (int k = t.rank; k < n * n; k += t.size) {
    int i, j;
    split2(dn, k, i, j);
    const int sum = dot_i16(mt + j * n, itmp + i * qsize, qsize, j);
    int r = clampi((sum + add_2) >> shift_2, -32768, 32767);
    for (int m = 0; m < scale; m++)
      for (int x = 0; x < scale; x++) {
        int yy = scale * i + m, xx = scale * j + x;
        rec[yy * rstride + xx] = (PIX)sat_pix(r + (int)pred[yy * pstride + xx], bitdepth);
      }
  }
  t.sync();
}

template <int SD, int SS, int V> TK_DEV void copy_rows_vec(const Team t, void* dst_, int dpitch, const void* src_, int spitch, int rowbytes, int h) {
  const int ppr = rowbytes / V;
#if TK_HOST
  for (int k = t.rank; k < ppr * h; k += t.size) {
    const int i = k / ppr, j = k - i * ppr;
    __builtin_memcpy((char*)dst_ + (size_t)i * dpitch + j * V, (const char*)src_ + (size_t)i * spitch + j * V, V);
  }
#else
  typedef uint32_t __attribute__((ext_vector_type(V / 4))) vec_t;
  const auto dst = spc<SD>((char*)dst_);
  const auto src = spc<SS>((const char*)src_);
  const int lg = (ppr & (ppr - 1)) ? -1 : ilog2((unsigned)ppr);
  for (int k = t.rank; k < ppr * h; k += t.size) {
    int i, j;
    if (lg >= 0) { i = k >> lg; j = k & (ppr - 1); } else { i = k / ppr; j = k - i * ppr; }
    *(typename SpT<SD, vec_t>::ptr)(dst + i * dpitch + j * V) = *(typename SpT<SS, const vec_t>::ptr)(src + i * spitch + j * V);
  }
#endif
}
template <int SD, int SS, typename PIX>
TK_DEV void copy_block(const Team t, PIX* dst_, int dstride, const PIX* src_, int sstride, int w, int h) {
  dst_ = tk_uniform_ptr(dst_); src_ = tk_uniform_ptr(src_); dstride = tk_uniform(dstride); sstride = tk_uniform(sstride); w = tk_uniform(w); h = tk_uniform(h);
  const int S = (int)sizeof(PIX);
#ifdef TK_NOVEC
  const unsigned al = 1u;
#else
  const unsigned al = (unsigned)(uintptr_t)dst_ | (unsigned)(uintptr_t)src_ | (unsigned)(dstride * S) | (unsigned)(sstride * S) | (unsigned)(w * S);
#endif
  if (!(al & 15u)) { copy_rows_vec<SD, SS, 16>(t, dst_, dstride * S, src_, sstride * S, w * S, h); return; }
  if (!(al & 7u)) { copy_rows_vec<SD, SS, 8>(t, dst_, dstride * S, src_, sstride * S, w * S, h); return; }
  if (!(al & 3u)) { copy_rows_vec<SD, SS, 4>(t, dst_, dstride * S, src_, sstride * S, w * S, h); return; }
  const auto dst = spc<SD>(dst_);
  const auto src = spc<SS>(src_);
  if ((w & (w - 1)) == 0) {
    const Pow2 pw = mk_pow2(w);
    for (int k = t.rank; k < w * h; k += t.size) {
      int i, j;
      split2(pw, k, i, j);
      dst[i * dstride + j] = src[i * sstride + j];
    }
  } else {
    for (int k = t.rank; k < w * h; k += t.size) {
      int i = k / w, j = k - i * w;
      dst[i * dstride + j] = src[i * sstride + j];
    }
  }
}

template <typename PIX, int SP, int SC>
TK_DEVNI int code_tu_sp(const Team t, XformWs* ws, const PIX* org, int ostride, const PIX* pred, int pstride, PIX* rec,
                   int rstride, int size, int qp, int coeff_type, int fast, int16_t* coefq, int bitdepth) {
  org = tk_uniform_ptr(org); pred = tk_uniform_ptr(pred); rec = tk_uniform_ptr(rec); coefq = tk_uniform_ptr(coefq); ws = tk_uniform_ptr(ws);
  ostride = tk_uniform(ostride); pstride = tk_uniform(pstride); rstride = tk_uniform(rstride); size = tk_uniform(size);
  qp = tk_uniform(qp); coeff_type = tk_uniform(coeff_type); fast = tk_uniform(fast); bitdepth = tk_uniform(bitdepth);
  TK_PROF_T0();
  fwd_transform<PIX, SP>(t, ws, org, ostride, pred, pstride, size, fast, bitdepth);
  TK_PROF_ADD(ws, 30);
  TK_PROF_MARK(pq0_);
  int cbp = quantize_team<SC>(t, ws, coefq, qp, size, (coeff_type >> 1) & 1);
  TK_PROF_ACC(ws, 12, pq0_);
  if (cbp) {
    TK_PROF_MARK(pi0_);
    dequantize<SC>(t, ws, coefq, qp, size);
    inv_transform_recon<PIX, SP>(t, ws, pred, pstride, rec, rstride, size, bitdepth);
    TK_PROF_ACC(ws, 31, pi0_);
  } else {
    copy_block<SP, SP>(t, rec, rstride, pred, pstride, size, size);
    t.sync();
  }
#if !defined(THOR_PROF_ME) && !defined(THOR_PROF_MD)
  TK_PROF_ADD(ws, (size <= 4 ? 16 : size == 8 ? 17 : size == 16 ? 18 : size == 32 ? 19 : 20));
  TK_PROF_CNT(ws, (size <= 4 ? 21 : size == 8 ? 22 : size == 16 ? 23 : size == 32 ? 24 : 25));
#endif
  TK_PROF_ADD(ws, 6);
  return cbp;
}
template <typename PIX>
TK_DEV int code_tu(const Team t, XformWs* ws, const PIX* org, int ostride, const PIX* pred, int pstride, PIX* rec,
                   int rstride, int size, int qp, int coeff_type, int fast, int16_t* coefq, int bitdepth) {
  const int lb = tk_uniform(tk_is_lds(pred)), lc = tk_uniform(tk_is_lds(coefq));
  if (lb) return code_tu_sp<PIX, SP_LDS, SP_LDS>(t, ws, org, ostride, pred, pstride, rec, rstride, size, qp, coeff_type, fast, coefq, bitdepth);
  if (lc) return code_tu_sp<PIX, SP_GLOBAL, SP_LDS>(t, ws, org, ostride, pred, pstride, rec, rstride, size, qp, coeff_type, fast, coefq, bitdepth);
  return code_tu_sp<PIX, SP_GLOBAL, SP_GLOBAL>(t, ws, org, ostride, pred, pstride, rec, rstride, size, qp, coeff_type, fast, coefq, bitdepth);
}

}
```

Baseline: 164.0.

## Reuse staged ME reference window across searches and tighten subpel window bounds

Motion estimation now remembers which reference window is staged in LDS (ref, origin, size). A later CB-window staging with identical parameters skips the global-to-LDS copy, and a whole-CB search records its window as valid so it can be reused. Explicit window invalidation is added around the bipred, queue and MD search loops to keep correctness. Subpel 'outside' checks are relaxed to the exact filter footprint, so more candidates use the LDS path. A kernel for sequential ME testing and profiling hooks are also added. The risk is stale-window bugs if invalidation misses a path.

```diff
diff --git a/include/thor_hip.h b/include/thor_hip.h
--- a/include/thor_hip.h
+++ b/include/thor_hip.h
@@ -117,6 +117,8 @@
 
 int thor_hip_kat_motion_estimate(const void* cur, const void* ref, int width, int height, int bitdepth, int n, const int* par, const double* lambda,
                                  const int16_t* cand, int ncand_total, int* out);
+int thor_hip_kat_motion_estimate_seq(const void* ref0, const void* ref1, int width, int height, int bitdepth, int n, int k, const int* par, const double* lambda,
+                                     const int16_t* cand, int ncand_total, const void* orgs, const int* ref_idx, int* out);
 int thor_hip_kat_motion_estimate_bi(const void* cur, const void* ref0, const void* ref1, int width, int height, int bitdepth, int n, const int* par,
                                     const double* lambda, const int16_t* cand, int* out, int16_t* list_out);
 int thor_hip_kat_early_skip(const int* chroma, const void* org, const void* pred, const int* size, const int* qp, const float* thr, int bitdepth, int n, int* out);
diff --git a/thor_amd/binding.py b/thor_amd/binding.py
--- a/thor_amd/binding.py
+++ b/thor_amd/binding.py
@@ -426,6 +426,19 @@
     return out
 
 
+def kat_motion_estimate_seq(ref0, ref1, par, lam, cand, orgs, ref_idx, bitdepth=8):
+    T = _pix(bitdepth)
+    ref0 = np.ascontiguousarray(ref0, dtype=T); ref1 = np.ascontiguousarray(ref1, dtype=T); orgs = np.ascontiguousarray(orgs, dtype=T)
+    par = np.ascontiguousarray(par, dtype=np.int32); lam = np.ascontiguousarray(lam, dtype=np.float64); cand = np.ascontiguousarray(cand, dtype=np.int16).reshape(-1, 2)
+    ref_idx = np.ascontiguousarray(ref_idx, dtype=np.int32)
+    n, K = ref_idx.shape
+    assert ref0.shape == ref1.shape and par.shape == (n, 17) and len(lam) == n and orgs.shape == (n, K, 4096)
+    out = np.full((n, K, 3), -1, dtype=np.int32)
+    _kat('thor_hip_kat_motion_estimate_seq', _vp(ref0), _vp(ref1), ref0.shape[1], ref0.shape[0], bitdepth, n, K, _vp(par), _vp(lam), _vp(cand), len(cand), _vp(orgs), _vp(ref_idx),
+         _vp(out))
+    return out
+
+
 def kat_motion_estimate_bi(cur, ref0, ref1, par, lam, cand, bitdepth=8):
     T = _pix(bitdepth)
     cur, ref0, ref1 = (np.ascontiguousarray(a, dtype=T) for a in (cur, ref0, ref1))
diff --git a/thor_amd/csrc/hip_kat.h b/thor_amd/csrc/hip_kat.h
--- a/thor_amd/csrc/hip_kat.h
+++ b/thor_amd/csrc/hip_kat.h
@@ -134,6 +134,42 @@
   if (bi && lane < 6) { list_out[12 * it + 2 * lane] = lists->mvcand[0][lane].x; list_out[12 * it + 2 * lane + 1] = lists->mvcand[0][lane].y; }
 }
 template <typename PIX>
+__global__ __launch_bounds__(kWgThreads, (sizeof(PIX) == 1 ? (int)kOcc : 2)) void k_kat_me_seq(int K, Plane3<PIX> ref0, Plane3<PIX> ref1, int fw, int fh, int bitdepth, const int* par, const double* lam,
+                                                                                               const int16_t* cand, const PIX* orgs, const int* ridx, unsigned char* big, int* out) {
+  __shared__ WgShared sh;
+  __shared__ SmallWs<PIX> sws;
+  const int lane = (int)threadIdx.x, it = (int)blockIdx.x;
+  TeamWs<PIX> ws = make_ws(&sws, &sh, (BigWs<PIX>*)big);
+  const Team t = mk_team(lane, 64, sh.tabs.izz);
+  xform_tables_fill(&sh.tabs, lane, 64);
+  const int* q = par + kKatMePar * it;
+  const int cbx = q[0], cby = q[1], cb = q[2], pux = cbx + q[3], puy = cby + q[4], pw = q[5], ph = q[6];
+  MeLists* lists = &sh.lists;
+  const int lds_blk = __builtin_amdgcn_readfirstlane(cb <= kLdsBlk);
+  PIX* orgc = (PIX*)sh.org_raw;
+  MeArgs a;
+  a.cb_size = cb; a.ostride = pw; a.width = pw; a.height = ph; a.rstride = ref0.sy; a.sign = q[11]; a.fwidth = fw; a.fheight = fh;
+  a.xpos = cbx; a.ypos = cby; a.pu_x = pux; a.pu_y = puy; a.enable_bipred = q[12]; a.bitdepth = bitdepth; a.speed = q[13]; a.lam = lam[it];
+  const mv_t mvc = mk_mv(q[7], q[8]), mvp = mk_mv(q[9], q[10]);
+  for (int k = 0; k < K; k++) {
+    const int r = __builtin_amdgcn_readfirstlane(ridx[it * K + k]);
+    const Plane3<PIX> rf = r ? ref1 : ref0;
+    const PIX* og = orgs + (size_t)(it * K + k) * 4096;
+    __syncthreads();
+    for (int c = lane; c < q[14]; c += 64) { lists->mvcand[r][c].x = cand[2 * (q[15] + c)]; lists->mvcand[r][c].y = cand[2 * (q[15] + c) + 1]; }
+    if (lane == 0) { lists->mvcand_num[r] = q[14]; lists->mvcand_mask[r] = 0; lists->best_ref = 0; }
+    if (lds_blk)
+      for (int c = lane; c < pw * ph; c += 64) orgc[c] = og[c];
+    __syncthreads();
+    if (k == 0 && q[16]) me_stage_cb_window<PIX>(t, ws.mep, rf.y + (size_t)cby * rf.sy + cbx, rf.sy, cbx, cby, cb, mvc, a.sign, fw, fh, r);
+    const PIX* rp = rf.y + (size_t)puy * rf.sy + pux;
+    mv_t mv = mk_mv(0, 0);
+    const unsigned cost = lds_blk ? motion_estimate<PIX, SP_LDS>(t, ws.mep, orgc, rp, a, mvc, mvp, r, &mv) : motion_estimate<PIX, SP_GLOBAL>(t, ws.mep, og, rp, a, mvc, mvp, r, &mv);
+    __syncthreads();
+    if (lane == 0) { out[3 * (it * K + k)] = mv.x; out[3 * (it * K + k) + 1] = mv.y; out[3 * (it * K + k) + 2] = (int)cost; }
+  }
+}
+template <typename PIX>
 __global__ __launch_bounds__(kWgThreads, (sizeof(PIX) == 1 ? (int)kOcc : 2)) void k_kat_early_skip(const int* chroma, const PIX* org, const PIX* pred, const int* size, const int* qp,
                                                                                                    const float* thr, int bitdepth, unsigned char* big, int* out) {
   __shared__ FrameJob<PIX> sJ;
@@ -469,6 +505,40 @@
   return 0;
 }
 template <typename PIX>
+int kat_me_seq(const PIX* ref0, const PIX* ref1, int width, int height, int bitdepth, int n, int K, const int* par, const double* lam, const int16_t* cand, int ncand_total,
+               const PIX* orgs, const int* ridx, int* out) {
+  if (!ref0 || !ref1 || !par || !lam || !orgs || !ridx || !out || n <= 0 || K < 1 || K > 8 || ncand_total < 0 || (ncand_total && !cand) || width % 8 || height % 8 || width < 16 ||
+      height < 16 || width > 8192 || height > 8192)
+    return 1;
+  auto pow2 = [](int v, int lo, int hi) { return v >= lo && v <= hi && !(v & (v - 1)); };
+  for (int i = 0; i < n; i++) {
+    const int* q = par + kKatMePar * i;
+    if (!pow2(q[2], 8, 64) || !pow2(q[5], 4, q[2]) || !pow2(q[6], 4, q[2]) || (q[11] & ~1) || (q[12] & ~1) || q[13] < 0 || q[13] > 2 || !(lam[i] >= 0.0 && lam[i] <= 1e6)) return 1;
+    if (q[0] < 0 || q[1] < 0 || q[0] + q[2] > width || q[1] + q[2] > height || q[3] < 0 || q[4] < 0 || q[3] + q[5] > q[2] || q[4] + q[6] > q[2] || q[3] % 4 || q[4] % 4) return 2;
+    for (int k = 7; k <= 10; k++) if (q[k] < -8192 || q[k] > 8192) return 1;
+    if (q[14] < 0 || q[14] > 64 || q[15] < 0 || q[15] + q[14] > ncand_total) return 2;
+    for (int c = 0; c < q[14]; c++) if (cand[2 * (q[15] + c)] < -2047 || cand[2 * (q[15] + c)] > 2047 || cand[2 * (q[15] + c) + 1] < -2047 || cand[2 * (q[15] + c) + 1] > 2047) return 1;
+    for (int k = 0; k < K; k++) if (ridx[i * K + k] & ~1) return 1;
+  }
+  if (!ensure_init_any()) return 3;
+  DevFrame<PIX> f0 = kat_luma_frame(ref0, width, height, 1), f1 = kat_luma_frame(ref1, width, height, 1);
+  {
+    DevBuf<int> d_par((size_t)kKatMePar * n, par), d_r((size_t)n * K, ridx);
+    DevBuf<double> d_lam(n, lam);
+    DevBuf<int16_t> d_cand((size_t)2 * (ncand_total ? ncand_total : 1));
+    if (ncand_total) backend::h2d(d_cand, cand, (size_t)4 * ncand_total);
+    DevBuf<PIX> d_org((size_t)n * K * 4096 + 16, nullptr);
+    backend::h2d(d_org, orgs, (size_t)n * K * 4096 * sizeof(PIX));
+    DevBuf<unsigned char> d_big(sizeof(BigWs<PIX>));
+    DevBuf<int> d_o((size_t)3 * n * K);
+    hipLaunchKernelGGL(k_kat_me_seq<PIX>, dim3(n), dim3(64), 0, g_stream, K, f0.p, f1.p, width, height, bitdepth, d_par, d_lam, d_cand, d_org, d_r, d_big, d_o);
+    HIPCHECK(hipGetLastError());
+    backend::d2h(out, d_o, (size_t)3 * n * K * 4);
+  }
+  f0.release(); f1.release();
+  return 0;
+}
+template <typename PIX>
 int kat_early_skip(const int* chroma, const PIX* org, const PIX* pred, const int* size, const int* qp, const float* thr, int bitdepth, int n, int* out) {
   if (!chroma || !org || !pred || !size || !qp || !thr || !out || n <= 0) return 1;
   for (int i = 0; i < n; i++) {
@@ -526,6 +596,11 @@
                                                const double* lambda, const int16_t* cand, int* out, int16_t* list_out) {
   KAT_BD(kat_me<uint8_t>(1, (const uint8_t*)cur, (const uint8_t*)ref0, (const uint8_t*)ref1, width, height, 8, n, par, lambda, cand, 6 * n, out, list_out),
          kat_me<uint16_t>(1, (const uint16_t*)cur, (const uint16_t*)ref0, (const uint16_t*)ref1, width, height, bitdepth, n, par, lambda, cand, 6 * n, out, list_out));
+}
+extern "C" int thor_hip_kat_motion_estimate_seq(const void* ref0, const void* ref1, int width, int height, int bitdepth, int n, int k, const int* par, const double* lambda,
+                                                const int16_t* cand, int ncand_total, const void* orgs, const int* ref_idx, int* out) {
+  KAT_BD(kat_me_seq<uint8_t>((const uint8_t*)ref0, (const uint8_t*)ref1, width, height, 8, n, k, par, lambda, cand, ncand_total, (const uint8_t*)orgs, ref_idx, out),
+         kat_me_seq<uint16_t>((const uint16_t*)ref0, (const uint16_t*)ref1, width, height, bitdepth, n, k, par, lambda, cand, ncand_total, (const uint16_t*)orgs, ref_idx, out));
 }
 extern "C" int thor_hip_kat_early_skip(const int* chroma, const void* org, const void* pred, const int* size, const int* qp, const float* thr, int bitdepth, int n, int* out) {
   KAT_BD(kat_early_skip<uint8_t>(chroma, (const uint8_t*)org, (const uint8_t*)pred, size, qp, thr, 8, n, out),
diff --git a/thor_amd/csrc/tk_block_md.h b/thor_amd/csrc/tk_block_md.h
--- a/thor_amd/csrc/tk_block_md.h
+++ b/thor_amd/csrc/tk_block_md.h
@@ -61,12 +61,14 @@
         nd.syn.mvp = mvp;
         mv_center[r] = mvp;
         unsigned sad_inter = 0xffffffffu;
+        me_drop_window(t, ws->mep);
         for (int part = 0; part < max_pb; part++) {
           unsigned sad = search_inter<PIX, SP>(t, J, ws, nd.ypos, nd.xpos, size, oy, ws->org_sy, r, mv_center[r], mvp, mv_all[part], part, J.sign[r]);
           add_cands4(t, ws, r, mv_all[part]);
           mv_center[r] = mv_all[0][0];
           sad_inter = sad < sad_inter ? sad : sad_inter;
         }
+        me_drop_window(t, ws->mep);
         if (intra_inter_sad) {
           do_inter = sad_inter < sad_intra;
           if (sad_inter < sad_intra) do_intra = 0;
diff --git a/thor_amd/csrc/tk_block_queue.h b/thor_amd/csrc/tk_block_queue.h
--- a/thor_amd/csrc/tk_block_queue.h
+++ b/thor_amd/csrc/tk_block_queue.h
@@ -151,8 +151,7 @@
   if (t.rank == 0) add_mvcand(ws->mep, r, mvp);
   t.sync();
   mv_t mv_center = mvp;
-  if (t.rank == 0) ldsc(ws->mep)->cwin_valid = 0;
-  t.sync();
+  me_drop_window(t, ws->mep);
   for (int part = 0; part < max_pb; part++) {
     mv_t mv_all[4];
     search_inter<PIX, SP>(t, J, ws, nd.ypos, nd.xpos, size, oy, ws->org_sy, r, mv_center, mvp, mv_all, part, J.sign[r]);
@@ -171,8 +170,7 @@
     }
     t.sync();
   }
-  if (t.rank == 0) ldsc(ws->mep)->cwin_valid = 0;
-  t.sync();
+  me_drop_window(t, ws->mep);
 }
 
 template <typename PIX, int SP>
@@ -223,7 +221,7 @@
   int ref0 = 0, ref1 = 0;
   unsigned min_sad = 1u << 30;
   if (wg.wave == 0 && t.rank == 0) sh->bp_org8 = ws->org8;
-  t.sync();
+  me_drop_window(t, ws->mep);
   wg.barrier();
   PIX* const org8 = (PIX*)sh->bp_org8;
   const int whole = nd.bw == size && nd.bh == size;
@@ -283,6 +281,7 @@
         }
       }
     }
+  me_drop_window(t, ws->mep);
   for (int tb = 0; tb <= max_tb - 1; tb++)
     if (wg.wave == tb % wg.nwaves) {
       BlkParam p = blank_param();
diff --git a/thor_amd/csrc/tk_block_search.h b/thor_amd/csrc/tk_block_search.h
--- a/thor_amd/csrc/tk_block_search.h
+++ b/thor_amd/csrc/tk_block_search.h
@@ -99,6 +99,7 @@
   const int osy = ws->org_sy;
   int prev_ref[2] = {-1, -1}, prev_cnt[2][kMaxRefs];
   mv_t prev_mv[2][4];
+  me_drop_window(t, ws->mep);
   for (int n = 0; n < num_iter; n++) {
     const int stop = part == 0 ? 0 : 1;
     for (int list = 1; list >= stop; list--) {
@@ -141,6 +142,7 @@
       }
     }
   }
+  me_drop_window(t, ws->mep);
   *ref_idx0 = min_ref0;
   *ref_idx1 = min_ref1;
   for (int i = 0; i < 4; i++) { mv_arr0[i] = min0[i]; mv_arr1[i] = min1[i]; }
diff --git a/thor_amd/csrc/tk_common.h b/thor_amd/csrc/tk_common.h
--- a/thor_amd/csrc/tk_common.h
+++ b/thor_amd/csrc/tk_common.h
@@ -50,6 +50,11 @@
 #define TK_PROF_SUBPEL 1
 #else
 #define TK_PROF_SUBPEL 0
+#endif
+#if TK_PROF_DEV && defined(THOR_PROF_WIN)
+#define TK_PROF_WIN 1
+#else
+#define TK_PROF_WIN 0
 #endif
 #if defined(TK_MDW_INLINE)
 #define TK_MDW TK_DEV
diff --git a/thor_amd/csrc/tk_me.h b/thor_amd/csrc/tk_me.h
--- a/thor_amd/csrc/tk_me.h
+++ b/thor_amd/csrc/tk_me.h
@@ -4,6 +4,44 @@
 #include "tk_me_fastsub.h"
 
 namespace tk {
+
+template <typename PIX>
+TK_DEV void me_stage_rows(const Team t, MeWs* w_, const PIX* src, int rstride, int Ww, int Wh, int pitch) {
+  const uint32_t* w32 = lds_ld(&w_->win);
+  const int rowb = Ww * (int)sizeof(PIX);
+  const int spr = (rowb + 15) >> 4, total = spr * Wh;
+#if TK_PROF_WIN
+  const long long pw0_ = (long long)__builtin_readcyclecounter();
+#endif
+  t.sync();
+  for (int k0 = 0; k0 < total; k0 += t.size) {
+    const int k = k0 + t.rank;
+    if (k < total) {
+      const int row = k / spr, sg = k - row * spr;
+      const Seg16 v = seg_load<SP_GLOBAL, 16>((const char*)(src + row * rstride) + 16 * sg);
+      const int d = (row * pitch + 16 * sg) >> 2;
+      const int nd = tmin(4, (rowb - 16 * sg) >> 2);
+#if TK_HOST
+      for (int q = 0; q < nd; q++) ((uint32_t*)w32)[d + q] = v.d[q];
+#else
+      TK_LDS uint32_t* l = (TK_LDS uint32_t*)(uint32_t)(uintptr_t)w32 + d;
+      l[0] = v.d[0];
+      if (nd > 1) l[1] = v.d[1];
+      if (nd > 2) l[2] = v.d[2];
+      if (nd > 3) l[3] = v.d[3];
+#endif
+    }
+  }
+  t.sync();
+#if TK_PROF_WIN
+  if (t.rank == 0) { const auto w = ldsc(w_); w->prof[30] += 1; w->prof[31] += (long long)__builtin_readcyclecounter() - pw0_; }
+#endif
+}
+
+TK_DEV void me_drop_window(const Team t, MeWs* w_) {
+  if (t.rank == 0) ldsc(w_)->cwin_valid = 0;
+  t.sync();
+}
 
 template <typename PIX>
 TK_DEV void me_stage_cb_window(const Team t, MeWs* w_, const PIX* ref_cb, int rstride, int cb_x, int cb_y, int cb, mv_t mvc, int sign, int fwidth,
@@ -18,29 +56,11 @@
   const int ox = s * (mv_ref.x >> 2) - R, oy = s * (mv_ref.y >> 2) - R;
   const int ok = TKU(w->win != nullptr && R >= kMeWinRmin && cb_x + ox >= -kPadY && cb_x + ox + Ww <= fwidth + kPadY && cb_y + oy >= -kPadY &&
                      cb_y + oy + Wh <= fheight + kPadY);
-  t.sync();
-  if (ok) {
-    const uint32_t* w32 = lds_ld(&w_->win);
-    const int rowb = Ww * S, spr = (rowb + 15) >> 4, total = spr * Wh;
-    for (int k0 = 0; k0 < total; k0 += t.size) {
-      const int k = k0 + t.rank;
-      if (k < total) {
-        const int row = k / spr, sg = k - row * spr;
-        const Seg16 v = seg_load<SP_GLOBAL, 16>((const char*)(ref_cb + (oy + row) * rstride + ox) + 16 * sg);
-        const int d = (row * pitch + 16 * sg) >> 2;
-        const int nd = tmin(4, (rowb - 16 * sg) >> 2);
-#if TK_HOST
-        for (int q = 0; q < nd; q++) ((uint32_t*)w32)[d + q] = v.d[q];
-#else
-        TK_LDS uint32_t* l = (TK_LDS uint32_t*)(uint32_t)(uintptr_t)w32 + d;
-        l[0] = v.d[0];
-        if (nd > 1) l[1] = v.d[1];
-        if (nd > 2) l[2] = v.d[2];
-        if (nd > 3) l[3] = v.d[3];
-#endif
-      }
-    }
-  }
+#ifndef TK_ME_WIN_NO_REUSE
+  if (TKU(ok && w->cwin_valid && w->cwin_ref == ref_idx && w->cwin_ax == cb_x + ox && w->cwin_ay == cb_y + oy && w->cwin_Ww == Ww && w->cwin_Wh == Wh)) return;
+#endif
+  if (ok) me_stage_rows<PIX>(t, w_, ref_cb + oy * rstride + ox, rstride, Ww, Wh, pitch);
+  else t.sync();
   if (t.rank == 0) {
     w->cwin_valid = ok; w->cwin_ref = ref_idx; w->cwin_ax = cb_x + ox; w->cwin_ay = cb_y + oy; w->cwin_Ww = Ww; w->cwin_Wh = Wh; w->cwin_pitch = pitch;
   }
@@ -110,28 +130,17 @@
                    a.pu_y + win.oy + win.Wh <= a.fheight + kPadY);
     }
     if (win.on) {
-      const int rowb = win.Ww * S;
-      const int spr = (rowb + 15) >> 4, total = spr * win.Wh;
-      t.sync();
-      for (int k0 = 0; k0 < total; k0 += t.size) {
-        const int k = k0 + t.rank;
-        if (k < total) {
-          const int row = k / spr, sg = k - row * spr;
-          const Seg16 v = seg_load<SP_GLOBAL, 16>((const char*)(ref + (win.oy + row) * a.rstride + win.ox) + 16 * sg);
-          const int d = (row * win.pitch + 16 * sg) >> 2;
-          const int nd = tmin(4, (rowb - 16 * sg) >> 2);
-#if TK_HOST
-          for (int q = 0; q < nd; q++) ((uint32_t*)win.w32)[d + q] = v.d[q];
-#else
-          TK_LDS uint32_t* l = (TK_LDS uint32_t*)(uint32_t)(uintptr_t)win.w32 + d;
-          l[0] = v.d[0];
-          if (nd > 1) l[1] = v.d[1];
-          if (nd > 2) l[2] = v.d[2];
-          if (nd > 3) l[3] = v.d[3];
-#endif
-        }
-      }
-      t.sync();
+      me_stage_rows<PIX>(t, w_, ref + win.oy * a.rstride + win.ox, a.rstride, win.Ww, win.Wh, win.pitch);
+#ifndef TK_ME_WIN_NO_REUSE
+      const int whole = TKU(a.width == a.cb_size && a.height == a.cb_size && a.pu_x == a.xpos && a.pu_y == a.ypos);
+      if (whole || TKU(w->cwin_valid)) {
+        if (t.rank == 0) {
+          w->cwin_valid = whole; w->cwin_ref = ref_idx; w->cwin_ax = a.pu_x + win.ox; w->cwin_ay = a.pu_y + win.oy; w->cwin_Ww = win.Ww; w->cwin_Wh = win.Wh;
+          w->cwin_pitch = win.pitch;
+        }
+        t.sync();
+      }
+#endif
     }
   }
   auto eval_wide = [&](int n) -> unsigned long long {
diff --git a/thor_amd/csrc/tk_me_lanes.h b/thor_amd/csrc/tk_me_lanes.h
--- a/thor_amd/csrc/tk_me_lanes.h
+++ b/thor_amd/csrc/tk_me_lanes.h
@@ -244,7 +244,7 @@
   const mv_t mv = mk_mv(base.x + ox, base.y + oy);
   const SubPel sp = luma_setup(mv, sign, width, height, fw, fh, xpos, ypos, bip);
   const int centre = sp.ver_frac == 2 && sp.hor_frac == 2 && bip < 2;
-  const int outside = !(sp.hor_int - 2 >= win.ox && sp.hor_int + width + 6 <= win.ox + win.Ww && sp.ver_int - 2 >= win.oy && sp.ver_int + height + 3 <= win.oy + win.Wh);
+  const int outside = !(sp.hor_int - 2 >= win.ox && sp.hor_int + width + 5 <= win.ox + win.Ww && sp.ver_int - 2 >= win.oy && sp.ver_int + height + 3 <= win.oy + win.Wh);
   if (team_ballot(t, outside) != 0ull) return kNone;
   const int dual = team_ballot(t, centre) != 0ull;
   const unsigned long long thA = centre ? 0x0000000001010000ull : sp.ph, thB = centre ? 0x0000000102020100ull : sp.ph;
@@ -317,7 +317,7 @@
   const mv_t mv = mk_mv(base.x + ox, base.y + oy);
   const SubPel sp = luma_setup(mv, sign, width, height, fw, fh, xpos, ypos, bip);
   const int centre = sp.ver_frac == 2 && sp.hor_frac == 2 && bip < 2;
-  const int outside = !(sp.hor_int - 2 >= win.ox && sp.hor_int + width + 6 <= win.ox + win.Ww && sp.ver_int - 2 >= win.oy && sp.ver_int + height + 3 <= win.oy + win.Wh);
+  const int outside = !(sp.hor_int - 2 >= win.ox && sp.hor_int + width + 3 <= win.ox + win.Ww && sp.ver_int - 2 >= win.oy && sp.ver_int + height + 3 <= win.oy + win.Wh);
   if (team_ballot(t, outside) != 0ull) return kNone;
   const int dual = team_ballot(t, centre) != 0ull;
   auto pair = [](int a, int b) -> uint32_t { return (uint32_t)(uint16_t)(int16_t)a | ((uint32_t)(uint16_t)(int16_t)b << 16); };
diff --git a/thor_amd/csrc/tk_xform.h b/thor_amd/csrc/tk_xform.h
--- a/thor_amd/csrc/tk_xform.h
+++ b/thor_amd/csrc/tk_xform.h
@@ -450,7 +450,9 @@
   qp = tk_uniform(qp); coeff_type = tk_uniform(coeff_type); fast = tk_uniform(fast); bitdepth = tk_uniform(bitdepth);
   TK_PROF_T0();
   fwd_transform<PIX, SP>(t, ws, org, ostride, pred, pstride, size, fast, bitdepth);
+#ifndef THOR_PROF_WIN
   TK_PROF_ADD(ws, 30);
+#endif
   TK_PROF_MARK(pq0_);
   int cbp = quantize_team<SC>(t, ws, coefq, qp, size, (coeff_type >> 1) & 1);
   TK_PROF_ACC(ws, 12, pq0_);
@@ -458,7 +460,9 @@
     TK_PROF_MARK(pi0_);
     dequantize<SC>(t, ws, coefq, qp, size);
     inv_transform_recon<PIX, SP>(t, ws, pred, pstride, rec, rstride, size, bitdepth);
+#ifndef THOR_PROF_WIN
     TK_PROF_ACC(ws, 31, pi0_);
+#endif
   } else {
     copy_block<SP, SP>(t, rec, rstride, pred, pstride, size, size);
     t.sync();
```

Result: no change. 164.6, median of 6 (+0.4%).
